# zbw2577/fea-large

Measured on AMD Instinct MI355X. Metric: element-stiffness assemblies/sec, higher is better.
Workload: dtype f64; 1 GPU; 10349856 TET4/1GP neohookean block (66x396x66 Kuhn cubes on the 1x6x1 bar), stiffness+residual assembly, deformed state k1=1.1; elements=10349856, nodes=1782133, scalar_nnz=236453589, clock_ramp_launches_before_warmup=80

## Files before the change

### fea-large_amd/csrc/feahip_internal.h

```cpp
#pragma once
#include <hip/hip_runtime.h>
#include <algorithm>
#include <cstdint>
#include <cstdio>
#include <initializer_list>
#include <string>
#include <thread>
#include <type_traits>
#include <vector>
#include "../../include/fea_hip.h"

hipError_t feahip_device_malloc(void **p, size_t bytes);
#define hipMalloc(p, bytes) feahip_device_malloc((void **)(p), (bytes))

#define FEA_MAX_NPE 10
#define FEA_MAX_GAUSS 27

#define FEA_CHUNK_BLOCKS 128
#define FEA_CHUNK_ROWS 16
#define FEA_WAVES_PER_WG 4
#define FEA_RED_BLOCKS 2048

struct ElemTable {
  double w[FEA_MAX_GAUSS];
  double dN[FEA_MAX_GAUSS][3][FEA_MAX_NPE];
};

#define FEA_HIP_CHECK(ctx, call)                                            \
  do {                                                                      \
    hipError_t _e = (call);                                                 \
    if (_e != hipSuccess) {                                                 \
      (ctx)->err = std::string(#call) + ": " + hipGetErrorString(_e);       \
      return FEAHIP_EHIP;                                                   \
    }                                                                       \
  } while (0)

template <class F>
void parallel_ranges(int n, int serial_below, F f)
{
  unsigned hw = std::thread::hardware_concurrency();
  int nt = (int)std::min<unsigned>(hw ? hw : 4, 32);
  if (n < serial_below) nt = 1;
  if (nt <= 1) { f(0, n); return; }
  std::vector<std::thread> th;
  for (int t = 0; t < nt; ++t) {
    int lo = (int)((long long)n * t / nt), hi = (int)((long long)n * (t + 1) / nt);
    th.emplace_back([=] { f(lo, hi); });
  }
  for (auto &x : th) x.join();
}
inline int round_up(int v, int m) { return (v + m - 1) / m * m; }

struct HostPattern {
  std::vector<int> rowptr, colidx;
  std::vector<int> incptr;
  std::vector<uint32_t> inc;
  std::vector<uint8_t> incslot;
  std::vector<int> chunk;
  std::vector<int> diag;
  std::vector<uint32_t> inc_rows;
  std::vector<int> achunk;
  std::vector<int> super_achunk;
  int max_rowlen = 0;
  int break_chunk = 0, break_super = 0;
};
int build_host_pattern(int N, int E, int npe, const int *conn, HostPattern &hp,
                       std::string &err, int row_break = -1);
inline int inc_elem(uint32_t w) { return (int)(w & 0x0FFFFFFFu); }
inline int inc_node(uint32_t w) { return (int)(w >> 28); }
inline int csr_pos(const HostPattern &hp, int a, int b)
{
  const int *cb = hp.colidx.data() + hp.rowptr[a], *ce = hp.colidx.data() + hp.rowptr[a + 1];
  return hp.rowptr[a] + (int)(std::lower_bound(cb, ce, b) - cb);
}

#define FEA_VISIT_MAX_NODES 64
#define FEA_VISIT_MAX_VISITS 128
#define FEA_ACHUNK_BLOCKS 80
#define FEA_ACHUNK_ROWS 8
#define FEA_SUPER_CHUNKS 8
struct VisitDesc {
  int r0, r1, b0, nb;
  int node_off, nnode;
  int visit_off, nvisit;
};
struct HostVisits {
  std::vector<VisitDesc> desc;
  std::vector<int> vnode;
  std::vector<uint32_t> vrec;
  bool ok = false;
};
void build_host_visits(int N, int E, const int *conn, const HostPattern &hp, HostVisits &out);
#define FEA_QUAD_BLOCKS 256
#define FEA_QUAD_PAIRS 512
#define FEA_QUAD_ELEMS 64
#define FEA_QUAD_NODES 126
#define FEA_QUAD_VISITS 96
struct QuadDesc {
  int r0, r1, b0, nb;
  int elem_off, nelem;
  int pair_off, npair;
  int node_off, nnode;
};
struct HostQuad {
  std::vector<QuadDesc> desc;
  std::vector<int> qnode;
  std::vector<uint32_t> qelem;
  std::vector<uint32_t> qpair;
  bool ok = false;
};
void build_host_quad(int N, int E, int npe, const int *conn, const HostPattern &hp, int p_lo, int p_hi, HostQuad &out);
int ensure_quad(feahip_ctx *c);
int launch_assemble_quad(feahip_ctx *c, bool doF);

inline bool first_visit(const HostPattern &hp, const int *conn, int npe, uint32_t w, int r0, int r)
{
  const int e = inc_elem(w), la = inc_node(w);
  for (int k = 0; k < npe; ++k) {
    const int g = conn[(size_t)e * npe + k];
    if (k != la && g >= r0 && g < r) return false;
  }
  return true;
}
template <class Fits>
void chunk_costs(const HostPattern &hp, const int *conn, int npe, int r0, int row_hi, int L, std::vector<int> &fresh,
                 uint16_t *cost, Fits fits)
{
  int nel = 0, ntask = 0;
  for (int l = 1; l <= L && r0 + l <= row_hi; ++l) {
    const int r = r0 + l - 1;
    fresh.clear();
    for (int q = hp.incptr[r]; q < hp.incptr[r + 1]; ++q)
      if (first_visit(hp, conn, npe, hp.inc_rows[q], r0, r)) fresh.push_back(inc_elem(hp.inc_rows[q]));
    nel += (int)fresh.size();
    const int *cb = hp.colidx.data() + hp.rowptr[r], *ce = hp.colidx.data() + hp.rowptr[r + 1];
    ntask += (int)(ce - cb) - 1 - (int)(std::lower_bound(cb, ce, r) - std::lower_bound(cb, ce, r0));
    if (!fits(r, l, nel, ntask, fresh)) break;
    cost[l - 1] = (uint16_t)nel;
  }
}
int partition_rows(const std::vector<uint16_t> &cost, int row_lo, int row_hi, int L, int alpha, std::vector<int> &first_row);
void chunk_elements(const HostPattern &hp, int r0, int r1, std::vector<int> &el);
void chunk_block_tasks(const HostPattern &hp, int r0, int r1, std::vector<uint32_t> &tpos, std::vector<int> &task_of);
void chunk_block_lists(const HostPattern &hp, const int *conn, int npe, int r0, int r1, const std::vector<int> &el,
                       const std::vector<int> &task_of, int ntask, int la_shift, int lb_shift,
                       std::vector<std::vector<uint16_t>> &lists);
long long count_distinct_elems(const HostPattern &hp, const int *conn, int npe, int r0, int r1);
struct HostChunkMaps {
  std::vector<unsigned char> blob;
  std::vector<int> first_row;
  long long total_evals = 0, distinct_elems = 0;
  int nchunks = 0;
  bool ok = false;
};

#ifndef FEA_G_BIG
#define FEA_G_BIG 1
#endif
#if FEA_G_BIG == 1
#define FEA_G_THREADS 1024
#define FEA_G_TASK_THREADS 768
#define FEA_G_MAX_ROWS 64
#define FEA_G_MAX_NODES 256
#define FEA_G_MAX_ELEMS 719
#define FEA_G_ELEMS_TARGET 672
#define FEA_G_CELL 4, 4, 4
#elif FEA_G_BIG == 2
#define FEA_G_THREADS 512
#define FEA_G_TASK_THREADS 384
#define FEA_G_MAX_ROWS 32
#define FEA_G_MAX_NODES 128
#define FEA_G_MAX_ELEMS 351
#define FEA_G_ELEMS_TARGET 320
#define FEA_G_CELL 4, 2, 3
#else
#define FEA_G_THREADS 256
#define FEA_G_TASK_THREADS 192
#define FEA_G_MAX_ROWS 16
#define FEA_G_MAX_NODES 128
#define FEA_G_MAX_ELEMS 239
#define FEA_G_ELEMS_TARGET 216
#define FEA_G_CELL 4, 2, 2
#endif
#define FEA_G_DIAG_LANES (FEA_G_THREADS - FEA_G_TASK_THREADS)
#define FEA_G_SLOT_BITS 10
#define FEA_G_MAX_SLOTS 1024
#define FEA_G_REGW 6
struct GatherHeader {
  int r0, r1, b0, nb;
  int nnode, nelem, noffd, depth;
  int nvthr, vdepth;
  int ddepth;
  unsigned wdepth[3];
  int flags;
  int pad[1];
};
static_assert(sizeof(GatherHeader) == 64 && FEA_G_TASK_THREADS / 64 <= 12, "GatherHeader: 64 bytes, twelve block-wave slots");
struct GatherLayout {
  int stride;
  int o_nodes, o_elems, o_bpos, o_rows, o_vlist, o_dlist, o_clist;
  int max_nodes, max_elems, max_tile;
  int max_tasks, max_depth, max_vthr, max_vdepth, max_ddepth;
  int o_emat;
};
struct HostGather : HostChunkMaps {
  GatherLayout lay;
  int same_as_previous = 0;
};
void build_host_gather(int N, int E, const int *conn, const HostPattern &hp, int row_lo, int row_hi, HostGather &out,
                       const uint8_t *elem_mat = nullptr);
int ensure_gather(feahip_ctx *c);
int launch_assemble_gather(feahip_ctx *c, bool doK, bool doF);

#ifndef FEA_Q_THREADS
#define FEA_Q_THREADS 256
#endif
#define FEA_Q_WAVES (FEA_Q_THREADS / 64)
#define FEA_Q_MAX_ROWS 64
#define FEA_Q_MAX_NODES 240
#define FEA_Q_MAX_ELEMS 127
#ifndef FEA_Q_SLOTS
#define FEA_Q_SLOTS 5
#endif
#define FEA_Q_REGW 4
#define FEA_Q_MAX_PASS 7
#define FEA_Q_FLANES 128
#define FEA_Q_ROWS_U16 200
struct Gather10Header {
  int r0, r1, b0, nb;
  int nnode, nelem, ntask, npass;
  int nft, fdw;
  unsigned char prow[8];
  unsigned char cnt[40];
  unsigned char sw[8];
  int pad[8];
};
static_assert(FEA_Q_SLOTS * FEA_Q_WAVES <= 40 && FEA_Q_SLOTS <= 8, "Gather10Header: cnt / sw too small");
static_assert(sizeof(Gather10Header) == 128, "Gather10Header is 128 bytes");
struct Gather10Layout {
  int stride;
  int o_nodes, o_elems, o_rows, o_tpos, o_flist, o_clist;
  int max_nodes, max_elems, max_cw, max_fdw, tile_blocks;
};
enum Gather10Limit {
  G10_FITS = FEAHIP_G10_LIMIT_NONE, G10_ELEMS = FEAHIP_G10_LIMIT_ELEMS, G10_ROW_LENGTH = FEAHIP_G10_LIMIT_ROW_LENGTH,
  G10_TASKS = FEAHIP_G10_LIMIT_TASKS, G10_RESIDUAL_LANES = FEAHIP_G10_LIMIT_RESIDUAL_LANES,
  G10_LIST_LENGTH = FEAHIP_G10_LIMIT_LIST_LENGTH, G10_PASSES = FEAHIP_G10_LIMIT_PASSES, G10_OTHER = FEAHIP_G10_LIMIT_OTHER
};
struct HostGather10 : HostChunkMaps {
  Gather10Layout lay;
  std::vector<int> elist;
  int npe = 10;
  int limit = G10_FITS;
  int limit_row = -1;
  int tile_blocks = 0;
};
void build_host_gather10(int N, int E, int npe, const int *conn, const HostPattern &hp, int row_lo, int row_hi, HostGather10 &out);
int ensure_gather10(feahip_ctx *c);
int launch_assemble_gather10(feahip_ctx *c, bool doK, bool doF);

int launch_assemble_visit(feahip_ctx *c, bool doK, bool doF);

enum class MapOutcome { none, built, failed, declined };
struct MapCache {
  int key0 = -1, key1 = -1;
  MapOutcome outcome = MapOutcome::none;
  long long bytes = 0;
  bool built() const { return outcome == MapOutcome::built; }
  bool is(MapOutcome o, int k0, int k1) const { return outcome == o && key0 == k0 && key1 == k1; }
  bool settled(int k0, int k1) const { return is(MapOutcome::built, k0, k1) || is(MapOutcome::failed, k0, k1); }
  void record(MapOutcome o, int k0, int k1) { outcome = o; key0 = k0; key1 = k1; }
};
inline void dev_free(std::initializer_list<void *> ptrs) { for (void *p : ptrs) if (p) (void)hipFree(p); }
struct GenericMaps : MapCache {
  int *d_incptr = nullptr;
  uint32_t *d_inc = nullptr;
  uint8_t *d_incslot = nullptr;
  void release() { dev_free({d_incptr, d_inc, d_incslot}); *this = GenericMaps(); }
};
struct VisitMaps : MapCache {
  VisitDesc *d_desc = nullptr;
  int *d_node = nullptr;
  uint32_t *d_rec = nullptr;
  int nrecords = 0;
  void release() { dev_free({d_desc, d_node, d_rec}); *this = VisitMaps(); }
};
struct QuadMaps : MapCache {
  QuadDesc *d_desc = nullptr;
  uint32_t *d_elem = nullptr, *d_pair = nullptr;
  int *d_node = nullptr;
  int nchunks = 0;
  void release() { dev_free({d_desc, d_elem, d_pair, d_node}); *this = QuadMaps(); }
};
struct GatherCache : MapCache {
  unsigned char *d_maps = nullptr;
  int nchunks = 0;
  double evals_per_element = 0;
  int same_words = 0;
};
struct GatherMaps : GatherCache {
  GatherLayout lay{};
  void release() { dev_free({d_maps}); *this = GatherMaps(); }
};
struct Gather10Maps : GatherCache {
  Gather10Layout lay{};
  int *d_elist = nullptr;
  double *d_state = nullptr;
  int nloc = 0;
  void release() { dev_free({d_maps, d_elist, d_state}); *this = Gather10Maps(); }
};

struct SurfaceLoads {
  int nfaces = 0, npf = 0;
  std::vector<int> h_lnode;
  int *d_fnode = nullptr;
  int *d_kind = nullptr;
  double *d_val = nullptr;
  double *d_fc = nullptr;
  int *d_lnode = nullptr, *d_lptr = nullptr, *d_lslot = nullptr;
  void release() { dev_free({d_fnode, d_kind, d_val, d_fc, d_lnode, d_lptr, d_lslot}); *this = SurfaceLoads(); }
};

struct MassState {
  bool set = false;
  bool stale = false;
  int n_rho = 0, n_mat = 0, Gm = 0;
  std::vector<double> rho, w, N, dN;
  double *d_m_base = nullptr;
  double *d_m = nullptr;
  long long kb0 = -1, kb1 = -1;
  double *d_vel = nullptr, *d_acc = nullptr, *d_xt = nullptr, *d_vt = nullptr;
  double *d_body = nullptr;
  double body[3] = {0, 0, 0};
  double time = 0;
  double *d_ml = nullptr;
  int ml_row0 = -1, ml_row1 = -1;
  double *d_ke_part = nullptr;
  int ke_parts = 0;
  void release_m() { dev_free({d_m_base}); d_m_base = d_m = nullptr; kb0 = kb1 = -1; }
  void release_lump() { dev_free({d_ml, d_ke_part}); d_ml = d_ke_part = nullptr; ml_row0 = ml_row1 = -1; ke_parts = 0; }
  void release() { dev_free({d_m_base, d_vel, d_acc, d_xt, d_vt, d_body, d_ml, d_ke_part}); *this = MassState(); }
};

struct feahip_ctx {
  int device = 0;
  hipStream_t stream = nullptr;
  std::string err;

  int N = 0, E = 0, npe = 0, G = 0, ndof = 0;
  int nnzb = 0;
  int nchunks = 0;
  int chunk0 = 0, nchunks_local = 0;
  int nachunks = 0, achunk0 = 0, nachunks_local = 0;
  std::vector<int> h_super_achunk, h_chunk;
  int rank = 0, nranks = 1, row0 = 0, row1 = 0;
  struct Transport *tr = nullptr;
  bool owns_tr = false;
  std::vector<int> peer, send_off, recv_off;
  int nsend = 0, nrecv = 0;
  int *d_send_idx = nullptr, *d_recv_idx = nullptr;
  double *d_send_buf = nullptr, *d_recv_buf = nullptr;
  int max_rowlen = 0;
  bool linear_tet = false;
  int model = 0;
  double lambda = 0, mu = 0;
  int n_materials = 0;
  std::vector<double> h_mat_params;
  std::vector<uint8_t> h_elem_mat;
  double2 *d_mat = nullptr;
  uint8_t *d_elem_mat = nullptr;
  double *d_f_discard = nullptr;
  int strategy = FEAHIP_ASM_AUTO;
  int last_strategy = FEAHIP_ASM_AUTO;

  ElemTable table;
  ElemTable *d_table = nullptr;

  int *d_conn = nullptr;
  double *d_X0 = nullptr;
  double *d_x = nullptr;
  int *d_rowptr = nullptr;
  int *d_colidx = nullptr;
  double *d_K = nullptr;
  double *d_Kstash = nullptr;
  double *d_K_base = nullptr, *d_Kstash_base = nullptr;
  double *d_K_alloc = nullptr, *d_Kstash_alloc = nullptr;
  long long kb0 = 0, kb1 = 0;
  bool have_stash = false;
  int *d_chunk = nullptr;
  int *d_diag = nullptr;
  GenericMaps generic;
  VisitMaps visits;
  QuadMaps quad;
  GatherMaps gather;
  Gather10Maps gather10;
  double *d_f = nullptr, *d_u = nullptr;
  double *d_r = nullptr, *d_p = nullptr, *d_q = nullptr, *d_minv = nullptr;
  double *d_part = nullptr;
  double *d_z = nullptr, *d_w = nullptr, *d_s = nullptr;
  int pcg_variant = -1;
  int ichunk_lo = 0, ichunk_hi = 0;
  hipStream_t comm_stream = nullptr;
  hipEvent_t ev_packed = nullptr, ev_unpacked = nullptr;
  double *d_scal = nullptr;
  int *d_flag = nullptr;
  int n_presc = 0;
  int n_cdof = 0;
  int *d_cdof = nullptr;
  double *d_cval = nullptr;
  uint8_t *d_dofmask = nullptr;
  double *d_F = nullptr, *d_S = nullptr;
  bool state_valid = false;

  std::vector<int> h_rowptr, h_colidx;
  std::vector<int> h_conn;
  struct HostPattern *h_pat = nullptr;
  bool incslot_ok = false;

  int last_bad = 0;

  std::vector<int> perm, iperm;
  int rank_own = -1;
  std::vector<int> rank_node_global, rank_elem_global;
  int rank_n_global = 0;
  int rank_e_global = 0;
  bool rank_local_ids = false;

  unsigned long long k_epoch = 0, stash_epoch = 0;
  bool k_bc = false;
  bool k_valid = false;
  int linesearch_max = 0;
  int precond = 0;
  void *amg = nullptr;
  void *coarse = nullptr;
  double *d_vred = nullptr;
  size_t vred_cap = 0;
  SurfaceLoads surf;
  double load_factor = 0;
  double *d2_f = nullptr, *d2_u = nullptr, *d2_r = nullptr, *d2_p = nullptr, *d2_q = nullptr;
  double *d_u2 = nullptr;
  double *d2_part = nullptr;
  double *d2_scal = nullptr;
  int *d2_flag = nullptr;
  MassState mass;
};

template <class F>
void with_kf(bool doK, bool doF, F &&f)
{
  if (doK && doF) f(std::true_type(), std::true_type());
  else if (doK)   f(std::true_type(), std::false_type());
  else            f(std::false_type(), std::true_type());
}

int launch_assemble(feahip_ctx *c, bool doK, bool doF);
int launch_state_export(feahip_ctx *c, double *d_grads = nullptr, double *d_detj = nullptr);
int launch_apply_bc(feahip_ctx *c, double lambda);
int launch_update_nodes_bc(feahip_ctx *c, double lambda);
int launch_surface_loads(feahip_ctx *c, double *d_fv);
int resolve_surface_faces(int N, int E, int npe, const int *conn, int nfaces, int npf, const int *face_nodes,
                          int *face_elem, int *face_local, std::string &why);
int set_surface_loads(feahip_ctx *c, int nfaces, int npf, const int *face_nodes, const int *kind, const double *values);
int ensure_generic_maps(feahip_ctx *c);
int ensure_k(feahip_ctx *c);
void release_k(feahip_ctx *c);
int ensure_visits(feahip_ctx *c);
int dist_nodes_add_scaled(std::vector<feahip_ctx *> &R, double eta, bool exchange);
int launch_update_nodes_solution(feahip_ctx *c, const double *d_u);
int launch_spmv(feahip_ctx *c, const double *d_xv, double *d_yv);
int precond_apply(feahip_ctx *c, const double *r, const double **z);
int solve_pcg(feahip_ctx *c, int type, double tol, int max_iter, int *iters,
              double *resid);
int time_pcg_iteration(feahip_ctx *c, int warmup, int iters, double *avg_ms);
bool pcg_outcome(int flag, int it, const double *scal, int *iters, double *resid);
void enq_reduce_final(feahip_ctx *c, int n, int nsums, int stride, const double *part, double *out);
void enq_precond_blockjacobi(feahip_ctx *c);
int ensure_solve2(feahip_ctx *c);
void release_solve2(feahip_ctx *c);
int solve2_refused(feahip_ctx *c, const char *who);
int launch_spmv2(feahip_ctx *c, const double *d_x2, double *d_y2);
int launch_interleave(feahip_ctx *c, const double *a, const double *b, double *out2);
int launch_deinterleave(feahip_ctx *c, const double *in2, double *a, double *b);
int solve_pcg2(feahip_ctx *c, int type, double tol, int max_iter, int *iters, double *resid);
int time_pcg2_iteration(feahip_ctx *c, int warmup, int iters, double *avg_ms);
int mass_set(feahip_ctx *c, int n_rho, const double *rho, int mass_points, const double *weights, const double *forms,
             const double *dforms);
int mass_ensure(feahip_ctx *c, const char *who);
int mass_set_body_force(feahip_ctx *c, const double *b);
int launch_body_force(feahip_ctx *c, double *d_fv);
int launch_mass_add(feahip_ctx *c, double coef);
int launch_mass_residual(feahip_ctx *c, double a0);
int launch_mass_product(feahip_ctx *c, const double *d_v4, double *d_y);
int launch_newmark_predict(feahip_ctx *c, double dt, double beta, double gamma);
int launch_newmark_correct(feahip_ctx *c, double dt, double beta, double gamma);
int launch_vec3_to_nodes(feahip_ctx *c, const double *d_v3, double *d_v4);
int lump_ensure(feahip_ctx *c, const char *who);
int launch_explicit_kick(feahip_ctx *c, double dt);
int launch_explicit_presc(feahip_ctx *c, double dlambda, double dt);
int launch_explicit_finish(feahip_ctx *c, double dt);
int launch_kinetic_energy(feahip_ctx *c, double *d_out);
// ... 98 lines not shown
```

### fea-large_amd/csrc/gather.cpp

```cpp
#include "feahip_internal.h"
#include <algorithm>
#include <cstdlib>
#include <cstring>

int partition_rows(const std::vector<uint16_t> &cost, int row_lo, int row_hi, int L, int alpha, std::vector<int> &first_row)
{
  const int nrows = row_hi - row_lo;
  std::vector<long long> best((size_t)nrows + 1, -1);
  std::vector<unsigned char> from((size_t)nrows + 1, 0);
  best[0] = 0;
  for (int j = 1; j <= nrows; ++j) {
    long long b = -1; int bl = 0;
    for (int l = 1; l <= L && l <= j; ++l) {
      const uint16_t c = cost[(size_t)(j - l) * L + (l - 1)];
      if (c == 0xFFFFu || best[j - l] < 0) continue;
      const long long v = best[j - l] + c + alpha;
      if (b < 0 || v < b) { b = v; bl = l; }
    }
    if (b < 0) return row_lo + j - 1;
    best[j] = b; from[j] = (unsigned char)bl;
  }
  std::vector<int> cuts;
  for (int j = nrows; j > 0; j -= from[j]) cuts.push_back(row_lo + j);
  cuts.push_back(row_lo);
  first_row.assign(cuts.rbegin(), cuts.rend());
  return -1;
}

void chunk_elements(const HostPattern &hp, int r0, int r1, std::vector<int> &el)
{
  el.clear();
  for (int q = hp.incptr[r0]; q < hp.incptr[r1]; ++q) el.push_back(inc_elem(hp.inc_rows[q]));
  std::sort(el.begin(), el.end());
  el.erase(std::unique(el.begin(), el.end()), el.end());
}

void chunk_block_tasks(const HostPattern &hp, int r0, int r1, std::vector<uint32_t> &tpos, std::vector<int> &task_of)
{
  const int b0 = hp.rowptr[r0];
  tpos.clear();
  task_of.assign((size_t)(hp.rowptr[r1] - b0), -1);
  for (int a = r0; a < r1; ++a)
    for (int q = hp.rowptr[a]; q < hp.rowptr[a + 1]; ++q) {
      const int b = hp.colidx[q];
      if (b == a || (b >= r0 && b < a)) continue;
      const uint32_t m = b > a && b < r1 ? (uint32_t)(csr_pos(hp, b, a) - b0) : 0xFFFFu;
      task_of[q - b0] = (int)tpos.size();
      tpos.push_back((uint32_t)(q - b0) | m << 16);
    }
}

void chunk_block_lists(const HostPattern &hp, const int *conn, int npe, int r0, int r1, const std::vector<int> &el,
                       const std::vector<int> &task_of, int ntask, int la_shift, int lb_shift,
                       std::vector<std::vector<uint16_t>> &lists)
{
  const int b0 = hp.rowptr[r0];
  lists.assign((size_t)ntask, std::vector<uint16_t>());
  for (int a = r0; a < r1; ++a)
    for (int q = hp.incptr[a]; q < hp.incptr[a + 1]; ++q) {
      const int e = inc_elem(hp.inc_rows[q]), la = inc_node(hp.inc_rows[q]);
      const int le = (int)(std::lower_bound(el.begin(), el.end(), e) - el.begin());
      for (int lb = 0; lb < npe; ++lb) {
        if (lb == la) continue;
        const int b = conn[(size_t)e * npe + lb];
        if (b == a) continue;
        const int t = task_of[csr_pos(hp, a, b) - b0];
        if (t < 0) continue;
        lists[(size_t)t].push_back((uint16_t)(le | la << la_shift | lb << lb_shift));
      }
    }
}

long long count_distinct_elems(const HostPattern &hp, const int *conn, int npe, int r0, int r1)
{
  long long d = 0;
  for (int a = r0; a < r1; ++a)
    for (int q = hp.incptr[a]; q < hp.incptr[a + 1]; ++q) d += first_visit(hp, conn, npe, hp.inc_rows[q], r0, a);
  return d;
}

#define G_RS 0
#define G_RD 66
#define G_VF 130
#define G_ROWS_U16 200
#define G_TASK_THREADS FEA_G_TASK_THREADS
#define G_SLOT(w) ((w) & 1023u)
#define G_LA(w) (((w) >> 10) & 3)
#define G_LB(w) (((w) >> 12) & 3)
#define G_NGROUPS (FEA_G_THREADS / 16)

namespace {
inline int b128_group(int t)
{
  static const unsigned char g32[32] = {0, 0, 0, 0, 1, 1, 1, 1, 1, 1, 1, 1, 0, 0, 0, 0, 1, 1, 1, 1, 0, 0, 0, 0, 0, 0, 0, 0, 1, 1, 1, 1};
  return (t >> 6) * 4 + ((t >> 5) & 1) * 2 + g32[t & 31];
}

bool partition(int N, const int *conn, const HostPattern &hp, int row_lo, int row_hi, std::vector<int> &first_row)
{
  int max_rows = FEA_G_MAX_ROWS, max_elems = FEA_G_BIG == 1 ? FEA_G_MAX_ELEMS : FEA_G_ELEMS_TARGET, alpha = 24;
  if (const char *e = getenv("FEAHIP_GATHER_ROWS")) max_rows = std::max(1, std::min(FEA_G_MAX_ROWS, atoi(e)));
  if (const char *e = getenv("FEAHIP_GATHER_ELEMS")) max_elems = std::max(8, std::min(FEA_G_MAX_ELEMS, atoi(e)));
  if (const char *e = getenv("FEAHIP_GATHER_ALPHA")) alpha = std::max(0, atoi(e));
  const int L = max_rows, nrows = row_hi - row_lo;
  std::vector<uint16_t> cost((size_t)nrows * L, 0xFFFFu);
  parallel_ranges(nrows, 4096, [&](int lo, int hi) {
    std::vector<int> nstamp((size_t)N, -1), fresh;
    for (int i = lo; i < hi; ++i) {
      const int r0 = row_lo + i;
      int nnod = 0, nvis = 0;
      chunk_costs(hp, conn, 4, r0, row_hi, L, fresh, &cost[(size_t)i * L], [&](int r, int l, int nel, int ntask, const std::vector<int> &fr) {
        if (nstamp[r] != r0) { nstamp[r] = r0; ++nnod; }
        for (int e : fr)
          for (int k = 0; k < 4; ++k) {
            const int g = conn[(size_t)e * 4 + k];
            if (nstamp[g] != r0) { nstamp[g] = r0; ++nnod; }
          }
        nvis += hp.incptr[r + 1] - hp.incptr[r];
        return nel <= (l > 1 ? max_elems : FEA_G_MAX_ELEMS) && nnod <= FEA_G_MAX_NODES && ntask <= G_TASK_THREADS &&
               nvis <= 4 * G_TASK_THREADS;
      });
    }
  });
  return partition_rows(cost, row_lo, row_hi, L, alpha, first_row) < 0;
}

struct Read { uint16_t set; uint8_t off; };

void sort_unique(std::vector<Read> &rv)
{
  std::sort(rv.begin(), rv.end(), [](const Read &a, const Read &b) { return a.set != b.set ? a.set < b.set : a.off < b.off; });
  rv.erase(std::unique(rv.begin(), rv.end(), [](const Read &a, const Read &b) { return a.set == b.set && a.off == b.off; }), rv.end());
}

void most_read_first(const std::vector<std::vector<Read>> &reads, std::vector<int> &order)
{
  order.resize(reads.size());
  for (size_t i = 0; i < reads.size(); ++i) order[i] = (int)i;
  std::stable_sort(order.begin(), order.end(), [&](int a, int b) { return reads[a].size() > reads[b].size(); });
}

void bank_slots(const std::vector<std::vector<Read>> &reads, const std::vector<int> &order, int nsets, int step,
                std::vector<int> cap, std::vector<uint8_t> &occ, std::vector<int> &res, std::vector<int> &slot)
{
  const int n = (int)reads.size();
  occ.assign((size_t)nsets * 16, 0);
  res.assign((size_t)n, -1);
  auto bank = [&](const Read &rd, int r) { return (size_t)rd.set * 16 + ((rd.off + step * r) & 15); };
  for (int pass = 0; pass < 2; ++pass)
    for (int i : order) {
      if (res[i] >= 0) {
        for (const Read &rd : reads[i]) --occ[bank(rd, res[i])];
        ++cap[res[i]];
      }
      int br = -1; long bc = 0;
      for (int r = 0; r < 16; ++r) {
        if (cap[r] <= 0) continue;
        long c = 0;
        for (const Read &rd : reads[i]) c += occ[bank(rd, r)];
        if (br < 0 || c < bc) { br = r; bc = c; }
      }
      res[i] = br; --cap[br];
      for (const Read &rd : reads[i]) ++occ[bank(rd, br)];
    }
  int next[16];
  for (int r = 0; r < 16; ++r) next[r] = r;
  slot.resize((size_t)n);
  for (int i = 0; i < n; ++i) { slot[i] = next[res[i]]; next[res[i]] += 16; }
}

struct Local {
  GatherHeader h;
  std::vector<int> nodes;
  std::vector<uint32_t> elems, tpos;
  std::vector<uint16_t> rows, vlist, clist, dlist;
  std::vector<uint8_t> emat;
};

struct ChunkBuilder {
  const int *conn;
  const HostPattern &hp;
  const uint8_t *elem_mat;
  int r0 = 0, r1 = 0, nrows = 0, b0 = 0, nb = 0, nelem = 0, nnode = 0, nslots = 0, nnslots = 0;
  int ntask = 0, wdepth[G_TASK_THREADS / 64] = {0}, dwords = 0, ddwords = 0, zslot = 0;
  std::vector<int> el, nd, task_of, thr_blk, order, res, eslot, nslot;
  std::vector<uint32_t> btpos;
  std::vector<std::vector<uint16_t>> blists, lists, dl;
  std::vector<std::vector<Read>> reads;
  std::vector<uint8_t> occ;

  ChunkBuilder(const int *c, const HostPattern &p, const uint8_t *em) : conn(c), hp(p), elem_mat(em) {}
  int lnode(int g) const { return (int)(std::lower_bound(nd.begin(), nd.end(), g) - nd.begin()); }
  int lelem(int e) const { return (int)(std::lower_bound(el.begin(), el.end(), e) - el.begin()); }

  bool build(int row0, int row1, Local &L)
  {
    r0 = row0; r1 = row1; nrows = r1 - r0; b0 = hp.rowptr[r0]; nb = hp.rowptr[r1] - b0;
    if (!chunk_lists(L)) return false;
    deal();
    bank_schedule();
    emit(L);
    return true;
  }

  bool chunk_lists(Local &L)
  {
    chunk_elements(hp, r0, r1, el);
    nd.clear();
    for (int a = r0; a < r1; ++a) nd.push_back(a);
    for (int e : el)
      for (int k = 0; k < 4; ++k) nd.push_back(conn[(size_t)e * 4 + k]);
    std::sort(nd.begin(), nd.end());
    nd.erase(std::unique(nd.begin(), nd.end()), nd.end());
    nnode = (int)nd.size(); nelem = (int)el.size();
    nslots = 16 * ((nelem + 1 + 15) / 16); nnslots = 16 * ((nnode + 15) / 16);
    if (nnslots > FEA_G_MAX_NODES || nslots > FEA_G_MAX_SLOTS || nrows > FEA_G_MAX_ROWS) return false;
    L.rows.assign(G_ROWS_U16, 0);
    for (int a = r0; a < r1; ++a) {
      L.rows[G_RS + (a - r0)] = (uint16_t)(hp.rowptr[a] - b0);
      L.rows[G_RD + (a - r0)] = (uint16_t)(hp.diag[a] - b0);
    }
    L.rows[G_RS + nrows] = (uint16_t)nb;
    chunk_block_tasks(hp, r0, r1, btpos, task_of);
    const int nblk = (int)btpos.size();
    if (nblk > G_TASK_THREADS) return false;
    chunk_block_lists(hp, conn, 4, r0, r1, el, task_of, nblk, 10, 12, blists);
    dl.assign((size_t)4 * FEA_G_MAX_ROWS, std::vector<uint16_t>());
    for (int a = r0; a < r1; ++a)
      for (int q = hp.incptr[a], kv = 0; q < hp.incptr[a + 1]; ++q, ++kv)
        dl[(size_t)4 * (a - r0) + (kv & 3)].push_back((uint16_t)(lelem(inc_elem(hp.inc_rows[q])) | (inc_node(hp.inc_rows[q]) << 10)));
    return true;
  }

  void deal()
  {
    constexpr int NBW = G_TASK_THREADS / 64;
    const int nblk = (int)btpos.size();
    thr_blk.assign((size_t)G_TASK_THREADS, -1);
    std::fill(wdepth, wdepth + NBW, 0);
    ntask = 0;
    auto words = [&](int i) { return ((int)blists[i].size() + 1) / 2; };
    order.resize((size_t)nblk);
    for (int i = 0; i < nblk; ++i) order[i] = i;
    std::stable_sort(order.begin(), order.end(), [&](int x, int y) { return words(x) > words(y); });
    std::vector<int> seq;
    seq.reserve((size_t)nblk);
    for (size_t c0 = 0; c0 < order.size();) {
      size_t c1 = c0;
      while (c1 < order.size() && words(order[c1]) == words(order[c0])) ++c1;
      std::vector<int> bucket[16];
      for (size_t k = c0; k < c1; ++k) bucket[btpos[order[k]] & 15u].push_back(order[k]);
      size_t left = c1 - c0;
      while (left) {
        const int room = 16 - (int)(seq.size() & 15);
        int rs[16];
        for (int r = 0; r < 16; ++r) rs[r] = r;
        std::stable_sort(rs, rs + 16, [&](int x, int y) { return bucket[x].size() > bucket[y].size(); });
        unsigned mused = 0;
        int taken = 0;
        for (int pass = 0; pass < 2 && taken < room && left; ++pass)
          for (int q = 0; q < 16 && taken < room && left; ++q) {
            std::vector<int> &bk = bucket[rs[q]];
            if (bk.empty()) continue;
            size_t pick = 0;
            for (size_t c = 0; c < bk.size() && c < 8; ++c) {
              const unsigned mp = btpos[bk[c]] >> 16;
              if (mp == 0xFFFFu || !((mused >> (mp & 15u)) & 1u)) { pick = c; break; }
            }
            const unsigned mp = btpos[bk[pick]] >> 16;
            if (mp != 0xFFFFu) mused |= 1u << (mp & 15u);
            seq.push_back(bk[pick]);
            bk.erase(bk.begin() + (long)pick);
            ++taken; --left;
          }
      }
      c0 = c1;
    }
    const int nwaves = (nblk + 63) / 64;
    std::vector<int> wcost((size_t)nwaves, 0), word((size_t)nwaves);
    for (int w = 0; w < nwaves; ++w) {
      for (int l = 0; l < 64 && w * 64 + l < nblk; ++l) wcost[w] = std::max(wcost[w], words(seq[(size_t)w * 64 + l]));
      word[w] = w;
    }
    std::stable_sort(word.begin(), word.end(), [&](int x, int y) { return wcost[x] > wcost[y]; });
    int load[4] = {0, 0, 0, 0}, used[4] = {0, 0, 0, 0};
    for (int w : word) {
      int bs = -1;
      for (int sd = 0; sd < 4; ++sd)
        if (used[sd] * 4 + sd < NBW && (bs < 0 || load[sd] < load[bs])) bs = sd;
      const int slot = used[bs] * 4 + bs;
      ++used[bs]; load[bs] += wcost[w];
      wdepth[slot] = wcost[w];
      for (int l = 0; l < 64 && w * 64 + l < nblk; ++l) thr_blk[(size_t)slot * 64 + l] = seq[(size_t)w * 64 + l];
      ntask = std::max(ntask, slot * 64 + std::min(64, nblk - w * 64));
    }
    lists.assign((size_t)ntask, std::vector<uint16_t>());
    for (int t = 0; t < ntask; ++t)
      if (thr_blk[t] >= 0) lists[t] = blists[thr_blk[t]];
    int depth = 0, ddepth = 0;
    for (auto &l : lists) depth = std::max(depth, (int)l.size());
    for (auto &l : dl) ddepth = std::max(ddepth, (int)l.size());
    dwords = (depth + 1) / 2; ddwords = (ddepth + 1) / 2;
  }

  void bank_schedule()
  {
    reads.assign((size_t)nelem, std::vector<Read>());
    const int nsteps = std::max(2 * dwords, 2 * ddwords);
    auto add_reads = [&](int lane, int step, uint16_t w, bool diag) {
      const int le = (int)G_SLOT(w), la = G_LA(w), lb = G_LB(w);
      const int grp = b128_group(lane);
      const int offs[6] = {la, 8 + la, diag ? 4 + la : lb, diag ? -1 : 4 + lb, diag ? -1 : 8 + lb, 12};
      for (int kind = 0; kind < 6; ++kind)
        if (offs[kind] >= 0) reads[le].push_back({(uint16_t)((grp * nsteps + step) * 6 + kind), (uint8_t)offs[kind]});
    };
    for (int t = 0; t < ntask; ++t)
      for (size_t k = 0; k < lists[t].size(); ++k) add_reads(t, (int)k, lists[t][k], false);
    for (int l = 0; l < 4 * nrows; ++l)
      for (size_t k = 0; k < dl[l].size(); ++k) add_reads(G_TASK_THREADS + l, (int)k, dl[l][k], true);
    most_read_first(reads, order);
    for (auto &rv : reads) sort_unique(rv);
    std::vector<int> cap(16, nslots / 16);
    --cap[15];
    bank_slots(reads, order, G_NGROUPS * nsteps * 6, -3, cap, occ, res, eslot);
    std::vector<char> used((size_t)nslots, 0);
    for (int e = 0; e < nelem; ++e) used[eslot[e]] = 1;
    zslot = 0;
    while (used[zslot]) ++zslot;

    reads.assign((size_t)nnode, std::vector<Read>());
    for (int e = 0; e < nelem; ++e)
      for (int k = 0; k < 4; ++k) reads[lnode(conn[(size_t)el[e] * 4 + k])].push_back({(uint16_t)(b128_group(eslot[e]) * 4 + k), 0});
    for (auto &rv : reads) sort_unique(rv);
    most_read_first(reads, order);
    bank_slots(reads, order, G_NGROUPS * 4, 1, std::vector<int>(16, nnslots / 16), occ, res, nslot);
  }

  void emit(Local &L)
  {
    L.nodes.assign((size_t)nnslots, 0);
    for (int i = 0; i < nnode; ++i) L.nodes[nslot[i]] = nd[i];
    L.elems.assign((size_t)nslots, 0xFFFFFFFFu);
    for (int i = 0; i < nelem; ++i) {
      uint32_t w = 0;
      for (int k = 0; k < 4; ++k) w |= (uint32_t)nslot[lnode(conn[(size_t)el[i] * 4 + k])] << (8 * k);
      L.elems[eslot[i]] = w;
    }
    L.emat.clear();
    if (elem_mat) {
      L.emat.assign((size_t)nslots, 0);
      for (int i = 0; i < nelem; ++i) L.emat[eslot[i]] = elem_mat[el[i]];
    }
    L.tpos.assign((size_t)ntask, 0xFFFFFFFFu);
    for (int t = 0; t < ntask; ++t)
      if (thr_blk[t] >= 0) L.tpos[t] = btpos[thr_blk[t]];
    auto reslot = [&](uint16_t w) { return (uint16_t)((w & 0xFC00u) | (uint16_t)eslot[G_SLOT(w)]); };
    L.clist.assign((size_t)dwords * 2 * FEA_G_THREADS, (uint16_t)zslot);
    for (int t = 0; t < ntask; ++t)
      for (size_t k = 0; k < lists[t].size(); ++k)
        L.clist[((size_t)(k / 2) * FEA_G_THREADS + t) * 2 + (k & 1)] = reslot(lists[t][k]);
    L.dlist.assign((size_t)ddwords * 2 * FEA_G_DIAG_LANES, (uint16_t)zslot);
    for (int l = 0; l < 4 * nrows; ++l)
      for (size_t k = 0; k < dl[l].size(); ++k)
        L.dlist[((size_t)(k / 2) * FEA_G_DIAG_LANES + l) * 2 + (k & 1)] = reslot(dl[l][k]);
    int vdepth = 1;
    for (;; ++vdepth) {
      int need = 0;
      for (int a = r0; a < r1; ++a) need += (hp.incptr[a + 1] - hp.incptr[a] + vdepth - 1) / vdepth;
      if (need <= G_TASK_THREADS) break;
    }
    int nvthr = 0;
    for (int a = r0; a < r1; ++a) {
      L.rows[G_VF + (a - r0)] = (uint16_t)nvthr;
      nvthr += (hp.incptr[a + 1] - hp.incptr[a] + vdepth - 1) / vdepth;
    }
    L.rows[G_VF + nrows] = (uint16_t)nvthr;
    L.vlist.assign((size_t)vdepth * FEA_G_THREADS, (uint16_t)zslot);
    for (int a = r0; a < r1; ++a) {
      const int t0 = L.rows[G_VF + (a - r0)];
      for (int q = hp.incptr[a], k = 0; q < hp.incptr[a + 1]; ++q, ++k)
        L.vlist[(size_t)(k % vdepth) * FEA_G_THREADS + t0 + k / vdepth] = (uint16_t)(eslot[lelem(inc_elem(hp.inc_rows[q]))] | (inc_node(hp.inc_rows[q]) << 10));
    }
    GatherHeader &h = L.h;
    memset(&h, 0, sizeof(h));
    h.r0 = r0; h.r1 = r1; h.b0 = b0; h.nb = nb; h.nnode = nnslots; h.nelem = nslots; h.noffd = ntask;
    h.depth = dwords; h.nvthr = nvthr; h.vdepth = vdepth; h.ddepth = ddwords;
    for (int w = 0; w < G_TASK_THREADS / 64; ++w) h.wdepth[w >> 2] |= (unsigned)std::min(wdepth[w], 255) << (8 * (w & 3));
  }
};

bool lay_out(const std::vector<Local> &loc, bool materials, HostGather &out)
{
  const int nch = (int)loc.size();
  int m_v = 0, m_c = 0, m_d = 0, g_nodes = 0, g_elems = 0, g_tile = 0;
  GatherLayout &lay = out.lay;
  memset(&lay, 0, sizeof(lay));
  for (const Local &L : loc) {
    m_v = std::max(m_v, (int)L.vlist.size() * 2); m_c = std::max(m_c, (int)L.clist.size() * 2); m_d = std::max(m_d, (int)L.dlist.size() * 2);
    g_nodes = std::max(g_nodes, L.h.nnode); g_elems = std::max(g_elems, L.h.nelem); g_tile = std::max(g_tile, L.h.nb);
    lay.max_tasks = std::max(lay.max_tasks, L.h.noffd); lay.max_depth = std::max(lay.max_depth, L.h.depth);
    lay.max_vthr = std::max(lay.max_vthr, L.h.nvthr); lay.max_vdepth = std::max(lay.max_vdepth, L.h.vdepth);
    lay.max_ddepth = std::max(lay.max_ddepth, L.h.ddepth);
  }
  lay.max_nodes = g_nodes; lay.max_elems = g_elems; lay.max_tile = g_tile;
  lay.o_nodes = 64;
  lay.o_elems = lay.o_nodes + round_up(4 * FEA_G_MAX_NODES, 64);
  lay.o_bpos = lay.o_elems + round_up(4 * FEA_G_THREADS, 64);
  lay.o_rows = lay.o_bpos + round_up(4 * FEA_G_THREADS, 64);
  lay.o_vlist = lay.o_rows + round_up(2 * G_ROWS_U16, 64);
  lay.o_dlist = lay.o_vlist + round_up(m_v, 64);
  lay.o_clist = lay.o_dlist + round_up(m_d, 64);
  lay.stride = round_up(lay.o_clist + m_c, 128);
  if (materials) { lay.o_emat = lay.stride; lay.stride += round_up(FEA_G_THREADS, 128); }
  if ((long long)nch * lay.stride > 0x7FFFFFFF00LL) return false;
  out.blob.assign((size_t)nch * lay.stride, 0);
  parallel_ranges(nch, 512, [&](int lo, int hi) {
    for (int p = lo; p < hi; ++p) {
      const Local &L = loc[p];
      unsigned char *rec = out.blob.data() + (size_t)p * lay.stride;
      memcpy(rec, &L.h, sizeof(GatherHeader));
      memcpy(rec + lay.o_nodes, L.nodes.data(), L.nodes.size() * 4);
      memcpy(rec + lay.o_elems, L.elems.data(), L.elems.size() * 4);
      memcpy(rec + lay.o_bpos, L.tpos.data(), L.tpos.size() * 4);
      memcpy(rec + lay.o_rows, L.rows.data(), L.rows.size() * 2);
      memcpy(rec + lay.o_vlist, L.vlist.data(), L.vlist.size() * 2);
      memcpy(rec + lay.o_dlist, L.dlist.data(), L.dlist.size() * 2);
      memcpy(rec + lay.o_clist, L.clist.data(), L.clist.size() * 2);
      if (lay.o_emat) memcpy(rec + lay.o_emat, L.emat.data(), L.emat.size());
    }
  });
  return true;
}

void mark_repeats(HostGather &out, int nch)
{
  const GatherLayout &lay = out.lay;
  out.same_as_previous = 0;
  for (int p = 0; p + 1 < nch; ++p) {
    const unsigned char *r0 = out.blob.data() + (size_t)p * lay.stride, *r1 = r0 + lay.stride;
    const GatherHeader &h0 = *reinterpret_cast<const GatherHeader *>(r0), &h1 = *reinterpret_cast<const GatherHeader *>(r1);
    const bool same = h0.nelem == h1.nelem && h0.noffd == h1.noffd && h0.depth == h1.depth && h0.nvthr == h1.nvthr &&
                      h0.vdepth == h1.vdepth && h0.ddepth == h1.ddepth && h0.r1 - h0.r0 == h1.r1 - h1.r0 &&
                      memcmp(r0 + lay.o_elems, r1 + lay.o_elems, (size_t)((lay.o_emat ? lay.o_emat : lay.stride) - lay.o_elems)) == 0;
    if (same) { reinterpret_cast<GatherHeader *>(out.blob.data() + (size_t)p * lay.stride)->flags |= 1; ++out.same_as_previous; }
  }
}
}

void build_host_gather(int N, int E, const int *conn, const HostPattern &hp, int row_lo, int row_hi, HostGather &out,
                       const uint8_t *elem_mat)
{
  (void)E;
  out.ok = false; out.nchunks = 0; out.blob.clear(); out.first_row.clear();
  if (row_lo < 0 || row_hi > N || row_lo >= row_hi) return;
  if (!partition(N, conn, hp, row_lo, row_hi, out.first_row)) return;
  const int nch = (int)out.first_row.size() - 1;
  std::vector<Local> loc((size_t)nch);
  std::vector<char> bad((size_t)nch, 0);
  parallel_ranges(nch, 512, [&](int lo, int hi) {
    ChunkBuilder cb(conn, hp, elem_mat);
    for (int p = lo; p < hi; ++p) bad[p] = !cb.build(out.first_row[p], out.first_row[p + 1], loc[p]);
  });
  for (int p = 0; p < nch; ++p)
    if (bad[p]) return;
  if (!lay_out(loc, elem_mat != nullptr, out)) return;
  mark_repeats(out, nch);
  out.nchunks = nch;
  out.total_evals = 0;
  for (const Local &L : loc)
    for (uint32_t w : L.elems) out.total_evals += w != 0xFFFFFFFFu;
  out.distinct_elems = count_distinct_elems(hp, conn, 4, row_lo, row_hi);
  out.ok = true;
}

namespace {
inline unsigned long long mix(unsigned long long h, unsigned long long v)
{
  h ^= v + 0x9E3779B97F4A7C15ull + (h << 6) + (h >> 2);
  return h * 0xBF58476D1CE4E5B9ull;
}
inline unsigned long long contribution_hash(int a, int b, const int *g, int npe, int pair)
{
  unsigned long long h = 0x1234567ull;
  h = mix(h, (unsigned long long)a); h = mix(h, (unsigned long long)b);
  for (int k = 0; k < npe; ++k) h = mix(h, (unsigned long long)g[k]);
  return mix(h, (unsigned long long)pair);
}
int row_of(const HostPattern &hp, int r0, int r1, int b0, int pos)
{
  int a = r0;
  while (a + 1 < r1 && hp.rowptr[a + 1] - b0 <= pos) ++a;
  return a;
}

void gather_row_digest(const HostGather &hg, const HostPattern &hp, unsigned long long *rowhash)
{
  const GatherLayout &lay = hg.lay;
  for (int p = 0; p < hg.nchunks; ++p) {
    const unsigned char *rec = hg.blob.data() + (size_t)p * lay.stride;
    const GatherHeader &h = *reinterpret_cast<const GatherHeader *>(rec);
    const int *nodes = reinterpret_cast<const int *>(rec + lay.o_nodes);
    const uint32_t *elems = reinterpret_cast<const uint32_t *>(rec + lay.o_elems);
    const uint32_t *tpos = reinterpret_cast<const uint32_t *>(rec + lay.o_bpos);
    const uint16_t *clist = reinterpret_cast<const uint16_t *>(rec + lay.o_clist);
    const uint16_t *dlist = reinterpret_cast<const uint16_t *>(rec + lay.o_dlist);
    auto element_nodes = [&](int slot, int g[4]) {
      for (int k = 0; k < 4; ++k) g[k] = nodes[(elems[slot] >> (8 * k)) & 255u];
    };
    for (int t = 0; t < h.noffd; ++t) {
      if (tpos[t] == 0xFFFFFFFFu) continue;
      const int bpos = (int)(tpos[t] & 0xFFFFu), mpos = (int)(tpos[t] >> 16);
      const int a = row_of(hp, h.r0, h.r1, h.b0, bpos), b = hp.colidx[h.b0 + bpos];
      for (int k = 0; k < 2 * h.depth; ++k) {
        const uint16_t w = clist[((size_t)(k / 2) * FEA_G_THREADS + t) * 2 + (k & 1)];
        const int slot = (int)G_SLOT(w), la = G_LA(w), lb = G_LB(w);
        if (elems[slot] == 0xFFFFFFFFu) continue;
        int g[4];
        element_nodes(slot, g);
        rowhash[a] += contribution_hash(a, b, g, 4, la * 4 + lb);
        if (mpos != 0xFFFF) rowhash[b] += contribution_hash(b, a, g, 4, lb * 4 + la);
      }
    }
    for (int l = 0; l < 4 * (h.r1 - h.r0); ++l)
      for (int k = 0; k < 2 * h.ddepth; ++k) {
        const uint16_t w = dlist[((size_t)(k / 2) * FEA_G_DIAG_LANES + l) * 2 + (k & 1)];
        const int slot = (int)G_SLOT(w), la = G_LA(w);
        if (elems[slot] == 0xFFFFFFFFu) continue;
        int g[4];
        element_nodes(slot, g);
        const int a = h.r0 + (l >> 2);
        rowhash[a] += contribution_hash(a, a, g, 4, la * 4 + la);
      }
  }
}

void gather10_row_digest(const HostGather10 &hg, const HostPattern &hp, const int *conn, unsigned long long *rowhash)
{
  const Gather10Layout &lay = hg.lay;
  for (int p = 0; p < hg.nchunks; ++p) {
    const unsigned char *rec = hg.blob.data() + (size_t)p * lay.stride;
    const Gather10Header &h = *reinterpret_cast<const Gather10Header *>(rec);
    const uint32_t *elems = reinterpret_cast<const uint32_t *>(rec + lay.o_elems);
    const uint32_t *tpos = reinterpret_cast<const uint32_t *>(rec + lay.o_tpos);
    const uint16_t *cl = reinterpret_cast<const uint16_t *>(rec + lay.o_clist);
    int row0 = 0;
    for (int s = 0; s < FEA_Q_SLOTS; ++s) {
      for (int t = 0; t < FEA_Q_THREADS; ++t) {
        const uint32_t tw = tpos[s * FEA_Q_THREADS + t];
        if (tw == 0xFFFFFFFFu) continue;
        const int bpos = (int)(tw & 0xFFFFu), mpos = (int)(tw >> 16);
        const int a = row_of(hp, h.r0, h.r1, h.b0, bpos), b = hp.colidx[h.b0 + bpos];
        for (int k = 0; k < 2 * h.sw[s]; ++k) {
          const uint16_t w = cl[(((size_t)row0 + k / 2) * FEA_Q_THREADS + t) * 2 + (k & 1)];
          const int le = w & 127, la = (w >> 7) & 15, lb = (w >> 11) & 15;
          if (le == lay.max_elems) continue;
          int g[16];
          for (int j = 0; j < hg.npe; ++j) g[j] = conn[(size_t)hg.elist[elems[le]] * hg.npe + j];
          rowhash[a] += contribution_hash(a, b, g, hg.npe, la * 16 + lb);
          if (mpos != 0xFFFF) rowhash[b] += contribution_hash(b, a, g, hg.npe, lb * 16 + la);
        }
      }
      row0 += h.sw[s];
    }
  }
}

void quad_row_digest(const HostQuad &hq, const HostPattern &hp, unsigned long long *rowhash)
{
  for (const QuadDesc &d : hq.desc) {
    for (int p = 0; p < d.npair; ++p) {
      const uint32_t w = hq.qpair[(size_t)d.pair_off + p];
      const int eli = (int)(w & 63u), la = (int)((w >> 6) & 15u), lb = (int)((w >> 10) & 15u), pos = (int)((w >> 14) & 255u);
      const int a = d.r0 + (int)((w >> 22) & 15u), b = hp.colidx[d.b0 + pos];
      const uint32_t *we = hq.qelem.data() + ((size_t)d.elem_off + eli) * 3;
      int g[10];
      for (int k = 0; k < 10; ++k) g[k] = hq.qnode[(size_t)d.node_off + ((we[k / 4] >> (8 * (k % 4))) & 255u)];
      rowhash[a] += contribution_hash(a, b, g, 10, la * 16 + lb);
    }
  }
}
}

extern "C" int feahip_host_assembly_digest(int n_nodes, int n_elems, int npe, const int *elements, int rank, int nranks,
                                           unsigned long long *rowhash, int *rows)
{
  if (!elements || !rowhash || !rows || n_nodes <= 0 || n_elems <= 0 || nranks < 1 || rank < 0 || rank >= nranks) return FEAHIP_EINVAL;
  HostPattern hp;
  std::string err;
  int rc = build_host_pattern(n_nodes, n_elems, npe, elements, hp, err);
  if (rc) return rc;
  int row0, row1;
  shard_row_range(hp.chunk, rank, nranks, row0, row1);
  rows[0] = row0; rows[1] = row1;
  for (int a = 0; a < n_nodes; ++a) rowhash[a] = 0;
  if (npe == 4) {
    HostGather hg;
    build_host_gather(n_nodes, n_elems, elements, hp, row0, row1, hg);
    if (!hg.ok) return FEAHIP_EINVAL;
    gather_row_digest(hg, hp, rowhash);
  } else {
    bool done = false;
    if (npe == 10 || npe == 8) {
      HostGather10 hg;
      build_host_gather10(n_nodes, n_elems, npe, elements, hp, row0, row1, hg);
      if (hg.ok && (double)hg.total_evals <= 12.0 * (double)hg.distinct_elems) {
        gather10_row_digest(hg, hp, elements, rowhash);
        done = true;
      }
    }
    if (!done) {
      if (hp.super_achunk.empty()) return FEAHIP_EINVAL;
      const int nchunks = (int)hp.chunk.size() - 1;
      const int nsuper = (nchunks + FEA_SUPER_CHUNKS - 1) / FEA_SUPER_CHUNKS;
      const int s0 = (int)((long long)nsuper * rank / nranks), s1 = (int)((long long)nsuper * (rank + 1) / nranks);
      HostQuad hq;
      build_host_quad(n_nodes, n_elems, npe, elements, hp, hp.super_achunk[s0], hp.super_achunk[s1], hq);
      if (!hq.ok) return FEAHIP_EINVAL;
      quad_row_digest(hq, hp, rowhash);
    }
  }
  return FEAHIP_OK;
}

extern "C" int feahip_host_gather_stats(int n_nodes, int n_elems, int npe, const int *elements, long long *stats, int *rows_hist)
{
  if (!elements || !stats || n_nodes <= 0 || n_elems <= 0 || (npe != 4 && npe != 10 && npe != 8)) return FEAHIP_EINVAL;
  HostPattern hp;
  std::string err;
  int rc = build_host_pattern(n_nodes, n_elems, npe, elements, hp, err);
  if (rc) return rc;
  stats[6] = stats[7] = 0;
  HostGather hg;
  HostGather10 hq;
  const HostChunkMaps &m = npe == 4 ? static_cast<const HostChunkMaps &>(hg) : hq;
  if (npe == 4) build_host_gather(n_nodes, n_elems, elements, hp, 0, n_nodes, hg);
  else build_host_gather10(n_nodes, n_elems, npe, elements, hp, 0, n_nodes, hq);
  if (!m.ok) return FEAHIP_EINVAL;
  stats[0] = m.nchunks; stats[1] = m.total_evals; stats[2] = m.distinct_elems; stats[3] = n_nodes;
  stats[4] = npe == 4 ? hg.same_as_previous : 0; stats[5] = (long long)m.blob.size();
  if (npe == 4) {
    for (int p = 0; p < hg.nchunks; ++p) {
      const GatherHeader &gh = *reinterpret_cast<const GatherHeader *>(hg.blob.data() + (size_t)p * hg.lay.stride);
      stats[6] += gh.depth > FEA_G_REGW; stats[7] += gh.ddepth > FEA_G_REGW;
    }
    if (getenv("FEAHIP_NUMBERING_VERBOSE")) {
      int hd[17] = {0}, hdd[17] = {0};
      for (int p = 0; p < hg.nchunks; ++p) {
        const GatherHeader &gh = *reinterpret_cast<const GatherHeader *>(hg.blob.data() + (size_t)p * hg.lay.stride);
        ++hd[std::min(gh.depth, 16)]; ++hdd[std::min(gh.ddepth, 16)];
      }
      for (int k = 0; k <= 16; ++k) if (hd[k] || hdd[k]) fprintf(stderr, "gather maps: %d words: %d chunks by block list, %d by diagonal list\n", k, hd[k], hdd[k]);
    }
  }
  if (rows_hist) {
    for (int l = 0; l <= FEA_G_MAX_ROWS; ++l) rows_hist[l] = 0;
    for (int p = 0; p < m.nchunks; ++p) ++rows_hist[std::min(m.first_row[p + 1] - m.first_row[p], FEA_G_MAX_ROWS)];
  }
  return FEAHIP_OK;
}

extern "C" int feahip_host_gather_chunks(int n_nodes, int n_elems, const int *elements, int capacity, int *flags)
{
  if (!elements || n_nodes <= 0 || n_elems <= 0 || capacity < 0 || (capacity > 0 && !flags)) return FEAHIP_EINVAL;
  HostPattern hp;
  std::string err;
  int rc = build_host_pattern(n_nodes, n_elems, 4, elements, hp, err);
  if (rc) return rc;
  HostGather hg;
  build_host_gather(n_nodes, n_elems, elements, hp, 0, n_nodes, hg);
  if (!hg.ok) return FEAHIP_EINVAL;
  for (int p = 0; p < hg.nchunks && p < capacity; ++p) {
    const GatherHeader &gh = *reinterpret_cast<const GatherHeader *>(hg.blob.data() + (size_t)p * hg.lay.stride);
    flags[p] = (gh.flags & 1) | (gh.depth > FEA_G_REGW ? 2 : 0) | (gh.ddepth > FEA_G_REGW ? 4 : 0);
  }
  return hg.nchunks;
}

#ifdef FEAHIP_DEBUG
extern "C" int feahip_debug_gather_record_host(int n_nodes, int n_elems, const int *elements, int chunk, int *layout_ints,
                                               unsigned char *record, int *nchunks)
{
  static HostGather hg;
  static int cached_n = -1, cached_e = -1;
  if (cached_n != n_nodes || cached_e != n_elems) {
    HostPattern hp;
    std::string err;
    if (build_host_pattern(n_nodes, n_elems, 4, elements, hp, err)) return FEAHIP_EINVAL;
    build_host_gather(n_nodes, n_elems, elements, hp, 0, n_nodes, hg);
    if (!hg.ok) return FEAHIP_EINVAL;
    cached_n = n_nodes; cached_e = n_elems;
  }
  if (chunk < 0) chunk = hg.nchunks / 2;
  memcpy(layout_ints, &hg.lay, sizeof(GatherLayout));
  if (nchunks) *nchunks = hg.nchunks;
  if (record) memcpy(record, hg.blob.data() + (size_t)chunk * hg.lay.stride, hg.lay.stride);
  return (int)(sizeof(GatherLayout) / sizeof(int));
}
#endif
```

### fea-large_amd/csrc/gather_device.h

```cpp
#pragma once
#include "fem_device.h"
#define PRIO_STATE 0
#define PRIO_GATHER 1
#define PRIO_OUT 3
#include <algorithm>
#include <cstdlib>
#include <cstring>

struct GatherArgs {
  int chunk0, nchunks, model;
  double lambda, mu;
  const ElemTable *tab;
  const unsigned char *maps;
  GatherLayout lay;
  const double *X0, *x;
  double *K, *f;
  int *bad;
  unsigned long long *stamps;
  int ablate;
  const double2 *mat;
};
#if defined(FEAHIP_DEBUG) && !defined(FEAHIP_NOABL)
#define G_ABL(bit) (A.ablate & (bit))
#else
#define G_ABL(bit) 0
#endif

#ifdef FEAHIP_DEBUG
#define G_STAMP(i) do { if (A.stamps) st[i] = __builtin_amdgcn_s_memtime(); } while (0)
#else
#define G_STAMP(i) do { } while (0)
#endif

#define G_RS 0
#define G_RD 66
#define G_VF 130
#define G_SLOT(w) ((w) & 1023u)
#define G_LA(w) (((w) >> 10) & 3)
#define G_LB(w) (((w) >> 12) & 3)

#define GREC 26
#define GREC_F 12

struct GRead { double2 pa, za, pb, qb, zb, vv; };
__device__ __forceinline__ GRead g_fetch(const double *sT, unsigned w)
{
  const double2 *T = reinterpret_cast<const double2 *>(sT + G_SLOT(w) * GREC);
  const int la = G_LA(w), lb = G_LB(w);
  GRead r;
  r.pa = T[la]; r.za = T[8 + la]; r.pb = T[lb]; r.qb = T[4 + lb]; r.zb = T[8 + lb]; r.vv = T[12];
  return r;
}
__device__ __forceinline__ void g_apply(const GRead &r, double (&acc)[9], double &accd)
{
  const double ga0 = r.pa.x, ga1 = r.pa.y, ga2 = r.za.x;
  const double gb0 = r.pb.x, gb1 = r.pb.y, gb2 = r.zb.x;
  const double tb0 = r.qb.x, tb1 = r.qb.y, tb2 = r.zb.y;
  const double vl = r.vv.x, vm = r.vv.y;
  const double h0 = vl * gb0, h1 = vl * gb1, h2 = vl * gb2;
  const double m0 = vm * gb0, m1 = vm * gb1, m2 = vm * gb2;
  accd = fma(ga0, tb0, fma(ga1, tb1, fma(ga2, tb2, accd)));
  acc[0] = fma(ga0, h0, fma(ga0, m0, acc[0])); acc[1] = fma(ga0, h1, fma(ga1, m0, acc[1])); acc[2] = fma(ga0, h2, fma(ga2, m0, acc[2]));
  acc[3] = fma(ga1, h0, fma(ga0, m1, acc[3])); acc[4] = fma(ga1, h1, fma(ga1, m1, acc[4])); acc[5] = fma(ga1, h2, fma(ga2, m1, acc[5]));
  acc[6] = fma(ga2, h0, fma(ga0, m2, acc[6])); acc[7] = fma(ga2, h1, fma(ga1, m2, acc[7])); acc[8] = fma(ga2, h2, fma(ga2, m2, acc[8]));
}
__device__ __forceinline__ void g_finish(double (&acc)[9], double accd)
{
  acc[0] += accd; acc[4] += accd; acc[8] += accd;
}
__device__ __forceinline__ void g_consume(const double *sT, unsigned w, double (&acc)[9], double &accd)
{
  g_apply(g_fetch(sT, w), acc, accd);
}
__device__ __forceinline__ void g_apply_cheap(const GRead &r, double (&acc)[9])
{
  acc[0] += r.pa.x; acc[1] += r.za.x; acc[2] += r.pb.x; acc[3] += r.qb.x; acc[4] += r.zb.x; acc[5] += r.vv.x;
}
__device__ __forceinline__ GRead g_fetch_cheap(const double *sT, unsigned w)
{
  GRead r; const double v = (double)w;
  r.pa = make_double2(v, v); r.za = r.pa; r.pb = r.pa; r.qb = r.pa; r.zb = r.pa; r.vv = r.pa;
  return r;
}

template <bool DOF>
__device__ __forceinline__ void g_consume_diag(const double *sT, unsigned w, double (&a)[6], double (&fa)[3])
{
  const double2 *T = reinterpret_cast<const double2 *>(sT + G_SLOT(w) * GREC);
  const int la = G_LA(w);
  const double2 pa = T[la], qa = T[4 + la], za = T[8 + la], vv = T[12];
  const double s = vv.x + vv.y;
  const double d = pa.x * qa.x + pa.y * qa.y + za.x * za.y;
  const double h0 = s * pa.x, h1 = s * pa.y, h2 = s * za.x;
  a[0] += fma(h0, pa.x, d); a[1] = fma(h0, pa.y, a[1]); a[2] = fma(h0, za.x, a[2]);
  a[3] += fma(h1, pa.y, d); a[4] = fma(h1, za.x, a[4]); a[5] += fma(h2, za.x, d);
  if (DOF) {
    fa[0] -= __dsub_rn(qa.x, __dmul_rn(vv.y, pa.x)); fa[1] -= __dsub_rn(qa.y, __dmul_rn(vv.y, pa.y)); fa[2] -= __dsub_rn(za.y, __dmul_rn(vv.y, za.x));
  }
}

template <bool DOK>
__device__ __forceinline__ void g_visit(const double *sT, unsigned w, double (&fa)[3])
{
  const int la = G_LA(w);
  if (DOK) {
    const double2 *T = reinterpret_cast<const double2 *>(sT + G_SLOT(w) * GREC);
    const double2 pa = T[la], qa = T[4 + la], za = T[8 + la];
    const double vm = T[12].y;
    fa[0] -= qa.x - vm * pa.x; fa[1] -= qa.y - vm * pa.y; fa[2] -= za.y - vm * za.x;
  } else {
    const double *T = sT + G_SLOT(w) * GREC_F;
    const double2 pa = *reinterpret_cast<const double2 *>(T + 2 * la);
    fa[0] -= pa.x; fa[1] -= pa.y; fa[2] -= T[8 + la];
  }
}

#define G_W2(addr, a, b, o) asm volatile("ds_write2_b64 %0, %1, %2 offset0:%3 offset1:%4" : : "v"(addr), "v"(a), "v"(b), "n"(o), "n"((o) + 1) : "memory")
#define G_LDS_DRAIN() asm volatile("s_waitcnt lgkmcnt(0)" ::: "memory")
#ifndef G_W128
#define G_W128 1
#endif
typedef double g_v2d __attribute__((ext_vector_type(2)));
#if G_W128
#undef G_W2
#define G_W2(addr, a, b, o) do { const g_v2d pr_ = {a, b}; asm volatile("ds_write_b128 %0, %1 offset:%2" : : "v"(addr), "v"(pr_), "n"((o) * 8) : "memory"); } while (0)
#endif

template <bool DOK>
__device__ __forceinline__ void g_store_record(double *dst, const double *R)
{
  const unsigned a = (unsigned)(size_t)(__attribute__((address_space(3))) const void *)dst;
  G_W2(a, R[0], R[1], 0); G_W2(a, R[3], R[4], 2); G_W2(a, R[6], R[7], 4); G_W2(a, R[9], R[10], 6);
  if (DOK) {
    G_W2(a, R[12], R[13], 8); G_W2(a, R[15], R[16], 10); G_W2(a, R[18], R[19], 12); G_W2(a, R[21], R[22], 14);
    G_W2(a, R[2], R[14], 16); G_W2(a, R[5], R[17], 18); G_W2(a, R[8], R[20], 20); G_W2(a, R[11], R[23], 22);
    G_W2(a, R[24], R[25], 24);
  } else {
    G_W2(a, R[2], R[5], 8); G_W2(a, R[8], R[11], 10);
  }
}

template <bool DOK>
__device__ __forceinline__ double lintet_record_nh(const double (&x)[4][3], const double (&X)[4][3], double w,
                                                   double lambda, double mu, double *R)
{
  double J[3][3], D[3][3];
#pragma unroll
  for (int i = 0; i < 3; ++i)
#pragma unroll
    for (int j = 0; j < 3; ++j) { J[i][j] = x[i + 1][j] - x[0][j]; D[i][j] = X[i + 1][j] - X[0][j]; }
  double c[3][3];
  c[0][0] = J[1][1] * J[2][2] - J[1][2] * J[2][1]; c[0][1] = J[1][2] * J[2][0] - J[1][0] * J[2][2]; c[0][2] = J[1][0] * J[2][1] - J[1][1] * J[2][0];
  c[1][0] = J[0][2] * J[2][1] - J[0][1] * J[2][2]; c[1][1] = J[0][0] * J[2][2] - J[0][2] * J[2][0]; c[1][2] = J[0][1] * J[2][0] - J[0][0] * J[2][1];
  c[2][0] = J[0][1] * J[1][2] - J[0][2] * J[1][1]; c[2][1] = J[0][2] * J[1][0] - J[0][0] * J[1][2]; c[2][2] = J[0][0] * J[1][1] - J[0][1] * J[1][0];
  const double detJ = J[0][0] * c[0][0] + J[0][1] * c[0][1] + J[0][2] * c[0][2];
  const double id = fd_rcp(detJ);
  double g[4][3];
#pragma unroll
  for (int k = 0; k < 3; ++k)
#pragma unroll
    for (int i = 0; i < 3; ++i) g[k + 1][i] = c[k][i] * id;
#pragma unroll
  for (int i = 0; i < 3; ++i) g[0][i] = -((g[1][i] + g[2][i]) + g[3][i]);
  double Fi[3][3];
#pragma unroll
  for (int i = 0; i < 3; ++i)
#pragma unroll
    for (int j = 0; j < 3; ++j) Fi[i][j] = g[1][j] * D[0][i] + g[2][j] * D[1][i] + g[3][j] * D[2][i];
  const double detFi = fd_det3(Fi);
  const double Jd = fd_rcp(detFi);
  const double lnJ = -fd_log(detFi);
  double c00 = 0, c01 = 0, c02 = 0, c11 = 0, c12 = 0, c22 = 0;
#pragma unroll
  for (int i = 0; i < 3; ++i) {
    c00 += Fi[i][0] * Fi[i][0]; c01 += Fi[i][0] * Fi[i][1]; c02 += Fi[i][0] * Fi[i][2];
    c11 += Fi[i][1] * Fi[i][1]; c12 += Fi[i][1] * Fi[i][2]; c22 += Fi[i][2] * Fi[i][2];
  }
  const double vol = w * fabs(detJ);
  const double m1 = (mu - lambda * lnJ) * detFi;
  const double vm = vol * m1;
  const double mJ = (vol * mu) * Jd;
  const double a00 = c11 * c22 - c12 * c12, a11 = c00 * c22 - c02 * c02, a22 = c00 * c11 - c01 * c01;
  const double a01 = c02 * c12 - c01 * c22, a02 = c01 * c12 - c02 * c11, a12 = c01 * c02 - c00 * c12;
  if (DOK) {
    const double T00 = mJ * a00, T11 = mJ * a11, T22 = mJ * a22, T01 = mJ * a01, T02 = mJ * a02, T12 = mJ * a12;
#pragma unroll
    for (int b = 0; b < 4; ++b)
#pragma unroll
      for (int i = 0; i < 3; ++i) R[b * 3 + i] = g[b][i];
#pragma unroll
    for (int b = 0; b < 4; ++b) {
      R[12 + b * 3 + 0] = fma(T00, g[b][0], fma(T01, g[b][1], T02 * g[b][2]));
      R[12 + b * 3 + 1] = fma(T11, g[b][1], fma(T01, g[b][0], T12 * g[b][2]));
      R[12 + b * 3 + 2] = fma(T22, g[b][2], fma(T02, g[b][0], T12 * g[b][1]));
    }
    R[24] = (vol * lambda) * detFi;
    R[25] = vm;
  } else {
    double S[3][3];
    S[0][0] = mJ * a00 - vm; S[1][1] = mJ * a11 - vm; S[2][2] = mJ * a22 - vm;
    S[0][1] = S[1][0] = mJ * a01; S[0][2] = S[2][0] = mJ * a02; S[1][2] = S[2][1] = mJ * a12;
#pragma unroll
    for (int b = 1; b < 4; ++b)
#pragma unroll
      for (int i = 0; i < 3; ++i) R[b * 3 + i] = S[i][0] * g[b][0] + S[i][1] * g[b][1] + S[i][2] * g[b][2];
#pragma unroll
    for (int i = 0; i < 3; ++i) R[i] = -((R[3 + i] + R[6 + i]) + R[9 + i]);
  }
  return detJ;
}

template <bool DOK>
__device__ __forceinline__ double lintet_record_a5(const double (&x)[4][3], const double (&X)[4][3], double w,
                                                   double lambda, double mu, double *R)
{
  double J[3][3], D[3][3];
#pragma unroll
  for (int i = 0; i < 3; ++i)
#pragma unroll
    for (int j = 0; j < 3; ++j) { J[i][j] = x[i + 1][j] - x[0][j]; D[i][j] = X[i + 1][j] - X[0][j]; }
  double c[3][3];
  c[0][0] = J[1][1] * J[2][2] - J[1][2] * J[2][1]; c[0][1] = J[1][2] * J[2][0] - J[1][0] * J[2][2]; c[0][2] = J[1][0] * J[2][1] - J[1][1] * J[2][0];
  c[1][0] = J[0][2] * J[2][1] - J[0][1] * J[2][2]; c[1][1] = J[0][0] * J[2][2] - J[0][2] * J[2][0]; c[1][2] = J[0][1] * J[2][0] - J[0][0] * J[2][1];
  c[2][0] = J[0][1] * J[1][2] - J[0][2] * J[1][1]; c[2][1] = J[0][2] * J[1][0] - J[0][0] * J[1][2]; c[2][2] = J[0][0] * J[1][1] - J[0][1] * J[1][0];
  const double detJ = J[0][0] * c[0][0] + J[0][1] * c[0][1] + J[0][2] * c[0][2];
  const double id = fd_rcp(detJ);
  double g[4][3];
#pragma unroll
  for (int k = 0; k < 3; ++k)
#pragma unroll
    for (int i = 0; i < 3; ++i) g[k + 1][i] = c[k][i] * id;
#pragma unroll
  for (int i = 0; i < 3; ++i) g[0][i] = -((g[1][i] + g[2][i]) + g[3][i]);
  double Fi[3][3];
#pragma unroll
  for (int i = 0; i < 3; ++i)
#pragma unroll
    for (int j = 0; j < 3; ++j) Fi[i][j] = g[1][j] * D[0][i] + g[2][j] * D[1][i] + g[3][j] * D[2][i];
  double A[3][3];
  A[0][0] = Fi[1][1] * Fi[2][2] - Fi[1][2] * Fi[2][1]; A[0][1] = Fi[0][2] * Fi[2][1] - Fi[0][1] * Fi[2][2]; A[0][2] = Fi[0][1] * Fi[1][2] - Fi[0][2] * Fi[1][1];
  A[1][0] = Fi[1][2] * Fi[2][0] - Fi[1][0] * Fi[2][2]; A[1][1] = Fi[0][0] * Fi[2][2] - Fi[0][2] * Fi[2][0]; A[1][2] = Fi[0][2] * Fi[1][0] - Fi[0][0] * Fi[1][2];
  A[2][0] = Fi[1][0] * Fi[2][1] - Fi[1][1] * Fi[2][0]; A[2][1] = Fi[0][1] * Fi[2][0] - Fi[0][0] * Fi[2][1]; A[2][2] = Fi[0][0] * Fi[1][1] - Fi[0][1] * Fi[1][0];
  const double detFi = Fi[0][0] * A[0][0] + Fi[0][1] * A[1][0] + Fi[0][2] * A[2][0];
  const double Jd = fd_rcp(detFi), J2 = Jd * Jd;
  const double b00 = J2 * (A[0][0] * A[0][0] + A[0][1] * A[0][1] + A[0][2] * A[0][2]);
  const double b01 = J2 * (A[0][0] * A[1][0] + A[0][1] * A[1][1] + A[0][2] * A[1][2]);
  const double b02 = J2 * (A[0][0] * A[2][0] + A[0][1] * A[2][1] + A[0][2] * A[2][2]);
  const double b11 = J2 * (A[1][0] * A[1][0] + A[1][1] * A[1][1] + A[1][2] * A[1][2]);
  const double b12 = J2 * (A[1][0] * A[2][0] + A[1][1] * A[2][1] + A[1][2] * A[2][2]);
  const double b22 = J2 * (A[2][0] * A[2][0] + A[2][1] * A[2][1] + A[2][2] * A[2][2]);
  const double I1 = 0.5 * ((b00 + b11 + b22) - 3.0);
  const double vol = w * fabs(detJ);
  const double vd = vol * detFi;
  const double a_ = vd * (lambda * I1 - mu), m_ = vd * mu;
  double S[3][3];
  S[0][0] = a_ * b00 + m_ * (b00 * b00 + b01 * b01 + b02 * b02);
  S[1][1] = a_ * b11 + m_ * (b01 * b01 + b11 * b11 + b12 * b12);
  S[2][2] = a_ * b22 + m_ * (b02 * b02 + b12 * b12 + b22 * b22);
  S[0][1] = S[1][0] = a_ * b01 + m_ * (b00 * b01 + b01 * b11 + b02 * b12);
  S[0][2] = S[2][0] = a_ * b02 + m_ * (b00 * b02 + b01 * b12 + b02 * b22);
  S[1][2] = S[2][1] = a_ * b12 + m_ * (b01 * b02 + b11 * b12 + b12 * b22);
  const double vm = vd * mu;
  if (DOK) {
#pragma unroll
    for (int b = 0; b < 4; ++b)
#pragma unroll
      for (int i = 0; i < 3; ++i) R[b * 3 + i] = g[b][i];
    const double T00 = S[0][0] + vm, T11 = S[1][1] + vm, T22 = S[2][2] + vm;
#pragma unroll
    for (int b = 0; b < 4; ++b) {
      R[12 + b * 3 + 0] = fma(T00, g[b][0], fma(S[0][1], g[b][1], S[0][2] * g[b][2]));
      R[12 + b * 3 + 1] = fma(T11, g[b][1], fma(S[0][1], g[b][0], S[1][2] * g[b][2]));
      R[12 + b * 3 + 2] = fma(T22, g[b][2], fma(S[0][2], g[b][0], S[1][2] * g[b][1]));
    }
    R[24] = vd * lambda;
    R[25] = vm;
  } else {
#pragma unroll
    for (int b = 1; b < 4; ++b)
#pragma unroll
      for (int i = 0; i < 3; ++i) R[b * 3 + i] = S[i][0] * g[b][0] + S[i][1] * g[b][1] + S[i][2] * g[b][2];
#pragma unroll
    for (int i = 0; i < 3; ++i) R[i] = -((R[3 + i] + R[6 + i]) + R[9 + i]);
  }
  return detJ;
}

template <int CTRL>
__device__ __forceinline__ double g_quad_perm(double x)
{
  int lo = __double2loint(x), hi = __double2hiint(x);
  lo = __builtin_amdgcn_update_dpp(0, lo, CTRL, 0xF, 0xF, true);
  hi = __builtin_amdgcn_update_dpp(0, hi, CTRL, 0xF, 0xF, true);
  return __hiloint2double(hi, lo);
}
__device__ __forceinline__ double g_quad_sum(double v)
{
  v += g_quad_perm<0xB1>(v);
  v += g_quad_perm<0x4E>(v);
  return v;
}

#define G_BARRIER() do { __builtin_amdgcn_fence(__ATOMIC_RELEASE, "workgroup", "local"); __builtin_amdgcn_s_barrier(); \
                         __builtin_amdgcn_fence(__ATOMIC_ACQUIRE, "workgroup", "local"); } while (0)

typedef int g_v8i __attribute__((ext_vector_type(8)));
typedef int g_v4i __attribute__((ext_vector_type(4)));

struct GMaps {
  unsigned eids, tpos, cw[FEA_G_REGW], vw[2];
  int kd, vb, ve;
};

#define G_TASK_THREADS FEA_G_TASK_THREADS

template <bool DOK, bool DOF>
__device__ __forceinline__ void g_load_maps(const GatherLayout &lay, const unsigned char *rec, int t, GMaps &m)
{
  const unsigned short *rows = reinterpret_cast<const unsigned short *>(rec + lay.o_rows);
  m.eids = 0xFFFFFFFFu; m.tpos = 0; m.kd = m.vb = m.ve = 0;
#pragma unroll
  for (int k = 0; k < FEA_G_REGW; ++k) m.cw[k] = 0;
  m.vw[0] = m.vw[1] = 0;
  if (t < lay.max_elems) m.eids = reinterpret_cast<const unsigned *>(rec + lay.o_elems)[t];
  if (DOK && t < ((lay.max_tasks + 63) & ~63)) {
    m.tpos = reinterpret_cast<const unsigned *>(rec + lay.o_bpos)[t];
#pragma unroll
    for (int k = 0; k < FEA_G_REGW; ++k)
      if (k < lay.max_depth) m.cw[k] = reinterpret_cast<const unsigned *>(rec + lay.o_clist)[k * FEA_G_THREADS + t];
  }
  if (DOK && t >= G_TASK_THREADS) {
    const int l = t - G_TASK_THREADS;
    m.kd = rows[G_RD + (l >> 2)];
#pragma unroll
    for (int k = 0; k < FEA_G_REGW; ++k)
      if (k < lay.max_ddepth) m.cw[k] = reinterpret_cast<const unsigned *>(rec + lay.o_dlist)[k * FEA_G_DIAG_LANES + l];
  }
  if (!DOK && t < ((lay.max_vthr + 63) & ~63)) {
#pragma unroll
// ... 10 lines not shown
```

### fea-large_amd/csrc/kernels_gather.hip

```cpp
#include "gather_device.h"
#ifndef G_NT_ROWS
#define G_NT_ROWS 1
#endif
template <bool DOK, bool DOF, bool NH, bool HET>
__global__ __launch_bounds__(FEA_G_THREADS, FEA_G_BIG ? 4 : 3)
void k_assemble_gather(GatherArgs A, int run_len)
{
  extern __shared__ double2 g_smem[];
  double2 *sC = g_smem;
  double *sT = reinterpret_cast<double *>(g_smem + A.lay.max_nodes * 3);
  const int t = threadIdx.x;
#ifdef FEAHIP_DEBUG
  unsigned long long st[8] = {0, 0, 0, 0, 0, 0, 0, 0}, sa[8] = {0, 0, 0, 0, 0, 0, 0, 0};
  const unsigned long long clk0 = __builtin_amdgcn_s_memtime(), real0 = __builtin_amdgcn_s_memrealtime();
#endif
  const int nruns = (A.nchunks + run_len - 1) / run_len;
  const int per = ((int)gridDim.x + 7) >> 3;
  const int ridx = ((int)blockIdx.x & 7) * per + ((int)blockIdx.x >> 3);
  if (ridx >= nruns) return;
  int chunk = ridx * run_len;
  const int cend = min(A.nchunks, chunk + run_len);
  constexpr int REC = DOK ? GREC : GREC_F;
  const size_t stride = (size_t)A.lay.stride;
  const unsigned char *rec = A.maps + (size_t)(A.chunk0 + chunk) * stride;
  const bool node_lane = t < A.lay.max_nodes;
  const int wslot = __builtin_amdgcn_readfirstlane(t >> 6);

  const double gauss_w = A.tab->w[0];
  GMaps mn;
  g_load_maps<DOK, DOF>(A.lay, G_ABL(64) ? A.maps + (size_t)A.chunk0 * stride : rec, t, mn);
  GatherHeader hn = *reinterpret_cast<const GatherHeader *>(rec);
  int node1 = reinterpret_cast<const int *>(rec + A.lay.o_nodes)[t & (FEA_G_MAX_NODES - 1)];
  if (node_lane) {
    const double *gx = A.x + (size_t)node1 * 4, *gX = A.X0 + (size_t)node1 * 4;
    const double2 a0 = *reinterpret_cast<const double2 *>(gx), a1 = *reinterpret_cast<const double2 *>(gx + 2);
    const double2 c0 = *reinterpret_cast<const double2 *>(gX), c1 = *reinterpret_cast<const double2 *>(gX + 2);
    sC[t * 3] = a0; sC[t * 3 + 1] = make_double2(a1.x, c0.x); sC[t * 3 + 2] = make_double2(c0.y, c1.x);
  }
  {
    const int cn = min(chunk + 1, cend - 1);
    node1 = reinterpret_cast<const int *>(A.maps + (size_t)(A.chunk0 + cn) * stride + A.lay.o_nodes)[t & (FEA_G_MAX_NODES - 1)];
  }
  int mid1 = 0;
  double2 pn = make_double2(A.lambda, A.mu);
  if constexpr (HET) {
    pn = A.mat[rec[A.lay.o_emat + t]];
    const int cn = min(chunk + 1, cend - 1);
    mid1 = (A.maps + (size_t)(A.chunk0 + cn) * stride + A.lay.o_emat)[t];
    asm volatile("" : : "v"(mid1), "v"(pn.x), "v"(pn.y));
  }
  asm volatile("" : : "v"(mn.eids), "v"(mn.tpos), "v"(mn.cw[0]), "v"(mn.cw[1]), "v"(mn.cw[2]), "v"(mn.cw[3]), "v"(mn.cw[4]), "v"(mn.cw[5]),
               "v"(mn.vw[0]), "v"(mn.vw[1]), "v"(mn.kd), "v"(mn.vb), "v"(mn.ve), "v"(node1), "v"(gauss_w));
  G_BARRIER();

  for (;;) {
    G_STAMP(0);
    const bool more = chunk + 1 < cend;
    const GatherHeader h = hn;
    int hword;
    double2 ca0, ca1, cc0, cc1;
    const GMaps m = mn;
    const int nrows = h.r1 - h.r0;
    const unsigned wdw = wslot < 4 ? h.wdepth[0] : (wslot < 8 ? h.wdepth[1] : h.wdepth[2]);
    const int wd = wslot < G_TASK_THREADS / 64 ? (int)((wdw >> (8 * (wslot & 3))) & 255u) : 0;
    rec = A.maps + (size_t)(A.chunk0 + chunk) * stride;

    __builtin_amdgcn_s_setprio(PRIO_STATE);
    if (t < h.nelem && m.eids != 0xFFFFFFFFu) {
      const unsigned eids = m.eids;
      const int nd[4] = {(int)(eids & 255u), (int)((eids >> 8) & 255u), (int)((eids >> 16) & 255u), (int)(eids >> 24)};
      double xe[4][3], Xe[4][3];
#pragma unroll
      for (int k = 0; k < 4; ++k) {
        const double2 *cc = sC + nd[k] * 3;
        const double2 p0 = cc[0], p1 = cc[1], p2 = cc[2];
        xe[k][0] = p0.x; xe[k][1] = p0.y; xe[k][2] = p1.x;
        Xe[k][0] = p1.y; Xe[k][1] = p2.x; Xe[k][2] = p2.y;
      }
      double R[REC];
      double detJ;
      if (G_ABL(8)) { detJ = 1.0; for (int q = 0; q < REC; ++q) R[q] = xe[q & 3][q % 3] + Xe[(q >> 2) & 3][q % 3]; }
      else detJ = NH ? lintet_record_nh<DOK>(xe, Xe, gauss_w, HET ? pn.x : A.lambda, HET ? pn.y : A.mu, R)
                     : lintet_record_a5<DOK>(xe, Xe, gauss_w, HET ? pn.x : A.lambda, HET ? pn.y : A.mu, R);
      if (!(detJ > 0.0)) {
        if (DOK) {
          const int *gn = reinterpret_cast<const int *>(rec + A.lay.o_nodes);
          const int g0 = min(min(gn[nd[0]], gn[nd[1]]), min(gn[nd[2]], gn[nd[3]]));
          if (g0 >= h.r0 && g0 < h.r1) atomicAdd(A.bad, 1);
        }
      }
      if (detJ == 0.0) {
        double2 *o = reinterpret_cast<double2 *>(sT + t * REC);
#pragma unroll
        for (int q = 0; q < REC / 2; ++q) o[q] = make_double2(0.0, 0.0);
      } else if (!G_ABL(1)) g_store_record<DOK>(sT + t * REC, R);
      else sT[t * REC] = R[0] + R[25 % REC];
    } else if (t < h.nelem) {
      double2 *o = reinterpret_cast<double2 *>(sT + t * REC);
#pragma unroll
      for (int q = 0; q < REC / 2; ++q) o[q] = make_double2(0.0, 0.0);
    }
    {
      const int c1 = min(chunk + 1, cend - 1), c2 = min(chunk + 2, cend - 1);
      const unsigned char *rec1 = A.maps + (size_t)(A.chunk0 + c1) * stride;
      hword = reinterpret_cast<const int *>(rec1)[t & 15];
      if (!(h.flags & 1) || G_ABL(64)) g_load_maps<DOK, DOF>(A.lay, G_ABL(64) ? A.maps + (size_t)A.chunk0 * stride : rec1, t, mn);
      if (wslot < FEA_G_MAX_NODES / 64) {
        const size_t n1 = (size_t)(node_lane ? node1 : 0);
        ca0 = *reinterpret_cast<const double2 *>(A.x + n1 * 4); ca1.x = A.x[n1 * 4 + 2];
        cc0 = *reinterpret_cast<const double2 *>(A.X0 + n1 * 4); cc1.x = A.X0[n1 * 4 + 2];
        node1 = reinterpret_cast<const int *>(A.maps + (size_t)(A.chunk0 + c2) * stride + A.lay.o_nodes)[t & (FEA_G_MAX_NODES - 1)];
      }
      if constexpr (HET) {
        if (wslot * 64 < A.lay.max_elems) {
          pn = A.mat[mid1];
          mid1 = (A.maps + (size_t)(A.chunk0 + c2) * stride + A.lay.o_emat)[t];
        }
      }
    }

    G_LDS_DRAIN();
    G_BARRIER();
    G_STAMP(1);

    __builtin_amdgcn_s_setprio(PRIO_GATHER);
    double acc[9] = {0, 0, 0, 0, 0, 0, 0, 0, 0}, accd = 0;
    if (DOK && t < h.noffd) {
#define G_FETCH(w) (G_ABL(4) ? g_fetch_cheap(sT, w) : g_fetch(sT, w))
#define G_APPLY(r) do { if (G_ABL(2)) g_apply_cheap(r, acc); else g_apply(r, acc, accd); } while (0)
#pragma unroll
      for (int k = 0; k < FEA_G_REGW; ++k)
        if (k < wd) { { const GRead r = G_FETCH(m.cw[k] & 0xFFFFu); G_APPLY(r); } { const GRead r = G_FETCH(m.cw[k] >> 16); G_APPLY(r); } }
      for (int k = FEA_G_REGW; k < wd; ++k) {
        const unsigned w = reinterpret_cast<const unsigned *>(rec + A.lay.o_clist)[k * FEA_G_THREADS + t];
        g_consume(sT, w & 0xFFFFu, acc, accd); g_consume(sT, w >> 16, acc, accd);
      }
      g_finish(acc, accd);
    }
    double dg[6] = {0, 0, 0, 0, 0, 0};
    double fa[3] = {0, 0, 0};
    if (DOK && t >= G_TASK_THREADS && t - G_TASK_THREADS < 4 * nrows) {
#pragma unroll
      for (int k = 0; k < FEA_G_REGW; ++k)
        if (k < h.ddepth) { g_consume_diag<DOF>(sT, m.cw[k] & 0xFFFFu, dg, fa); g_consume_diag<DOF>(sT, m.cw[k] >> 16, dg, fa); }
      for (int k = FEA_G_REGW; k < h.ddepth; ++k) {
        const unsigned w = reinterpret_cast<const unsigned *>(rec + A.lay.o_dlist)[k * FEA_G_DIAG_LANES + t - G_TASK_THREADS];
        g_consume_diag<DOF>(sT, w & 0xFFFFu, dg, fa); g_consume_diag<DOF>(sT, w >> 16, dg, fa);
      }
    }
    if (!DOK && t < h.nvthr) {
      g_visit<DOK>(sT, m.vw[0], fa);
      if (h.vdepth > 1) g_visit<DOK>(sT, m.vw[1], fa);
      for (int v = 2; v < h.vdepth; ++v)
        g_visit<DOK>(sT, reinterpret_cast<const unsigned short *>(rec + A.lay.o_vlist)[v * FEA_G_THREADS + t], fa);
    }
    G_STAMP(2);
    __builtin_amdgcn_s_setprio(PRIO_OUT);
    G_BARRIER();
    G_STAMP(3);

    const int odd = h.b0 & 1;
    double *sK = sT + odd;
    double *sF = DOK ? sT + ((A.lay.max_tile * 9 + 3) & ~1) : sT;
    if (DOK && t < h.noffd && !G_ABL(16)) {
      const int bpos = (int)(m.tpos & 0xFFFFu), mpos = (int)(m.tpos >> 16);
      if (bpos != 0xFFFF) {
#pragma unroll
        for (int q = 0; q < 9; ++q) sK[bpos * 9 + q] = acc[q];
      }
      if (mpos != 0xFFFF) {
#pragma unroll
        for (int i = 0; i < 3; ++i)
#pragma unroll
          for (int j = 0; j < 3; ++j) sK[mpos * 9 + 3 * j + i] = acc[3 * i + j];
      }
    }
    if (DOK && t >= G_TASK_THREADS) {
#pragma unroll
      for (int q = 0; q < 6; ++q) dg[q] = g_quad_sum(dg[q]);
      if (DOF) {
#pragma unroll
        for (int q = 0; q < 3; ++q) fa[q] = g_quad_sum(fa[q]);
      }
      if ((t & 3) == 0 && t - G_TASK_THREADS < 4 * nrows) {
        double *o = sK + m.kd * 9;
        o[0] = dg[0]; o[1] = dg[1]; o[2] = dg[2]; o[3] = dg[1]; o[4] = dg[3]; o[5] = dg[4]; o[6] = dg[2]; o[7] = dg[4]; o[8] = dg[5];
      }
    }
    if (!DOK && t < h.nvthr) { sF[t * 3] = fa[0]; sF[t * 3 + 1] = fa[1]; sF[t * 3 + 2] = fa[2]; }
    G_STAMP(4);
    asm volatile("" : : "v"(mn.eids), "v"(mn.tpos), "v"(mn.cw[0]), "v"(mn.cw[1]), "v"(mn.cw[2]), "v"(mn.cw[3]), "v"(mn.cw[4]), "v"(mn.cw[5]),
                 "v"(mn.vw[0]), "v"(mn.vw[1]), "v"(mn.kd), "v"(mn.vb), "v"(mn.ve), "v"(node1), "v"(hword));
    if constexpr (HET) asm volatile("" : : "v"(mid1), "v"(pn.x), "v"(pn.y));
    if (more && node_lane) {
      sC[t * 3] = ca0; sC[t * 3 + 1] = make_double2(ca1.x, cc0.x); sC[t * 3 + 2] = make_double2(cc0.y, cc1.x);
    }
    hn.r0 = __builtin_amdgcn_readlane(hword, 0); hn.r1 = __builtin_amdgcn_readlane(hword, 1);
    hn.b0 = __builtin_amdgcn_readlane(hword, 2); hn.nb = __builtin_amdgcn_readlane(hword, 3);
    hn.nnode = __builtin_amdgcn_readlane(hword, 4); hn.nelem = __builtin_amdgcn_readlane(hword, 5);
    hn.noffd = __builtin_amdgcn_readlane(hword, 6); hn.depth = __builtin_amdgcn_readlane(hword, 7);
    hn.nvthr = __builtin_amdgcn_readlane(hword, 8); hn.vdepth = __builtin_amdgcn_readlane(hword, 9);
    hn.ddepth = __builtin_amdgcn_readlane(hword, 10);
    hn.wdepth[0] = (unsigned)__builtin_amdgcn_readlane(hword, 11); hn.wdepth[1] = (unsigned)__builtin_amdgcn_readlane(hword, 12);
    hn.wdepth[2] = (unsigned)__builtin_amdgcn_readlane(hword, 13); hn.flags = __builtin_amdgcn_readlane(hword, 14);
    G_BARRIER();
    G_STAMP(5);
    if (!DOK) {
      const int ft = t;
      const int fr = ft / 3, fi = ft - 3 * fr;
      if (fr < nrows) {
        double a = 0;
        for (int k = m.vb; k < m.ve; ++k) a += sF[k * 3 + fi];
        A.f[(size_t)(h.r0 + fr) * 3 + fi] = a;
      }
    }
    if (DOK && DOF && t >= G_TASK_THREADS && (t & 3) == 0 && t - G_TASK_THREADS < 4 * nrows) {
      double *fo = A.f + (size_t)(h.r0 + ((t - G_TASK_THREADS) >> 2)) * 3;
      fo[0] = fa[0]; fo[1] = fa[1]; fo[2] = fa[2];
    }
    if (DOK) {
      double *Kd = A.K + (size_t)h.b0 * 9;
      const int total = h.nb * 9;
      if (odd && t == 0) Kd[0] = sK[0];
      const int npair = (total - odd) >> 1;
      for (int j = t; j < npair; j += FEA_G_THREADS) {
        const int p = odd + 2 * j;
        if (G_ABL(32) && j >= 64) break;
#if G_NT_ROWS
        __builtin_nontemporal_store(*reinterpret_cast<const g_v2d *>(sK + p), reinterpret_cast<g_v2d *>(Kd + p));
#else
        *reinterpret_cast<double2 *>(Kd + p) = *reinterpret_cast<const double2 *>(sK + p);
#endif
      }
      if (((total - odd) & 1) && t == 0) Kd[total - 1] = sK[total - 1];
    }
    G_BARRIER();
    G_STAMP(6);
#ifdef FEAHIP_DEBUG
    if (A.stamps) for (int i = 0; i < 6; ++i) sa[i] += st[i + 1] - st[i];
#endif
    if (!more) break;
    ++chunk;
  }
#ifdef FEAHIP_DEBUG
  if (A.stamps && (t & 63) == 0) {
    unsigned long long *o = A.stamps + ((size_t)ridx * (FEA_G_THREADS / 64) + (t >> 6)) * 8;
    for (int i = 0; i < 6; ++i) o[i] = sa[i];
    o[6] = __builtin_amdgcn_s_memtime() - clk0;
    o[7] = __builtin_amdgcn_s_memrealtime() - real0;
  }
#endif
}

int ensure_gather(feahip_ctx *c)
{
  GatherMaps &g = c->gather;
  if (g.settled(c->row0, c->row1)) return FEAHIP_OK;
  if (!c->h_pat || c->h_conn.empty() || !c->linear_tet || c->G != 1) return FEAHIP_OK;
  g.release();
  HostGather hg;
  build_host_gather(c->N, c->E, c->h_conn.data(), *c->h_pat, c->row0, c->row1, hg, c->n_materials ? c->h_elem_mat.data() : nullptr);
  if (!hg.ok) { g.record(MapOutcome::failed, c->row0, c->row1); return FEAHIP_OK; }
  FEA_HIP_CHECK(c, hipMalloc((void **)&g.d_maps, hg.blob.size() ? hg.blob.size() : 1));
  FEA_HIP_CHECK(c, hipMemcpy(g.d_maps, hg.blob.data(), hg.blob.size(), hipMemcpyHostToDevice));
  g.lay = hg.lay;
  g.nchunks = hg.nchunks;
  g.bytes = (long long)hg.blob.size();
  g.evals_per_element = hg.distinct_elems ? (double)hg.total_evals / (double)hg.distinct_elems : 0.0;
  g.same_words = hg.same_as_previous;
  g.record(MapOutcome::built, c->row0, c->row1);
  return FEAHIP_OK;
}

#ifdef FEAHIP_DEBUG
extern "C" int feahip_debug_gather_record(feahip_ctx *c, int chunk, int *layout_ints, unsigned char *record)
{
  int rc = ensure_gather(c);
  const GatherMaps &g = c->gather;
  if (rc || !g.built()) return FEAHIP_ESTATE;
  if (chunk < 0) chunk = g.nchunks / 2;
  memcpy(layout_ints, &g.lay, sizeof(GatherLayout));
  if (record) (void)hipMemcpy(record, g.d_maps + (size_t)chunk * g.lay.stride, g.lay.stride, hipMemcpyDeviceToHost);
  return (int)(sizeof(GatherLayout) / sizeof(int));
}
#endif

int launch_assemble_gather(feahip_ctx *c, bool doK, bool doF)
{
  const GatherMaps &g = c->gather;
  GatherArgs A;
  A.chunk0 = 0; A.nchunks = g.nchunks; A.model = c->model; A.lambda = c->lambda; A.mu = c->mu;
  A.tab = c->d_table; A.maps = g.d_maps; A.lay = g.lay; A.X0 = c->d_X0; A.x = c->d_x;
  A.K = c->d_K; A.f = c->d_f; A.bad = c->d_flag + 1; A.stamps = nullptr; A.ablate = 0; A.mat = c->d_mat;
  if (g.nchunks <= 0) return FEAHIP_OK;
#ifdef FEAHIP_DEBUG
  static unsigned long long *d_stamps = nullptr;
  static int stamps_cap = 0;
  { const char *e = getenv("FEAHIP_GATHER_ABLATE"); A.ablate = e ? atoi(e) : 0; }
  const char *dbg = getenv("FEAHIP_GATHER_STAMPS");
  if (dbg && atoi(dbg)) {
    if (!d_stamps || stamps_cap < g.nchunks) {
      if (d_stamps) (void)hipFree(d_stamps);
      (void)hipMalloc((void **)&d_stamps, sizeof(unsigned long long) * 8 * (FEA_G_THREADS / 64) * (size_t)g.nchunks);
      (void)hipMemset(d_stamps, 0, sizeof(unsigned long long) * 8 * (FEA_G_THREADS / 64) * (size_t)g.nchunks);
      stamps_cap = g.nchunks;
    }
    A.stamps = d_stamps;
  }
#endif
  static int run_env = -1;
  if (run_env < 0) { const char *e = getenv("FEAHIP_GATHER_RUN"); run_env = e && atoi(e) > 0 ? atoi(e) : 0; }
  static int ncu_of[64];
  int &ncu = ncu_of[c->device & 63];
  if (ncu <= 0) { hipDeviceProp_t p; ncu = (hipGetDeviceProperties(&p, c->device) == hipSuccess && p.multiProcessorCount > 0) ? p.multiProcessorCount : 256; }
  int run_len = 16;
  if (run_env) run_len = run_env;
  else if (FEA_G_BIG == 1) {
    long best = -1;
    for (int k = 2; k >= 1; --k) {
      const int rl = std::max(1, (g.nchunks + k * ncu - 1) / (k * ncu)), nr = (g.nchunks + rl - 1) / rl;
      const long cost = (long)((nr + ncu - 1) / ncu) * rl;
      if (best < 0 || cost < best) { best = cost; run_len = rl; }
    }
  }
  const int nruns = (g.nchunks + run_len - 1) / run_len;
  const dim3 grid((nruns + 7) & ~7), blk(FEA_G_THREADS);
  const int regK = std::max(A.lay.max_elems * GREC, ((A.lay.max_tile * 9 + 3) & ~1) + 3 * FEA_G_THREADS);
  const int regF = std::max(A.lay.max_elems * GREC_F, 3 * FEA_G_THREADS);
  const int ldsK = A.lay.max_nodes * 48 + ((regK + 1) & ~1) * 8, ldsF = A.lay.max_nodes * 48 + ((regF + 1) & ~1) * 8;
  const bool nh = c->model == FEAHIP_MODEL_COMPRESSIBLE_NEOHOOKEAN;
  const bool het = c->n_materials > 0;
  if (het != (g.lay.o_emat != 0)) { c->err = "gather maps and material table disagree"; return FEAHIP_ESTATE; }
  if (het && !nh && doK && !doF) {
    if (!c->d_f_discard) FEA_HIP_CHECK(c, hipMalloc((void **)&c->d_f_discard, sizeof(double) * (size_t)c->ndof));
    A.f = c->d_f_discard;
    doF = true;
  }
  auto launch = [&](auto K, auto F, auto M, auto H) -> int {
    if constexpr (H && K && !F && !M) { c->err = "gather assembly: no K-only A5 kernel with a material table"; return FEAHIP_ESTATE; }
    else {
    const int lds = K ? ldsK : ldsF;
    FEA_HIP_CHECK(c, hipFuncSetAttribute(reinterpret_cast<const void *>(&k_assemble_gather<K, F, M, H>), hipFuncAttributeMaxDynamicSharedMemorySize, lds));
    hipLaunchKernelGGL((k_assemble_gather<K, F, M, H>), grid, blk, lds, c->stream, A, run_len);
    return FEAHIP_OK;
    }
  };
  int rc;
  with_kf(doK, doF, [&](auto K, auto F) {
    auto model = [&](auto H) { return nh ? launch(K, F, std::true_type(), H) : launch(K, F, std::false_type(), H); };
    rc = het ? model(std::true_type()) : model(std::false_type());
  });
  if (rc) return rc;
  FEA_HIP_CHECK(c, hipGetLastError());
#ifdef FEAHIP_DEBUG
  if (A.stamps) {
    static int calls = 0;
    if (++calls == 50) {
      (void)hipStreamSynchronize(c->stream);
      constexpr int NW = FEA_G_THREADS / 64;
      std::vector<unsigned long long> hst((size_t)g.nchunks * 8 * NW);
      (void)hipMemcpy(hst.data(), A.stamps, hst.size() * 8, hipMemcpyDeviceToHost);
      double sum[NW][8] = {};
      for (int i = 0; i < nruns; ++i)
        for (int w = 0; w < NW; ++w)
          for (int q = 0; q < 8; ++q) sum[w][q] += (double)hst[((size_t)i * NW + w) * 8 + q];
      fprintf(stderr, "[gather stamps] in-kernel clock %.0f MHz (s_memtime / s_memrealtime x 100 MHz over a run), run = %.0f shader cycles for %d chunks\n",
              sum[0][7] > 0 ? 100.0 * sum[0][6] / sum[0][7] : 0.0, sum[0][6] / nruns, run_len);
      for (int w = 0; w < NW; w += (NW > 4 ? 5 : 1))
        fprintf(stderr, "[gather stamps K=%d F=%d wave %d, per chunk] state %.0f  gather %.0f  barrier B %.0f  tile writes %.0f  wait for the prefetched words + coordinates + barrier C %.0f  rows out (+ barrier D) %.0f cycles\n",
                (int)doK, (int)doF, w, sum[w][0] / g.nchunks, sum[w][1] / g.nchunks, sum[w][2] / g.nchunks, sum[w][3] / g.nchunks,
                sum[w][4] / g.nchunks, sum[w][5] / g.nchunks);
    }
  }
#endif
  return FEAHIP_OK;
}
```

### fea-large_amd/feahip.py

```python
import ctypes as C
import os

import numpy as np

_HERE = os.path.dirname(os.path.abspath(__file__))
LIB_PATH = os.environ.get("FEAHIP_LIB") or os.path.join(_HERE, "libfeahip.so")
HOST_LIB_PATH = os.path.join(_HERE, "libfeahost.so")

MODEL_A5, MODEL_COMPRESSIBLE_NEOHOOKEAN = 0, 1
CG, PCG_ILU, CHOLESKY = 0, 1, 2
EINVAL, ESTATE, ENOTCONVERGED = -1, -5, -6
ASM_AUTO, ASM_ROWOWNER, ASM_ATOMIC, ASM_PATCH, ASM_STAGED, ASM_PAIRED, ASM_PIPELINED, ASM_SHARED, ASM_GATHER = 0, 1, 2, 3, 4, 5, 6, 7, 8
TETRAHEDRA10, TETRAHEDRA4, HEXAHEDRA8 = 0, 1, 2
LOAD_PRESSURE, LOAD_TRACTION = 0, 1

_dp = C.POINTER(C.c_double)
_ip = C.POINTER(C.c_int)

ABI = {
    "feahip_create": [C.POINTER(C.c_void_p), C.c_int, C.c_int, C.c_int, C.c_int, C.c_int, _dp, _dp, _ip, _dp,
                      C.c_int, _dp, C.c_int, C.c_int, _ip, _ip, _dp],
    "feahip_destroy": [C.c_void_p],
    "feahip_last_error": [C.c_void_p],
    "feahip_create_error": [],
    "feahip_update_nodes_with_bc": [C.c_void_p, C.c_double],
    "feahip_update_state": [C.c_void_p, _ip],
    "feahip_create_stiffness": [C.c_void_p],
    "feahip_create_residual_forces": [C.c_void_p],
    "feahip_create_stiffness_and_residual": [C.c_void_p],
    "feahip_stash_stiffness": [C.c_void_p],
    "feahip_restore_stiffness": [C.c_void_p],
    "feahip_apply_prescribed_bc": [C.c_void_p, C.c_double],
    "feahip_solve_slae": [C.c_void_p, C.c_int, C.c_double, C.c_int, _ip, _dp],
    "feahip_solve_slae2": [C.c_void_p, C.c_int, C.c_double, C.c_int, _dp, _ip, _dp],
    "feahip_get_solution2": [C.c_void_p, _dp],
    "feahip_spmv2": [C.c_void_p, _dp, _dp],
    "feahip_solve_arclength": [C.c_void_p, C.c_double, C.c_int, C.c_int, C.c_double, C.c_int, C.c_double, C.c_int, _dp, _dp,
                               C.c_int, _ip, _ip],
    "feahip_energy": [C.c_void_p, _dp],
    "feahip_update_nodes_with_solution": [C.c_void_p, _dp],
    "feahip_solve": [C.c_void_p, C.c_int, C.c_int, C.c_int, C.c_double, C.c_int, C.c_double, C.c_int, _dp,
                     C.c_int, _ip, _ip],
    "feahip_set_nodes": [C.c_void_p, _dp],
    "feahip_get_nodes": [C.c_void_p, _dp],
    "feahip_get_forces": [C.c_void_p, _dp],
    "feahip_set_forces": [C.c_void_p, _dp],
    "feahip_get_solution": [C.c_void_p, _dp],
    "feahip_get_graddefs": [C.c_void_p, _dp],
    "feahip_get_stresses": [C.c_void_p, _dp],
    "feahip_get_shape_gradients": [C.c_void_p, _dp, _dp],
    "feahip_matrix_nnz": [C.c_void_p, C.POINTER(C.c_longlong)],
    "feahip_get_matrix_yale": [C.c_void_p, _ip, _ip, _dp],
    "feahip_get_matrix_yale64": [C.c_void_p, C.POINTER(C.c_longlong), _ip, _dp],
    "feahip_spmv": [C.c_void_p, _dp, _dp],
    "feahip_set_assembly": [C.c_void_p, C.c_int],
    "feahip_set_preconditioner": [C.c_void_p, C.c_int],
    "feahip_set_line_search": [C.c_void_p, C.c_int],
    "feahip_set_pcg_variant": [C.c_void_p, C.c_int],
    "feahip_set_row_shard": [C.c_void_p, C.c_int, C.c_int],
    "feahip_comm_unique_id": [C.c_void_p, C.c_int],
    "feahip_comm_init": [C.c_void_p, C.c_int, C.c_int, C.c_void_p],
    "feahip_owned_rows": [C.c_void_p, _ip, _ip],
    "feahip_group_init": [C.POINTER(C.c_void_p), C.c_int],
    "feahip_group_solve_slae": [C.POINTER(C.c_void_p), C.c_int, C.c_int, C.c_double, C.c_int, _ip, _dp],
    "feahip_group_energy": [C.POINTER(C.c_void_p), C.c_int, _dp],
    "feahip_group_update_nodes_with_solution": [C.POINTER(C.c_void_p), C.c_int],
    "feahip_group_solve": [C.POINTER(C.c_void_p), C.c_int, C.c_int, C.c_int, C.c_int, C.c_double, C.c_int,
                           C.c_double, C.c_int, _dp, C.c_int, _ip, _ip],
    "feahip_shard_plan": [C.c_int, C.c_int, C.c_int, _ip, C.c_int, C.c_int, _ip, _ip, _ip, _ip, _ip, _ip],
    "feahip_sync": [C.c_void_p],
    "feahip_time_kernel": [C.c_void_p, C.c_int, C.c_int, C.c_int, _dp],
    "feahip_sizes": [C.c_void_p, C.POINTER(C.c_longlong)],
    "feahip_host_gather_stats": [C.c_int, C.c_int, C.c_int, _ip, C.POINTER(C.c_longlong), _ip],
    "feahip_host_gather10_shape": [C.c_int, C.c_int, C.c_int, _ip, C.POINTER(C.c_longlong)],
    "feahip_host_gather_chunks": [C.c_int, C.c_int, _ip, C.c_int, _ip],
    "feahip_host_assembly_digest": [C.c_int, C.c_int, C.c_int, _ip, C.c_int, C.c_int, C.POINTER(C.c_ulonglong), _ip],
    "feahip_assembly_in_use": [C.c_void_p, _ip],
    "feahip_node_numbering": [C.c_void_p, _ip],
    "feahip_create_rank": [C.POINTER(C.c_void_p), C.c_int, C.c_int, C.c_int, C.c_int, C.c_int, C.c_int, C.c_int, _dp, _dp, _ip, _dp,
                           C.c_int, _dp, C.c_int, C.c_int, _ip, _ip, _dp],
    "feahip_create_rank_local": [C.POINTER(C.c_void_p), C.c_int, C.c_int, C.c_int, C.c_int, C.c_int, C.c_int, C.c_int, C.c_int,
                                 C.c_int, _dp, _dp, _ip, _dp, _ip, _ip, _ip, C.c_int, _dp, C.c_int, C.c_int, _ip, _ip, _dp],
    "feahip_host_rank_local_plan": [C.c_int, C.c_int, C.c_int, C.c_int, C.c_int, C.c_int, _ip, _ip, _ip, _ip, _ip, _ip, _ip,
                                    _ip, _ip],
    "feahip_host_slab_order": [C.c_int, C.c_int, C.c_int, C.c_int, _ip, _dp, _ip],
    "feahip_rank_counts": [C.c_void_p, C.POINTER(C.c_longlong)],
    "feahip_rank_maps": [C.c_void_p, _ip, _ip],
    "feahip_host_rank_plan": [C.c_int, C.c_int, C.c_int, C.c_int, C.c_int, _ip, _dp, _ip, _ip, _ip, _ip, _ip, _ip],
    "feahip_host_rank_mesh": [C.c_int, C.c_int, C.c_int, C.c_int, C.c_int, _ip, _dp, C.POINTER(C.c_longlong), _ip, _ip,
                              C.POINTER(C.c_longlong), _ip],
    "feahip_copy_bandwidth": [C.c_void_p, C.c_longlong, _dp],
    "feahip_copy_bandwidth_detail": [C.c_void_p, C.c_longlong, _dp],
    "feahip_assembly_stats": [C.c_void_p, _dp],
    "feahip_device_layout": [C.c_void_p, C.POINTER(C.c_longlong)],
    "feahip_host_numbering": [C.c_int, C.c_int, C.c_int, _ip, _dp, _ip],
    "feahip_set_surface_loads": [C.c_void_p, C.c_int, C.c_int, _ip, _ip, _dp],
    "feahip_get_surface_forces": [C.c_void_p, _dp],
    "feahip_set_load_factor": [C.c_void_p, C.c_double],
    "feahip_get_load_factor": [C.c_void_p, _dp],
    "feahip_set_materials": [C.c_void_p, C.c_int, _dp, _ip],
    "feahip_get_materials": [C.c_void_p, _ip, _dp, _ip],
    "feahip_host_surface_faces": [C.c_int, C.c_int, C.c_int, _ip, C.c_int, C.c_int, _ip, _ip, _ip, _ip],
    "feahip_apply_preconditioner": [C.c_void_p, _dp, _dp],
    "feahip_amg_info": [C.c_void_p, C.POINTER(C.c_longlong), _dp],
    "feahip_amg_level": [C.c_void_p, C.c_int, C.POINTER(C.c_longlong), _dp, _ip, _ip, _dp, _ip, _dp, _ip],
    "feahip_group_apply_preconditioner": [C.POINTER(C.c_void_p), C.c_int, C.POINTER(_dp), C.POINTER(_dp)],
    "feahip_coarse_info": [C.c_void_p, C.POINTER(C.c_longlong), _ip, _dp],
    "feahip_coarse_matrix": [C.c_void_p, _dp],
    "feahip_host_coarse_aggregates": [C.c_int, C.c_int, _ip],
    "feahip_set_mass": [C.c_void_p, C.c_int, _dp, C.c_int, _dp, _dp, _dp],
    "feahip_mass_spmv": [C.c_void_p, _dp, _dp],
    "feahip_set_body_force": [C.c_void_p, _dp],
    "feahip_set_velocities": [C.c_void_p, _dp],
    "feahip_get_velocities": [C.c_void_p, _dp],
    "feahip_set_accelerations": [C.c_void_p, _dp],
    "feahip_get_accelerations": [C.c_void_p, _dp],
    "feahip_get_time": [C.c_void_p, _dp],
    "feahip_set_time": [C.c_void_p, C.c_double],
    "feahip_consistent_acceleration": [C.c_void_p, C.c_int, C.c_double, C.c_int],
    "feahip_solve_dynamic": [C.c_void_p, C.c_int, C.c_double, C.c_double, C.c_double, C.c_double, C.c_int, C.c_double, C.c_int,
                             C.c_double, C.c_int, _dp, C.c_int, _ip, _ip],
    "feahip_group_solve_dynamic": [C.POINTER(C.c_void_p), C.c_int, C.c_int, C.c_double, C.c_double, C.c_double, C.c_double,
                                   C.c_int, C.c_double, C.c_int, C.c_double, C.c_int, _dp, C.c_int, _ip, _ip],
    "feahip_get_lumped_mass": [C.c_void_p, _dp],
    "feahip_stable_step": [C.c_void_p, _dp],
    "feahip_kinetic_energy": [C.c_void_p, _dp],
    "feahip_solve_explicit": [C.c_void_p, C.c_int, C.c_double, C.c_double, C.c_int, C.c_double, _dp, C.c_int, _ip],
    "feahip_group_solve_explicit": [C.POINTER(C.c_void_p), C.c_int, C.c_int, C.c_double, C.c_double, C.c_int, C.c_double, _dp,
                                    C.c_int, _ip],
}
MASS_POINTS = {TETRAHEDRA4: 4, TETRAHEDRA10: 27, HEXAHEDRA8: 8}
COARSE_INFO_KEYS = ("aggregates", "first_aggregate", "local_aggregates", "unknowns", "epoch", "owned_rows", "m", "pairs")
AMG_INFO_KEYS = ("levels", "gamma", "gamma_from", "gamma_until", "coarse_sweeps", "fine_bits", "coarse_f32", "fused_post",
                 "tail_from", "tail_entry", "tail_cop", "tail_lds_levels", "row0", "row1", "tail_blob")
TAIL_ENTRY = {0: None, 1: "lds", 2: "ell", 3: "l2"}

_lib = None
_host = None


class FeaHipError(RuntimeError):
    pass


def load_library():
    global _lib
    if _lib is None:
        if not os.path.exists(LIB_PATH):
            raise FeaHipError(
                f"{LIB_PATH} is missing: build it with `python -c 'import __graft_entry__ as g; g.build()'`; "
                "there is no fallback implementation")
        lib = C.CDLL(LIB_PATH)
        for name, args in ABI.items():
            fn = getattr(lib, name)
            fn.argtypes = args
            fn.restype = C.c_char_p if name in ("feahip_last_error", "feahip_create_error") else (
                None if name == "feahip_destroy" else C.c_int)
        _lib = lib
    return _lib


class FeaDeck(C.Structure):
    _fields_ = [
        ("model", C.c_int), ("parameters", C.c_double * 10), ("parameters_count", C.c_int),
        ("solver_type", C.c_int), ("solver_tolerance", C.c_double), ("solver_max_iter", C.c_int),
        ("ele_type", C.c_int), ("load_increments_count", C.c_int), ("desired_tolerance", C.c_double),
        ("max_newton_count", C.c_int), ("linesearch_max", C.c_int), ("arclength_max", C.c_int),
        ("modified_newton", C.c_int), ("nodes_per_element", C.c_int), ("gauss_nodes_count", C.c_int),
        ("nodes_count", C.c_int), ("nodes", _dp), ("elements_count", C.c_int), ("elements", _ip),
        ("prescribed_nodes_count", C.c_int), ("presc_node", _ip), ("presc_type", _ip), ("presc_values", _dp),
        ("surface_faces_count", C.c_int), ("surface_nodes_per_face", C.c_int), ("surface_nodes", _ip),
        ("surface_kind", _ip), ("surface_values", _dp),
        ("materials_count", C.c_int), ("material_params", _dp), ("element_material", _ip),
        ("has_dynamics", C.c_int), ("dynamics_steps", C.c_int), ("dynamics_dt", C.c_double), ("dynamics_beta", C.c_double),
        ("dynamics_gamma", C.c_double), ("dynamics_dlambda", C.c_double), ("density", C.c_double),
        ("has_body_force", C.c_int), ("body_force", C.c_double * 3),
        ("dynamics_explicit", C.c_int), ("dynamics_safety", C.c_double), ("dynamics_restep", C.c_int),
    ]


class StepSnapshot(C.Structure):
    _fields_ = [("nodes", _dp), ("stress0", _dp)]


def export_gmsh(path, deck, nodes_steps, stress0_steps):
    h = load_host_library()
    n = len(nodes_steps)
    keep = [(np.ascontiguousarray(a, dtype=np.float64), np.ascontiguousarray(b, dtype=np.float64))
            for a, b in zip(nodes_steps, stress0_steps)]
    arr = (StepSnapshot * max(n, 1))()
    for k, (a, b) in enumerate(keep):
        arr[k].nodes, arr[k].stress0 = _d(a), _d(b)
    fd = deck.to_struct()
    if h.fea_export_gmsh(os.fsencode(path), C.byref(fd), arr, n) != 0:
        raise FeaHipError(f"could not write {path}")


def load_host_library():
    global _host
    if _host is None:
        if not os.path.exists(HOST_LIB_PATH):
            raise FeaHipError(f"{HOST_LIB_PATH} is missing: run __graft_entry__.build()")
        load_library()
        h = C.CDLL(HOST_LIB_PATH)
        h.fea_deck_load.argtypes = [C.c_char_p, C.POINTER(FeaDeck), C.c_char_p, C.c_int]
        h.fea_deck_load.restype = C.c_int
        h.fea_deck_free.argtypes = [C.POINTER(FeaDeck)]
        h.fea_deck_free.restype = None
        h.fea_deck_save.argtypes = [C.c_char_p, C.POINTER(FeaDeck)]
        h.fea_deck_save.restype = C.c_int
        h.fea_element_tables.argtypes = [C.c_int, C.c_int, _dp, _dp, _dp]
        h.fea_element_tables.restype = C.c_int
        h.fea_deck_create_solver.argtypes = [C.POINTER(FeaDeck), C.c_int, C.POINTER(C.c_void_p), C.c_char_p, C.c_int]
        h.fea_deck_create_solver.restype = C.c_int
        h.fea_solve.argtypes = [C.POINTER(FeaDeck), C.c_void_p, C.c_void_p, _dp, C.c_int]
        h.fea_solve.restype = C.c_int
        h.fea_export_gmsh.argtypes = [C.c_char_p, C.POINTER(FeaDeck), C.POINTER(StepSnapshot), C.c_int]
        h.fea_export_gmsh.restype = C.c_int
        h.fea_export_name.argtypes = [C.c_char_p, C.c_char_p]
        h.fea_export_name.restype = None
        _host = h
    return _host


def _d(a):
    return a.ctypes.data_as(_dp)


def _i(a):
    return a.ctypes.data_as(_ip)


def element_tables(ele_type, gauss_count):
    h = load_host_library()
    npe = {TETRAHEDRA10: 10, TETRAHEDRA4: 4, HEXAHEDRA8: 8}[ele_type]
    w = np.zeros(gauss_count)
    forms = np.zeros((gauss_count, npe))
    dforms = np.zeros((gauss_count, 3, npe))
    rc = h.fea_element_tables(ele_type, gauss_count, _d(w), _d(forms), _d(dforms))
    if rc < 0:
        raise FeaHipError(f"unsupported element type {ele_type} with {gauss_count} Gauss points")
    return w, forms, dforms


def _take_dynamics(obj, kw):
    obj.density = kw.get("density")
    bf = kw.get("body_force")
    obj.body_force = None if bf is None else np.ascontiguousarray(bf, dtype=np.float64).reshape(3)
    dyn = kw.get("dynamics")
    obj.dynamics = None if dyn is None else {"steps": int(dyn.get("steps", 0)), "dt": float(dyn["dt"]),
                                             "beta": float(dyn.get("beta", 0.25)), "gamma": float(dyn.get("gamma", 0.5)),
                                             "dlambda": float(dyn.get("dlambda", 0.0))}
    if dyn is not None and dyn.get("scheme", "newmark") != "newmark":
        if dyn["scheme"] != "explicit":
            raise ValueError("dynamics scheme: newmark or explicit")
        obj.dynamics.update(scheme="explicit", safety=float(dyn.get("safety", 0.9)), restep=int(dyn.get("restep", 0)))
    elif dyn is not None and ("safety" in dyn or "restep" in dyn):
        raise ValueError("safety and restep belong to the explicit scheme")
    if (obj.dynamics is not None or obj.body_force is not None) and obj.density is None:
        raise ValueError("dynamics and body_force need a density")


class Deck:

    def __init__(self, **kw):
        self.model = kw.get("model", MODEL_COMPRESSIBLE_NEOHOOKEAN)
        self.parameters = np.array(kw.get("parameters", [100.0, 100.0]), dtype=np.float64)
        self.solver_type = kw.get("solver_type", CG)
        self.solver_tolerance = kw.get("solver_tolerance", 1e-14)
        self.solver_max_iter = kw.get("solver_max_iter", 20000)
        self.ele_type = kw.get("ele_type", TETRAHEDRA10)
        self.load_increments_count = kw.get("load_increments_count", 1)
        self.desired_tolerance = kw.get("desired_tolerance", 1e-8)
        self.max_newton_count = kw.get("max_newton_count", 20)
        self.modified_newton = kw.get("modified_newton", True)
        self.gauss_nodes_count = kw.get("gauss_nodes_count", 5)
        self.linesearch_max = kw.get("linesearch_max", 0)
        self.arclength_max = kw.get("arclength_max", 0)
        self.nodes = np.ascontiguousarray(kw["nodes"], dtype=np.float64)
        self.elements = np.ascontiguousarray(kw["elements"], dtype=np.int32)
        self.nodes_per_element = self.elements.shape[1]
        self.presc_node = np.ascontiguousarray(kw.get("presc_node", []), dtype=np.int32)
        self.presc_type = np.ascontiguousarray(kw.get("presc_type", []), dtype=np.int32)
        self.presc_values = np.ascontiguousarray(kw.get("presc_values", np.zeros((0, 3))), dtype=np.float64).reshape(-1, 3)
        faces = np.asarray(kw.get("surface_faces", np.zeros((0, 0))), dtype=np.int32)
        self.surface_faces = np.ascontiguousarray(faces.reshape(len(faces), -1) if faces.size else np.zeros((0, 0), dtype=np.int32))
        self.surface_kind = np.ascontiguousarray(kw.get("surface_kind", []), dtype=np.int32)
        self.surface_values = np.ascontiguousarray(kw.get("surface_values", np.zeros((0, 3))), dtype=np.float64).reshape(-1, 3)
        self.materials = np.ascontiguousarray(kw.get("materials", np.zeros((0, 2))), dtype=np.float64).reshape(-1, 2)
        self.element_material = np.ascontiguousarray(kw.get("element_material", []), dtype=np.int32)
        if len(self.element_material) != (len(self.elements) if len(self.materials) else 0):
            raise ValueError("materials and element_material come together, one id per element")
        _take_dynamics(self, kw)

    @staticmethod
    def load(path):
        h = load_host_library()
        fd = FeaDeck()
        err = C.create_string_buffer(512)
        if h.fea_deck_load(os.fsencode(path), C.byref(fd), err, 512) != 0:
            raise FeaHipError(f"{path}: {err.value.decode()}")
        try:
            n, e, npe, nb = fd.nodes_count, fd.elements_count, fd.nodes_per_element, fd.prescribed_nodes_count
            ns, npf, nm = fd.surface_faces_count, fd.surface_nodes_per_face, fd.materials_count
            deck = Deck(
                model=fd.model, parameters=[fd.parameters[0], fd.parameters[1]], solver_type=fd.solver_type,
                solver_tolerance=fd.solver_tolerance, solver_max_iter=fd.solver_max_iter, ele_type=fd.ele_type,
                load_increments_count=fd.load_increments_count, desired_tolerance=fd.desired_tolerance,
                max_newton_count=fd.max_newton_count, modified_newton=bool(fd.modified_newton),
                gauss_nodes_count=fd.gauss_nodes_count,
                nodes=np.ctypeslib.as_array(fd.nodes, (n, 3)).copy(),
                elements=np.ctypeslib.as_array(fd.elements, (e, npe)).copy(),
                presc_node=np.ctypeslib.as_array(fd.presc_node, (nb,)).copy() if nb else [],
                presc_type=np.ctypeslib.as_array(fd.presc_type, (nb,)).copy() if nb else [],
                presc_values=np.ctypeslib.as_array(fd.presc_values, (nb, 3)).copy() if nb else np.zeros((0, 3)),
                surface_faces=np.ctypeslib.as_array(fd.surface_nodes, (ns, npf)).copy() if ns else np.zeros((0, 0)),
                surface_kind=np.ctypeslib.as_array(fd.surface_kind, (ns,)).copy() if ns else [],
                surface_values=np.ctypeslib.as_array(fd.surface_values, (ns, 3)).copy() if ns else np.zeros((0, 3)),
                materials=np.ctypeslib.as_array(fd.material_params, (nm, 2)).copy() if nm else np.zeros((0, 2)),
                element_material=np.ctypeslib.as_array(fd.element_material, (e,)).copy() if nm else [],
                density=fd.density if fd.has_dynamics else None,
                body_force=[fd.body_force[k] for k in range(3)] if fd.has_body_force else None,
                dynamics=dict(steps=fd.dynamics_steps, dt=fd.dynamics_dt, beta=fd.dynamics_beta, gamma=fd.dynamics_gamma,
                              dlambda=fd.dynamics_dlambda,
                              **(dict(scheme="explicit", safety=fd.dynamics_safety, restep=fd.dynamics_restep)
                                 if fd.dynamics_explicit else {})) if fd.has_dynamics else None)
            deck.linesearch_max, deck.arclength_max = fd.linesearch_max, fd.arclength_max
            return deck
        finally:
            h.fea_deck_free(C.byref(fd))

    def to_struct(self):
        fd = FeaDeck()
        fd.model = self.model
        fd.parameters[0], fd.parameters[1] = float(self.parameters[0]), float(self.parameters[1])
        fd.parameters_count = 2
        fd.solver_type, fd.solver_tolerance, fd.solver_max_iter = self.solver_type, self.solver_tolerance, self.solver_max_iter
        fd.ele_type = self.ele_type
        fd.load_increments_count, fd.desired_tolerance = self.load_increments_count, self.desired_tolerance
        fd.max_newton_count, fd.modified_newton = self.max_newton_count, int(self.modified_newton)
        fd.nodes_per_element, fd.gauss_nodes_count = self.nodes_per_element, self.gauss_nodes_count
        fd.linesearch_max, fd.arclength_max = int(self.linesearch_max), int(self.arclength_max)
        fd.nodes_count, fd.nodes = len(self.nodes), _d(self.nodes)
        fd.elements_count, fd.elements = len(self.elements), _i(self.elements)
        fd.prescribed_nodes_count = len(self.presc_node)
        fd.presc_node, fd.presc_type, fd.presc_values = _i(self.presc_node), _i(self.presc_type), _d(self.presc_values)
        fd.surface_faces_count = len(self.surface_kind)
        fd.surface_nodes_per_face = self.surface_faces.shape[1] if len(self.surface_kind) else 0
        fd.surface_nodes, fd.surface_kind, fd.surface_values = _i(self.surface_faces), _i(self.surface_kind), _d(self.surface_values)
        self.materials = np.ascontiguousarray(self.materials, dtype=np.float64).reshape(-1, 2)
        self.element_material = np.ascontiguousarray(self.element_material, dtype=np.int32)
        fd.materials_count = len(self.materials)
        fd.material_params, fd.element_material = _d(self.materials), _i(self.element_material)
        if getattr(self, "density", None) is not None:
            rho = np.atleast_1d(np.asarray(self.density, dtype=np.float64))
            if len(rho) != 1:
                raise ValueError("the deck grammar holds one density; per-material densities go through set_mass")
            dyn = getattr(self, "dynamics", None) or {"steps": 0, "dt": 1.0, "beta": 0.25, "gamma": 0.5, "dlambda": 0.0}
            fd.has_dynamics, fd.density = 1, float(rho[0])
            fd.dynamics_steps, fd.dynamics_dt = dyn["steps"], dyn["dt"]
            fd.dynamics_beta, fd.dynamics_gamma, fd.dynamics_dlambda = dyn["beta"], dyn["gamma"], dyn["dlambda"]
            if dyn.get("scheme") == "explicit":
                fd.dynamics_explicit, fd.dynamics_safety, fd.dynamics_restep = 1, dyn["safety"], dyn["restep"]
            if getattr(self, "body_force", None) is not None:
                fd.has_body_force = 1
                for k in range(3):
                    fd.body_force[k] = float(self.body_force[k])
        return fd

    def save(self, path):
        h = load_host_library()
        fd = self.to_struct()
        if h.fea_deck_save(os.fsencode(path), C.byref(fd)) != 0:
            raise FeaHipError(f"could not write {path}")


class FeaSolver:

# ... 239 lines not shown
        self._chk(self._lib.feahip_solve_dynamic(
            self._ctx, ns, float(dyn.get("dt", 0.0) if dt is None else dt), float(dyn.get("beta", 0.25) if beta is None else beta),
            float(dyn.get("gamma", 0.5) if gamma is None else gamma), float(dyn.get("dlambda", 0.0) if dlambda is None else dlambda),
            mn, d.desired_tolerance if desired_tolerance is None else desired_tolerance,
            d.solver_type if solver_type is None else solver_type,
            d.solver_tolerance if solver_tolerance is None else solver_tolerance,
            d.solver_max_iter if solver_max_iter is None else solver_max_iter, _d(tol_log), cap, _i(its), C.byref(done)))
        n = int(its[:min(done.value + 1, ns)].sum())
        return done.value, its[:ns], tol_log[:n]

    def lumped_mass(self):
        ml = np.zeros(self.N)
        self._chk(self._lib.feahip_get_lumped_mass(self._ctx, _d(ml)))
        return ml

    def stable_step(self):
        dt = C.c_double(0)
        self._chk(self._lib.feahip_stable_step(self._ctx, C.byref(dt)))
        return dt.value

    def kinetic_energy(self):
        e = C.c_double(0)
        self._chk(self._lib.feahip_kinetic_energy(self._ctx, C.byref(e)))
        return e.value

    def solve_explicit(self, n_steps=None, dt=None, safety=None, restep=None, dlambda=None, check=True):
        dyn = getattr(self.deck, "dynamics", None) or {}
        ns = int(dyn.get("steps", 0) if n_steps is None else n_steps)
        log, done = np.zeros(max(ns, 1)), C.c_int(0)
        rc = self._lib.feahip_solve_explicit(
            self._ctx, ns, float(dyn.get("dt", 0.0) if dt is None else dt),
            float(dyn.get("safety", 0.9) if safety is None else safety), int(dyn.get("restep", 0) if restep is None else restep),
            float(dyn.get("dlambda", 0.0) if dlambda is None else dlambda), _d(log), len(log), C.byref(done))
        if check or rc != ENOTCONVERGED:
            self._chk(rc)
        taken = log[:ns][log[:ns] > 0]
        return (done.value, taken) if check else (done.value, taken, rc)

    def set_surface_loads(self, faces, kind, values):
        kind = np.ascontiguousarray(kind, dtype=np.int32).reshape(-1)
        n = len(kind)
        faces = np.ascontiguousarray(faces, dtype=np.int32).reshape(n, -1) if n else np.zeros((0, 1), dtype=np.int32)
        values = np.ascontiguousarray(values, dtype=np.float64).reshape(n, 3) if n else np.zeros((0, 3))
        self._chk(self._lib.feahip_set_surface_loads(self._ctx, n, faces.shape[1] if n else 0, _i(faces), _i(kind), _d(values)))

    def surface_forces(self):
        f = np.zeros(self.ndof)
        self._chk(self._lib.feahip_get_surface_forces(self._ctx, _d(f)))
        return f

    def load_factor(self):
        v = C.c_double(0)
        self._chk(self._lib.feahip_get_load_factor(self._ctx, C.byref(v)))
        return v.value

    def set_load_factor(self, lam):
        self._chk(self._lib.feahip_set_load_factor(self._ctx, lam))

    def set_nodes(self, x):
        x = np.ascontiguousarray(x, dtype=np.float64)
        assert x.shape == (self.N, 3)
        self._chk(self._lib.feahip_set_nodes(self._ctx, _d(x)))

    def nodes(self):
        x = np.zeros((self.N, 3))
        self._chk(self._lib.feahip_get_nodes(self._ctx, _d(x)))
        return x

    def shape_gradients(self):
        g = np.zeros((self.E, self.G, 3, self.npe))
        d = np.zeros((self.E, self.G))
        self._chk(self._lib.feahip_get_shape_gradients(self._ctx, _d(g), _d(d)))
        return g, d

    def forces(self):
        f = np.zeros(self.ndof)
        self._chk(self._lib.feahip_get_forces(self._ctx, _d(f)))
        return f

    def set_forces(self, f):
        f = np.ascontiguousarray(f, dtype=np.float64)
        assert f.shape == (self.ndof,)
        self._chk(self._lib.feahip_set_forces(self._ctx, _d(f)))

    def solution(self):
        u = np.zeros(self.ndof)
        self._chk(self._lib.feahip_get_solution(self._ctx, _d(u)))
        return u

    def graddefs(self):
        F = np.zeros((self.E, self.G, 3, 3))
        self._chk(self._lib.feahip_get_graddefs(self._ctx, _d(F)))
        return F

    def stresses(self):
        S = np.zeros((self.E, self.G, 3, 3))
        self._chk(self._lib.feahip_get_stresses(self._ctx, _d(S)))
        return S

    def matrix_yale(self):
        nnz = C.c_longlong(0)
        self._chk(self._lib.feahip_matrix_nnz(self._ctx, C.byref(nnz)))
        off = np.zeros(self.ndof + 1, dtype=np.int32)
        idx = np.zeros(nnz.value, dtype=np.int32)
        val = np.zeros(nnz.value)
        self._chk(self._lib.feahip_get_matrix_yale(self._ctx, _i(off), _i(idx), _d(val)))
        return off, idx, val

    def matrix_yale64(self):
        nnz = C.c_longlong(0)
        self._chk(self._lib.feahip_matrix_nnz(self._ctx, C.byref(nnz)))
        off = np.zeros(self.ndof + 1, dtype=np.int64)
        idx = np.zeros(nnz.value, dtype=np.int32)
        val = np.zeros(nnz.value)
        self._chk(self._lib.feahip_get_matrix_yale64(self._ctx, off.ctypes.data_as(C.POINTER(C.c_longlong)), _i(idx), _d(val)))
        return off, idx, val

    def spmv(self, x):
        x = np.ascontiguousarray(x, dtype=np.float64)
        y = np.zeros(self.ndof)
        self._chk(self._lib.feahip_spmv(self._ctx, _d(x), _d(y)))
        return y

    def spmv2(self, x2):
        x2 = np.ascontiguousarray(x2, dtype=np.float64)
        assert x2.shape == (2, self.ndof)
        y2 = np.zeros((2, self.ndof))
        self._chk(self._lib.feahip_spmv2(self._ctx, _d(x2), _d(y2)))
        return y2

    def set_preconditioner(self, kind):
        self._chk(self._lib.feahip_set_preconditioner(self._ctx, kind))
        self.preconditioner = kind

    def coarse_info(self):
        o = (C.c_longlong * 8)()
        self._chk(self._lib.feahip_coarse_info(self._ctx, o, None, None))
        d = dict(zip(COARSE_INFO_KEYS, [int(v) for v in o]))
        agg = np.zeros(max(d["owned_rows"], 1), dtype=np.int32)
        cent = np.zeros((max(d["aggregates"], 1), 3))
        self._chk(self._lib.feahip_coarse_info(self._ctx, o, _i(agg), _d(cent)))
        d.update(zip(COARSE_INFO_KEYS, [int(v) for v in o]))
        d["agg"], d["centroids"] = agg[:d["owned_rows"]], cent[:d["aggregates"]]
        return d

    def coarse_matrix(self):
        n = self.coarse_info()["unknowns"]
        A = np.zeros((n, n))
        self._chk(self._lib.feahip_coarse_matrix(self._ctx, _d(A)))
        return A

    def apply_preconditioner(self, r):
        r = np.ascontiguousarray(r, dtype=np.float64).ravel()
        z = np.zeros(self.ndof)
        self._chk(self._lib.feahip_apply_preconditioner(self._ctx, _d(r), _d(z)))
        return z

    def amg_info(self):
        o = (C.c_longlong * 16)()
        over = C.c_double(0)
        self._chk(self._lib.feahip_amg_info(self._ctx, o, C.byref(over)))
        d = dict(zip(AMG_INFO_KEYS, [int(v) for v in o]))
        d["tail_entry"] = TAIL_ENTRY[d["tail_entry"]]
        d["coarse_f32"], d["fused_post"], d["tail_cop"], d["tail_blob"] = (bool(d[k]) for k in ("coarse_f32", "fused_post", "tail_cop", "tail_blob"))
        d["tail_lds_levels"] = [l for l in range(d["levels"]) if d["tail_lds_levels"] >> l & 1]
        d["over"] = over.value
        return d

    def amg_level(self, level):
        cnt = (C.c_longlong * 4)()
        om = C.c_double(0)
        self._chk(self._lib.feahip_amg_level(self._ctx, level, cnt, C.byref(om), None, None, None, None, None, None))
        N, nnzb, Nc, bits = (int(v) for v in cnt)
        rowptr, colidx = np.zeros(N + 1, dtype=np.int32), np.zeros(max(nnzb, 1), dtype=np.int32)
        K, agg = np.zeros((max(nnzb, 1), 3, 3)), np.zeros(max(N, 1), dtype=np.int32)
        doff, typ = np.zeros((max(N, 1), 3)), np.zeros(max(N, 1), dtype=np.int32)
        self._chk(self._lib.feahip_amg_level(self._ctx, level, cnt, C.byref(om), _i(rowptr), _i(colidx), _d(K), _i(agg),
                                             _d(doff), _i(typ)))
        return dict(N=N, nnzb=nnzb, Nc=Nc, bits=bits, omega=om.value, rowptr=rowptr, colidx=colidx[:nnzb], K=K[:nnzb],
                    agg=agg[:N], doff=doff[:N], type=typ[:N])

    def set_pcg_variant(self, variant):
        self._chk(self._lib.feahip_set_pcg_variant(self._ctx, variant))

    def set_line_search(self, max_iterations):
        self._chk(self._lib.feahip_set_line_search(self._ctx, max_iterations))

    def set_assembly(self, strategy):
        self._chk(self._lib.feahip_set_assembly(self._ctx, strategy))

    def set_row_shard(self, rank, nranks):
        self._chk(self._lib.feahip_set_row_shard(self._ctx, rank, nranks))

    def owned_rows(self):
        a, b = C.c_int(0), C.c_int(0)
        self._chk(self._lib.feahip_owned_rows(self._ctx, C.byref(a), C.byref(b)))
        return a.value, b.value

    def node_numbering(self):
        out = np.empty(self.N, dtype=np.int32)
        self._chk(self._lib.feahip_node_numbering(self._ctx, _i(out)))
        return out

    def owned_nodes(self):
        r0, r1 = self.owned_rows()
        lib = self.node_numbering()
        return np.nonzero((lib >= r0) & (lib < r1))[0]

    def owned_dofs(self):
        return (3 * self.owned_nodes()[:, None] + np.arange(3)[None, :]).ravel()

    def comm_init(self, rank, nranks, unique_id):
        buf = C.create_string_buffer(bytes(unique_id), 128)
        self._chk(self._lib.feahip_comm_init(self._ctx, rank, nranks, buf))

    def sync(self):
        self._chk(self._lib.feahip_sync(self._ctx))

    def time_kernel(self, what, warmup=2, iters=10):
        ms = C.c_double(0)
        self._chk(self._lib.feahip_time_kernel(self._ctx, what, warmup, iters, C.byref(ms)))
        return ms.value

    def sizes(self):
        o = (C.c_longlong * 8)()
        self._chk(self._lib.feahip_sizes(self._ctx, o))
        keys = ["N", "E", "npe", "G", "nnzb", "nchunks", "aux_bytes", "max_rowlen"]
        return dict(zip(keys, [int(v) for v in o]))

    def copy_bandwidth(self, nbytes=1 << 30):
        v = C.c_double(0)
        self._chk(self._lib.feahip_copy_bandwidth(self._ctx, nbytes, C.byref(v)))
        return v.value

    def assembly_stats(self):
        v = (C.c_double * 4)()
        self._chk(self._lib.feahip_assembly_stats(self._ctx, v))
        return {"evals_per_element": float(v[0]), "chunks": int(v[1]), "chunks_with_predecessors_words": int(v[2]), "map_bytes": int(v[3])}

    def copy_bandwidth_detail(self, nbytes=1 << 30):
        v = (C.c_double * 4)()
        self._chk(self._lib.feahip_copy_bandwidth_detail(self._ctx, nbytes, v))
        return [float(x) for x in v]

    def device_layout(self):
        o = (C.c_longlong * 4)()
        self._chk(self._lib.feahip_device_layout(self._ctx, o))
        return {"K": int(o[0]), "colidx": int(o[1]), "p": int(o[2]), "q": int(o[3])}

    def assembly_in_use(self):
        v = C.c_int(0)
        self._chk(self._lib.feahip_assembly_in_use(self._ctx, C.byref(v)))
        return v.value


def host_numbering(elements, nodes):
    el = np.ascontiguousarray(elements, dtype=np.int32)
    x = np.ascontiguousarray(nodes, dtype=np.float64)
    out = np.empty(len(x), dtype=np.int32)
    rc = load_library().feahip_host_numbering(len(x), el.shape[0], el.shape[1], _i(el), _d(x), _i(out))
    if rc < 0:
        raise FeaHipError(f"feahip_host_numbering failed ({rc})")
    return out, bool(rc)


def host_surface_faces(elements, n_nodes, faces):
    el = np.ascontiguousarray(elements, dtype=np.int32)
    fc = np.ascontiguousarray(faces, dtype=np.int32)
    fc = fc.reshape(len(fc), -1)
    fe, fl = np.full(len(fc), -1, dtype=np.int32), np.full(len(fc), -1, dtype=np.int32)
    bad = C.c_int(-1)
    rc = load_library().feahip_host_surface_faces(n_nodes, el.shape[0], el.shape[1], _i(el), len(fc), fc.shape[1],
                                                  _i(fc), _i(fe), _i(fl), C.byref(bad))
    if rc not in (0, -1):
        raise FeaHipError(f"feahip_host_surface_faces failed ({rc})")
    return fe, fl, int(bad.value)


def host_gather_stats(elements, n_nodes):
    el = np.ascontiguousarray(elements, dtype=np.int32)
    st = np.zeros(8, dtype=np.int64)
    hist = np.zeros(65, dtype=np.int32)
    rc = load_library().feahip_host_gather_stats(n_nodes, el.shape[0], el.shape[1], _i(el), st.ctypes.data_as(C.POINTER(C.c_longlong)), _i(hist))
    if rc:
        raise FeaHipError(f"feahip_host_gather_stats failed ({rc})")
    return {"chunks": int(st[0]), "evals": int(st[1]), "elements": int(st[2]), "rows": int(st[3]),
            "evals_per_element": float(st[1]) / float(st[2]), "rows_per_chunk": float(st[3]) / float(st[0]),
            "chunks_with_predecessors_words": int(st[4]), "map_bytes": int(st[5]),
            "chunks_with_long_block_lists": int(st[6]), "chunks_with_long_diagonal_lists": int(st[7])}, hist


def host_gather_chunks(elements, n_nodes):
    el = np.ascontiguousarray(elements, dtype=np.int32)
    lib = load_library()
    n = lib.feahip_host_gather_chunks(n_nodes, el.shape[0], _i(el), 0, None)
    if n < 0:
        raise FeaHipError(f"feahip_host_gather_chunks failed ({n})")
    flags = np.zeros(n, dtype=np.int32)
    if lib.feahip_host_gather_chunks(n_nodes, el.shape[0], _i(el), n, _i(flags)) != n:
        raise FeaHipError("feahip_host_gather_chunks: chunk count changed")
    return flags


G10_LIMITS = {0: None, 1: "elements", 2: "row length", 3: "tasks", 4: "residual lanes", 5: "list length", 6: "passes",
              7: "other"}


def host_gather10_shape(elements, n_nodes):
    el = np.ascontiguousarray(elements, dtype=np.int32)
    o = np.zeros(16, dtype=np.int64)
    rc = load_library().feahip_host_gather10_shape(n_nodes, el.shape[0], el.shape[1], _i(el), o.ctypes.data_as(C.POINTER(C.c_longlong)))
    if rc:
        raise FeaHipError(f"feahip_host_gather10_shape failed ({rc})")
    ok = bool(o[0])
    return {"ok": ok, "limit": G10_LIMITS[int(o[1])], "chunks": int(o[2]), "max_elems": int(o[3]), "max_nodes": int(o[4]),
            "max_passes": int(o[5]), "min_passes": int(o[6]) if ok else 0, "longest_list": int(o[7]),
            "chunks_with_long_lists": int(o[8]), "max_fdw": int(o[9]), "tile_blocks": int(o[10]),
            "chunks_at_elem_limit": int(o[11]), "zero_slot": int(o[12]), "first_long_list_chunk": int(o[13]),
            "limit_row": int(o[14]), "max_rows": int(o[15])}


def host_assembly_digest(elements, n_nodes, rank=0, nranks=1):
    el = np.ascontiguousarray(elements, dtype=np.int32)
    h = np.zeros(n_nodes, dtype=np.uint64)
    rows = np.zeros(2, dtype=np.int32)
    rc = load_library().feahip_host_assembly_digest(n_nodes, el.shape[0], el.shape[1], _i(el), rank, nranks,
                                                    h.ctypes.data_as(C.POINTER(C.c_ulonglong)), _i(rows))
    if rc:
        raise FeaHipError(f"feahip_host_assembly_digest failed ({rc})")
    return h, (int(rows[0]), int(rows[1]))


def host_coarse_aggregates(n_owned, m):
    lib = load_library()
    mr = lib.feahip_host_coarse_aggregates(n_owned, m, None)
    if mr < 1:
        raise FeaHipError(f"feahip_host_coarse_aggregates failed ({mr})")
    first = np.zeros(mr + 1, dtype=np.int32)
    lib.feahip_host_coarse_aggregates(n_owned, m, _i(first))
    return first


def comm_unique_id():
    buf = C.create_string_buffer(128)
    n = load_library().feahip_comm_unique_id(buf, 128)
    if n <= 0:
        raise FeaHipError(f"feahip_comm_unique_id failed ({n})")
    return bytes(buf.raw[:128])


def shard_plan(deck, rank, nranks):
    lib = load_library()
    el = np.ascontiguousarray(deck.elements, dtype=np.int32)
    counts = np.zeros(5, dtype=np.int32)
    args = (len(deck.nodes), len(el), el.shape[1], _i(el), rank, nranks)
    rc = lib.feahip_shard_plan(*args, _i(counts), None, None, None, None, None)
    if rc != 0:
        raise FeaHipError(f"feahip_shard_plan failed ({rc})")
    npeer, nsend, nrecv = int(counts[0]), int(counts[1]), int(counts[2])
    peers = np.zeros(max(npeer, 1), dtype=np.int32)
    soff, roff = np.zeros(npeer + 1, dtype=np.int32), np.zeros(npeer + 1, dtype=np.int32)
    sidx, ridx = np.zeros(max(nsend, 1), dtype=np.int32), np.zeros(max(nrecv, 1), dtype=np.int32)
    rc = lib.feahip_shard_plan(*args, _i(counts), _i(peers), _i(soff), _i(roff), _i(sidx), _i(ridx))
    if rc != 0:
        raise FeaHipError(f"feahip_shard_plan failed ({rc})")
    return {"row0": int(counts[3]), "row1": int(counts[4]), "peers": [int(p) for p in peers[:npeer]],
            "send": [sidx[soff[k]:soff[k + 1]].copy() for k in range(npeer)],
            "recv": [ridx[roff[k]:roff[k + 1]].copy() for k in range(npeer)]}


class RankSolver(FeaSolver):

    def __init__(self, deck, rank, nranks, device=0):
        self._lib = load_library()
        self._ctx = C.c_void_p()
        self.deck = deck
        w, _, dforms = element_tables(deck.ele_type, deck.gauss_nodes_count)
        self.npe, self.G = deck.nodes_per_element, deck.gauss_nodes_count
        par = np.zeros(10)
        par[:2] = deck.parameters[:2]
        rc = self._lib.feahip_create_rank(
            C.byref(self._ctx), device, rank, nranks, len(deck.nodes), len(deck.elements), self.npe, self.G, _d(w), _d(dforms),
            _i(deck.elements), _d(deck.nodes), deck.model, _d(par), 2, len(deck.presc_node), _i(deck.presc_node),
            _i(deck.presc_type), _d(deck.presc_values))
        if rc != 0:
            self._ctx = C.c_void_p()
            raise FeaHipError(f"feahip_create_rank failed ({rc}): {self._lib.feahip_create_error().decode()}")
        o = (C.c_longlong * 8)()
        self._chk(self._lib.feahip_rank_counts(self._ctx, o))
        self.N, self.n_own, self.E, self.N_global = int(o[0]), int(o[1]), int(o[2]), int(o[3])
        self.nnzb_local, self.nnzb_owned, self.rows_sent, self.rows_received = int(o[4]), int(o[5]), int(o[6]), int(o[7])
        self.ndof = 3 * self.N
        self.node_global = np.empty(self.N, dtype=np.int32)
        self.elem_global = np.empty(self.E, dtype=np.int32)
        self._chk(self._lib.feahip_rank_maps(self._ctx, _i(self.node_global), _i(self.elem_global)))
        self._deck_surface_loads()
        self._deck_materials()
        self._deck_mass()


def host_rank_mesh(deck, rank, nranks, pattern=False):
    lib = load_library()
    el = np.ascontiguousarray(deck.elements, dtype=np.int32)
    x = np.ascontiguousarray(deck.nodes, dtype=np.float64)
    cnt = (C.c_longlong * 8)()
    args = (rank, nranks, len(x), el.shape[0], el.shape[1], _i(el), _d(x))
    rc = lib.feahip_host_rank_mesh(*args, cnt, None, None, None, None)
    if rc != 0:
        raise FeaHipError(f"feahip_host_rank_mesh failed ({rc})")
    names = ("local_nodes", "owned_nodes", "local_elements", "blocks_owned_rows", "blocks_local_rows", "peers", "rows_sent", "rows_received")
    out = {k: int(v) for k, v in zip(names, cnt)}
    if pattern:
        ng = np.empty(out["local_nodes"], dtype=np.int32); eg = np.empty(out["local_elements"], dtype=np.int32)
        rp = np.empty(out["owned_nodes"] + 1, dtype=np.int64); ci = np.empty(max(out["blocks_owned_rows"], 1), dtype=np.int32)
        rc = lib.feahip_host_rank_mesh(*args, cnt, _i(ng), _i(eg), rp.ctypes.data_as(C.POINTER(C.c_longlong)), _i(ci))
        if rc != 0:
            raise FeaHipError(f"feahip_host_rank_mesh failed ({rc})")
        out.update(node_global=ng, elem_global=eg, rowptr=rp, colidx=ci[:out["blocks_owned_rows"]])
    return out


def host_rank_plan(deck, rank, nranks):
    lib = load_library()
    el = np.ascontiguousarray(deck.elements, dtype=np.int32)
    x = np.ascontiguousarray(deck.nodes, dtype=np.float64)
    cnt = np.zeros(3, dtype=np.int32)
    args = (rank, nranks, len(x), el.shape[0], el.shape[1], _i(el), _d(x))
    if lib.feahip_host_rank_plan(*args, _i(cnt), None, None, None, None, None) != 0:
        raise FeaHipError("feahip_host_rank_plan failed")
    npeer, nsend, nrecv = (int(v) for v in cnt)
    peers = np.zeros(max(npeer, 1), dtype=np.int32)
    soff, roff = np.zeros(npeer + 1, dtype=np.int32), np.zeros(npeer + 1, dtype=np.int32)
    sidx, ridx = np.zeros(max(nsend, 1), dtype=np.int32), np.zeros(max(nrecv, 1), dtype=np.int32)
    if lib.feahip_host_rank_plan(*args, _i(cnt), _i(peers), _i(soff), _i(roff), _i(sidx), _i(ridx)) != 0:
        raise FeaHipError("feahip_host_rank_plan failed")
    return {"peers": [int(p) for p in peers[:npeer]],
            "send": [sidx[soff[k]:soff[k + 1]].copy() for k in range(npeer)],
            "recv": [ridx[roff[k]:roff[k + 1]].copy() for k in range(npeer)]}


class Slab:

    def __init__(self, **kw):
        self.model = kw.get("model", MODEL_COMPRESSIBLE_NEOHOOKEAN)
        self.parameters = np.array(kw.get("parameters", [100.0, 100.0]), dtype=np.float64)
        self.solver_type = kw.get("solver_type", CG)
        self.solver_tolerance = kw.get("solver_tolerance", 1e-14)
        self.solver_max_iter = kw.get("solver_max_iter", 20000)
        self.ele_type = kw.get("ele_type", TETRAHEDRA10)
        self.load_increments_count = kw.get("load_increments_count", 1)
        self.desired_tolerance = kw.get("desired_tolerance", 1e-8)
        self.max_newton_count = kw.get("max_newton_count", 20)
        self.modified_newton = kw.get("modified_newton", True)
        self.gauss_nodes_count = kw.get("gauss_nodes_count", 5)
        self.nodes = np.ascontiguousarray(kw["nodes"], dtype=np.float64).reshape(-1, 3)
        self.elements = np.ascontiguousarray(kw["elements"], dtype=np.int32)
        self.nodes_per_element = self.elements.shape[1]
        self.node_global = np.ascontiguousarray(kw["node_global"], dtype=np.int32)
        eg = kw.get("elem_global")
        self.elem_global = np.arange(len(self.elements), dtype=np.int32) if eg is None else np.ascontiguousarray(eg, dtype=np.int32)
        self.n_own = int(kw["n_own"])
        self.n_global_nodes = int(kw["n_global_nodes"])
        self.halo_owner = np.ascontiguousarray(kw.get("halo_owner", []), dtype=np.int32)
        self.presc_node = np.ascontiguousarray(kw.get("presc_node", []), dtype=np.int32)
        self.presc_type = np.ascontiguousarray(kw.get("presc_type", []), dtype=np.int32)
        self.presc_values = np.ascontiguousarray(kw.get("presc_values", np.zeros((0, 3))), dtype=np.float64).reshape(-1, 3)
        faces = np.asarray(kw.get("surface_faces", np.zeros((0, 0))), dtype=np.int32)
        self.surface_faces = np.ascontiguousarray(faces.reshape(len(faces), -1) if faces.size else np.zeros((0, 0), dtype=np.int32))
        self.surface_kind = np.ascontiguousarray(kw.get("surface_kind", []), dtype=np.int32)
        self.surface_values = np.ascontiguousarray(kw.get("surface_values", np.zeros((0, 3))), dtype=np.float64).reshape(-1, 3)
        self.materials = np.ascontiguousarray(kw.get("materials", np.zeros((0, 2))), dtype=np.float64).reshape(-1, 2)
        self.element_material = np.ascontiguousarray(kw.get("element_material", []), dtype=np.int32)
        if len(self.element_material) != (len(self.elements) if len(self.materials) else 0):
            raise ValueError("materials and element_material come together, one id per element")
        _take_dynamics(self, kw)

    def permuted(self, new_local_id):
        import copy
        new = np.ascontiguousarray(new_local_id, dtype=np.int32)
        n, no = len(self.nodes), self.n_own
        if not (np.array_equal(np.sort(new), np.arange(n)) and np.all(new[:no] < no)):
            raise ValueError("not a permutation of the local ids that keeps the owned nodes first")
        out = copy.copy(self)
        out.nodes = np.empty_like(self.nodes); out.nodes[new] = self.nodes
        out.node_global = np.empty_like(self.node_global); out.node_global[new] = self.node_global
        out.halo_owner = np.empty_like(self.halo_owner); out.halo_owner[new[no:] - no] = self.halo_owner
        out.elements = np.ascontiguousarray(new[self.elements])
        out.presc_node = np.ascontiguousarray(new[self.presc_node]) if len(self.presc_node) else self.presc_node
        if len(self.surface_kind):
            out.surface_faces = np.ascontiguousarray(new[self.surface_faces])
        return out

    def reordered(self):
        new = np.empty(len(self.nodes), dtype=np.int32)
        rc = load_library().feahip_host_slab_order(len(self.nodes), self.n_own, len(self.elements), self.nodes_per_element,
                                                   _i(self.elements), _d(self.nodes), _i(new))
        if rc < 0:
            raise FeaHipError(f"feahip_host_slab_order failed ({rc})")
        return self.permuted(new) if rc else self


class LocalRankSolver(FeaSolver):

    def __init__(self, slab, rank, nranks, device=0):
        self._lib = load_library()
        self._ctx = C.c_void_p()
        self.deck = self.slab = slab
        w, _, dforms = element_tables(slab.ele_type, slab.gauss_nodes_count)
        self.npe, self.G = slab.nodes_per_element, slab.gauss_nodes_count
        par = np.zeros(10)
        par[:2] = slab.parameters[:2]
        rc = self._lib.feahip_create_rank_local(
            C.byref(self._ctx), device, rank, nranks, slab.n_global_nodes, len(slab.nodes), slab.n_own, len(slab.elements),
            self.npe, self.G, _d(w), _d(dforms), _i(slab.elements), _d(slab.nodes), _i(slab.node_global), _i(slab.elem_global),
            _i(slab.halo_owner), slab.model, _d(par), 2, len(slab.presc_node), _i(slab.presc_node), _i(slab.presc_type),
            _d(slab.presc_values))
        if rc != 0:
            self._ctx = C.c_void_p()
            raise FeaHipError(f"feahip_create_rank_local failed ({rc}): {self._lib.feahip_create_error().decode()}")
        o = (C.c_longlong * 8)()
        self._chk(self._lib.feahip_rank_counts(self._ctx, o))
        self.N, self.n_own, self.E, self.N_global = int(o[0]), int(o[1]), int(o[2]), int(o[3])
        self.nnzb_local, self.nnzb_owned, self.rows_sent, self.rows_received = int(o[4]), int(o[5]), int(o[6]), int(o[7])
        self.ndof = 3 * self.N
        self.node_global = np.empty(self.N, dtype=np.int32)
        self.elem_global = np.empty(self.E, dtype=np.int32)
        self._chk(self._lib.feahip_rank_maps(self._ctx, _i(self.node_global), _i(self.elem_global)))
        self._deck_surface_loads()
        self._deck_materials()
        self._deck_mass()


def host_rank_local_plan(slab, rank, nranks):
    lib = load_library()
    cnt = np.zeros(3, dtype=np.int32)
    args = (rank, nranks, len(slab.nodes), slab.n_own, len(slab.elements), slab.nodes_per_element, _i(slab.elements),
            _i(slab.node_global), _i(slab.halo_owner))
    rc = lib.feahip_host_rank_local_plan(*args, _i(cnt), None, None, None, None, None)
    if rc != 0:
        raise FeaHipError(f"feahip_host_rank_local_plan failed ({rc}): {lib.feahip_create_error().decode()}")
    npeer, nsend, nrecv = (int(v) for v in cnt)
    peers = np.zeros(max(npeer, 1), dtype=np.int32)
    soff, roff = np.zeros(npeer + 1, dtype=np.int32), np.zeros(npeer + 1, dtype=np.int32)
    sidx, ridx = np.zeros(max(nsend, 1), dtype=np.int32), np.zeros(max(nrecv, 1), dtype=np.int32)
    rc = lib.feahip_host_rank_local_plan(*args, _i(cnt), _i(peers), _i(soff), _i(roff), _i(sidx), _i(ridx))
    if rc != 0:
        raise FeaHipError(f"feahip_host_rank_local_plan failed ({rc}): {lib.feahip_create_error().decode()}")
    return {"peers": [int(p) for p in peers[:npeer]],
            "send": [sidx[soff[k]:soff[k + 1]].copy() for k in range(npeer)],
            "recv": [ridx[roff[k]:roff[k + 1]].copy() for k in range(npeer)]}


def slab_of(deck, rank, nranks):
    N = len(deck.nodes)
    meshes = [host_rank_mesh(deck, r, nranks, pattern=True) for r in range(nranks)]
    owner = np.full(N, -1, dtype=np.int32)
    for r, m in enumerate(meshes):
        owner[m["node_global"][:m["owned_nodes"]]] = r
    m = meshes[rank]
    ng, eg, no = m["node_global"], m["elem_global"], m["owned_nodes"]
    local_of = np.full(N, -1, dtype=np.int64)
    local_of[ng] = np.arange(len(ng))
    kw = {k: getattr(deck, k) for k in ("model", "parameters", "solver_type", "solver_tolerance", "solver_max_iter", "ele_type",
                                         "load_increments_count", "desired_tolerance", "max_newton_count", "modified_newton",
                                         "gauss_nodes_count")}
    keep = local_of[deck.presc_node] >= 0 if len(deck.presc_node) else np.zeros(0, dtype=bool)
    if len(getattr(deck, "surface_kind", [])):
        fl = local_of[deck.surface_faces]
        fk = np.all(fl >= 0, axis=1)
        kw.update(surface_faces=fl[fk], surface_kind=deck.surface_kind[fk], surface_values=deck.surface_values[fk])
    if len(getattr(deck, "materials", [])):
        kw.update(materials=deck.materials, element_material=deck.element_material[eg])
    slab = Slab(nodes=deck.nodes[ng], elements=local_of[deck.elements[eg]], node_global=ng, elem_global=eg, n_own=no,
                n_global_nodes=N, halo_owner=owner[ng[no:]], presc_node=local_of[deck.presc_node[keep]] if keep.any() else [],
                presc_type=deck.presc_type[keep] if keep.any() else [],
                presc_values=deck.presc_values[keep] if keep.any() else np.zeros((0, 3)), **kw)
    for k in ("linesearch_max", "arclength_max", "density", "body_force", "dynamics"):
        if hasattr(deck, k):
            setattr(slab, k, getattr(deck, k))
    return slab


class FeaGroup:

    def __init__(self, deck, n=None, device=0, rank_contexts=False):
        slabs = list(deck) if isinstance(deck, (list, tuple)) else None
        if slabs is not None:
            if n not in (None, len(slabs)):
                raise ValueError("n slabs make n ranks")
            n, rank_contexts = len(slabs), True
        self.deck, self.n = deck, n
        self.n_global = slabs[0].n_global_nodes if slabs is not None else len(deck.nodes)
        self.rank_contexts = rank_contexts
        if slabs is not None:
            self.ranks = [LocalRankSolver(s, r, n, device=device) for r, s in enumerate(slabs)]
        elif rank_contexts:
            self.ranks = [RankSolver(deck, r, n, device=device) for r in range(n)]
        else:
            self.ranks = [FeaSolver(deck, device=device) for _ in range(n)]
        self._lib = load_library()
        self._arr = (C.c_void_p * n)(*[r._ctx for r in self.ranks])
        self._chk(self._lib.feahip_group_init(self._arr, n))
        self.rows = [r.owned_rows() for r in self.ranks]
        if rank_contexts:
            self.nodes = [r.node_global[:r.n_own].astype(np.int64) for r in self.ranks]
        else:
# ... 123 lines not shown
```

### include/fea_hip.h

```cpp
#ifndef FEA_HIP_H
#define FEA_HIP_H

#ifdef __cplusplus
extern "C" {
#endif

typedef struct feahip_ctx feahip_ctx;

enum {
  FEAHIP_OK = 0,
  FEAHIP_EINVAL = -1,
  FEAHIP_ENODEVICE = -2,
  FEAHIP_EHIP = -3,
  FEAHIP_ENOMEM = -4,
  FEAHIP_ESTATE = -5,
  FEAHIP_ENOTCONVERGED = -6,
  FEAHIP_ECOMM = -7
};

enum { FEAHIP_MODEL_A5 = 0, FEAHIP_MODEL_COMPRESSIBLE_NEOHOOKEAN = 1 };
enum { FEAHIP_CG = 0, FEAHIP_PCG_ILU = 1, FEAHIP_CHOLESKY = 2 };
enum {
  FEAHIP_ASM_AUTO = 0,
  FEAHIP_ASM_ROWOWNER = 1,
  FEAHIP_ASM_ATOMIC = 2,
  FEAHIP_ASM_PATCH = 3,
  FEAHIP_ASM_STAGED = 4,
  FEAHIP_ASM_PAIRED = 5,
  FEAHIP_ASM_PIPELINED = 6,
  FEAHIP_ASM_SHARED = 7,
  FEAHIP_ASM_GATHER = 8
};


int feahip_create(feahip_ctx **out, int device,
                  int n_nodes, int n_elems, int npe, int gauss_count,
                  const double *gauss_weights, const double *dforms,
                  const int *elements, const double *nodes0,
                  int model, const double *model_params, int params_count,
                  int n_presc, const int *presc_node, const int *presc_type,
                  const double *presc_values);

void feahip_destroy(feahip_ctx *ctx);

const char *feahip_last_error(const feahip_ctx *ctx);
const char *feahip_create_error(void);


int feahip_update_nodes_with_bc(feahip_ctx *ctx, double lambda);

int feahip_update_state(feahip_ctx *ctx, int *n_bad);

int feahip_create_stiffness(feahip_ctx *ctx);
int feahip_create_residual_forces(feahip_ctx *ctx);
int feahip_create_stiffness_and_residual(feahip_ctx *ctx);

int feahip_stash_stiffness(feahip_ctx *ctx);
int feahip_restore_stiffness(feahip_ctx *ctx);

int feahip_apply_prescribed_bc(feahip_ctx *ctx, double lambda);

int feahip_solve_slae(feahip_ctx *ctx, int solver_type, double tolerance,
                      int max_iterations, int *iters, double *resid);

int feahip_solve_slae2(feahip_ctx *ctx, int solver_type, double tolerance,
                       int max_iterations, const double *f2, int iters[2], double resid[2]);
int feahip_get_solution2(feahip_ctx *ctx, double *u2);

int feahip_energy(feahip_ctx *ctx, double *tolerance);

int feahip_update_nodes_with_solution(feahip_ctx *ctx, const double *u);

int feahip_solve(feahip_ctx *ctx, int load_increments, int max_newton,
                 int modified_newton, double desired_tolerance,
                 int solver_type, double solver_tolerance, int solver_max_iter,
                 double *tol_log, int tol_log_cap, int *its_log,
                 int *steps_done);

int feahip_solve_arclength(feahip_ctx *ctx, double lambda_max, int max_steps, int max_newton,
                           double desired_tolerance, int solver_type, double solver_tolerance,
                           int solver_max_iter, double *lambda_log, double *tol_log, int log_cap,
                           int *its_log, int *steps_done);

enum { FEAHIP_LOAD_PRESSURE = 0, FEAHIP_LOAD_TRACTION = 1 };
int feahip_set_surface_loads(feahip_ctx *ctx, int n_faces, int nodes_per_face, const int *face_nodes,
                             const int *kind, const double *values);
int feahip_get_surface_forces(feahip_ctx *ctx, double *f);
int feahip_set_load_factor(feahip_ctx *ctx, double lambda);
int feahip_get_load_factor(feahip_ctx *ctx, double *lambda);

#define FEAHIP_MAX_MATERIALS 256
int feahip_set_materials(feahip_ctx *ctx, int n_materials, const double *params, const int *elem_material);
int feahip_get_materials(feahip_ctx *ctx, int *n_materials, double *params, int *elem_material);
int feahip_set_mass(feahip_ctx *ctx, int n_rho, const double *rho, int mass_points, const double *weights,
                    const double *forms, const double *dforms);
int feahip_mass_spmv(feahip_ctx *ctx, const double *x, double *y);
int feahip_set_body_force(feahip_ctx *ctx, const double b[3]);
int feahip_set_velocities(feahip_ctx *ctx, const double *v);
int feahip_get_velocities(feahip_ctx *ctx, double *v);
int feahip_set_accelerations(feahip_ctx *ctx, const double *a);
int feahip_get_accelerations(feahip_ctx *ctx, double *a);
int feahip_get_time(feahip_ctx *ctx, double *t);
int feahip_set_time(feahip_ctx *ctx, double t);
int feahip_consistent_acceleration(feahip_ctx *ctx, int solver_type, double tolerance, int max_iterations);
int feahip_solve_dynamic(feahip_ctx *ctx, int n_steps, double dt, double beta, double gamma, double dlambda,
                         int max_newton, double desired_tolerance, int solver_type, double solver_tolerance,
                         int solver_max_iter, double *tol_log, int tol_log_cap, int *its_log, int *steps_done);

int feahip_host_surface_faces(int n_nodes, int n_elems, int npe, const int *elements, int n_faces,
                              int nodes_per_face, const int *face_nodes, int *face_elem, int *face_local,
                              int *bad);

int feahip_comm_unique_id(void *out, int cap);
int feahip_comm_init(feahip_ctx *ctx, int rank, int nranks, const void *unique_id);
int feahip_owned_rows(feahip_ctx *ctx, int *row0, int *row1);

int feahip_create_rank(feahip_ctx **out, int device, int rank, int nranks,
                       int n_nodes, int n_elems, int npe, int gauss_count,
                       const double *gauss_weights, const double *dforms,
                       const int *elements, const double *nodes0,
                       int model, const double *model_params, int params_count,
                       int n_presc, const int *presc_node, const int *presc_type,
                       const double *presc_values);
int feahip_create_rank_local(feahip_ctx **out, int device, int rank, int nranks,
        int n_global_nodes,
        int n_local, int n_own,
        int n_elems, int npe, int gauss_count,
        const double *gauss_weights, const double *dforms,
        const int *elements,
        const double *nodes0,
        const int *node_global,
        const int *elem_global,
        const int *halo_owner,
        int model, const double *model_params, int params_count,
        int n_presc, const int *presc_node , const int *presc_type,
        const double *presc_values);
int feahip_host_rank_local_plan(int rank, int nranks, int n_local, int n_own, int n_elems, int npe,
        const int *elements, const int *node_global, const int *halo_owner,
        int *counts3, int *peers, int *send_off, int *recv_off, int *send_idx, int *recv_idx);
int feahip_host_slab_order(int n_local, int n_own, int n_elems, int npe, const int *elements,
        const double *nodes0, int *new_local_id);
int feahip_rank_counts(feahip_ctx *ctx, long long *out8);
int feahip_rank_maps(feahip_ctx *ctx, int *node_global, int *elem_global);
int feahip_host_rank_mesh(int rank, int nranks, int n_nodes, int n_elems, int npe,
                          const int *elements, const double *nodes0, long long *counts8,
                          int *node_global, int *elem_global, long long *rowptr, int *colidx);

int feahip_host_rank_plan(int rank, int nranks, int n_nodes, int n_elems, int npe,
                          const int *elements, const double *nodes0, int *counts3, int *peers,
                          int *send_off, int *recv_off, int *send_idx, int *recv_idx);

int feahip_group_init(feahip_ctx **ctxs, int n);
int feahip_group_solve_slae(feahip_ctx **ctxs, int n, int solver_type, double tolerance,
                            int max_iterations, int *iters, double *resid);
int feahip_group_energy(feahip_ctx **ctxs, int n, double *tolerance);
int feahip_group_update_nodes_with_solution(feahip_ctx **ctxs, int n);
int feahip_group_solve(feahip_ctx **ctxs, int n, int load_increments, int max_newton,
                       int modified_newton, double desired_tolerance, int solver_type,
                       double solver_tolerance, int solver_max_iter, double *tol_log,
                       int tol_log_cap, int *its_log, int *steps_done);
int feahip_group_solve_dynamic(feahip_ctx **ctxs, int n, int n_steps, double dt, double beta, double gamma,
                               double dlambda, int max_newton, double desired_tolerance, int solver_type,
                               double solver_tolerance, int solver_max_iter, double *tol_log, int tol_log_cap,
                               int *its_log, int *steps_done);
int feahip_get_lumped_mass(feahip_ctx *ctx, double *ml);
int feahip_stable_step(feahip_ctx *ctx, double *dt_crit);
int feahip_kinetic_energy(feahip_ctx *ctx, double *e);
int feahip_solve_explicit(feahip_ctx *ctx, int n_steps, double dt, double safety, int restep,
                          double dlambda, double *dt_log, int dt_log_cap, int *steps_done);
int feahip_group_solve_explicit(feahip_ctx **ctxs, int n, int n_steps, double dt, double safety,
                                int restep, double dlambda, double *dt_log, int dt_log_cap,
                                int *steps_done);
int feahip_group_apply_preconditioner(feahip_ctx **ctxs, int n, const double *const *r,
                                      double *const *z);

int feahip_shard_plan(int n_nodes, int n_elems, int npe, const int *elements, int rank,
                      int nranks, int *counts, int *peers, int *send_off, int *recv_off,
                      int *send_idx, int *recv_idx);
int feahip_host_assembly_digest(int n_nodes, int n_elems, int npe, const int *elements, int rank, int nranks,
                                unsigned long long *rowhash, int *rows);

int feahip_host_gather_stats(int n_nodes, int n_elems, int npe, const int *elements,
                             long long *stats, int *rows_hist);

int feahip_host_gather_chunks(int n_nodes, int n_elems, const int *elements, int capacity, int *flags);

#define FEAHIP_G10_SHAPE_LEN 16
enum {
  FEAHIP_G10_LIMIT_NONE = 0, FEAHIP_G10_LIMIT_ELEMS = 1, FEAHIP_G10_LIMIT_ROW_LENGTH = 2,
  FEAHIP_G10_LIMIT_TASKS = 3, FEAHIP_G10_LIMIT_RESIDUAL_LANES = 4, FEAHIP_G10_LIMIT_LIST_LENGTH = 5,
  FEAHIP_G10_LIMIT_PASSES = 6, FEAHIP_G10_LIMIT_OTHER = 7
};
int feahip_host_gather10_shape(int n_nodes, int n_elems, int npe, const int *elements, long long *out);

int feahip_node_numbering(feahip_ctx *ctx, int *library_id_of_node);
int feahip_host_numbering(int n_nodes, int n_elems, int npe, const int *elements,
                          const double *nodes0, int *library_id_of_node);


int feahip_set_nodes(feahip_ctx *ctx, const double *nodes);
int feahip_get_nodes(feahip_ctx *ctx, double *nodes);
int feahip_get_forces(feahip_ctx *ctx, double *f);
int feahip_set_forces(feahip_ctx *ctx, const double *f);
int feahip_get_solution(feahip_ctx *ctx, double *u);
int feahip_get_graddefs(feahip_ctx *ctx, double *F);
int feahip_get_stresses(feahip_ctx *ctx, double *S);
int feahip_get_shape_gradients(feahip_ctx *ctx, double *grads, double *detj);

int feahip_matrix_nnz(feahip_ctx *ctx, long long *nnz);
int feahip_get_matrix_yale(feahip_ctx *ctx, int *offsets, int *indexes,
                           double *values);
int feahip_get_matrix_yale64(feahip_ctx *ctx, long long *offsets, int *indexes,
                             double *values);
int feahip_spmv(feahip_ctx *ctx, const double *x, double *y);
int feahip_spmv2(feahip_ctx *ctx, const double *x2, double *y2);


int feahip_set_assembly(feahip_ctx *ctx, int strategy);
int feahip_set_preconditioner(feahip_ctx *ctx, int kind);
int feahip_apply_preconditioner(feahip_ctx *ctx, const double *r, double *z);
int feahip_coarse_info(feahip_ctx *ctx, long long *out8, int *agg_of_owned_row, double *centroids);
int feahip_coarse_matrix(feahip_ctx *ctx, double *A);
int feahip_host_coarse_aggregates(int n_owned, int m, int *first_row_of_aggregate);
int feahip_amg_info(feahip_ctx *ctx, long long *out16, double *over);
int feahip_amg_level(feahip_ctx *ctx, int level, long long *counts, double *omega, int *rowptr, int *colidx,
                     double *K, int *agg, double *doff, int *type);
int feahip_set_pcg_variant(feahip_ctx *ctx, int variant);
int feahip_set_line_search(feahip_ctx *ctx, int max_iterations);
int feahip_set_row_shard(feahip_ctx *ctx, int rank, int nranks);
int feahip_sync(feahip_ctx *ctx);
int feahip_time_kernel(feahip_ctx *ctx, int what, int warmup, int iters,
                       double *avg_ms);
int feahip_copy_bandwidth(feahip_ctx *ctx, long long bytes, double *gbytes_per_s);
int feahip_copy_bandwidth_detail(feahip_ctx *ctx, long long bytes, double *out4);
int feahip_device_layout(feahip_ctx *ctx, long long *out4);
int feahip_sizes(feahip_ctx *ctx, long long *out8);
int feahip_assembly_stats(feahip_ctx *ctx, double *out4);
int feahip_assembly_in_use(feahip_ctx *ctx, int *strategy);

#ifdef __cplusplus
}
#endif
#endif
```

Before: 15.92 billion elements/s.

## Balance diagonal-row waves with block waves across SIMDs using a cost model

Rows in each gather chunk are sorted by visit count and packed into the diagonal waves, so each diagonal wave gets its own depth. Block-task waves and diagonal waves are then placed on wave slots together using a per-wave cost estimate, keeping the better of a cost-based and a word-count-based deal. The diagonal loop now runs to its own wave depth instead of the chunk maximum, and the row index is encoded in the upper bits of each diagonal word. The intent is to cut per-SIMD imbalance and wasted diagonal iterations, at the price of a more complex host builder and a hand-tuned cost model. A host API that exports the gather records is also added for inspection.

Result: no change. 15.86 billion elements/s (-0.4%).

```diff
diff --git a/fea-large_amd/csrc/feahip_internal.h b/fea-large_amd/csrc/feahip_internal.h
--- a/fea-large_amd/csrc/feahip_internal.h
+++ b/fea-large_amd/csrc/feahip_internal.h
@@ -193,9 +193,10 @@
   int ddepth;
   unsigned wdepth[3];
   int flags;
-  int pad[1];
-};
-static_assert(sizeof(GatherHeader) == 64 && FEA_G_TASK_THREADS / 64 <= 12, "GatherHeader: 64 bytes, twelve block-wave slots");
+  unsigned dwdepth;
+};
+static_assert(sizeof(GatherHeader) == 64 && FEA_G_TASK_THREADS / 64 <= 12 && FEA_G_DIAG_LANES / 64 <= 4 && FEA_G_MAX_ROWS <= 64,
+              "GatherHeader: 64 bytes, twelve block-wave slots, four diagonal waves; a row's offset in its chunk is six bits of its diagonal words");
 struct GatherLayout {
   int stride;
   int o_nodes, o_elems, o_bpos, o_rows, o_vlist, o_dlist, o_clist;
diff --git a/fea-large_amd/csrc/gather.cpp b/fea-large_amd/csrc/gather.cpp
--- a/fea-large_amd/csrc/gather.cpp
+++ b/fea-large_amd/csrc/gather.cpp
@@ -88,6 +88,9 @@
 #define G_LA(w) (((w) >> 10) & 3)
 #define G_LB(w) (((w) >> 12) & 3)
 #define G_NGROUPS (FEA_G_THREADS / 16)
+#define G_DIAG_WAVES (FEA_G_DIAG_LANES / 64)
+#define G_NO_ROW 0xFFFFu
+#define G_DIAG_ROW(e0, e1) ((int)(((e0) >> 12) & 15u) | (int)(((e1) >> 12) & 3u) << 4)
 
 namespace {
 inline int b128_group(int t)
@@ -125,6 +128,17 @@
   return partition_rows(cost, row_lo, row_hi, L, alpha, first_row) < 0;
 }
 
+constexpr int G_COST_BLOCK_ENTRY = 100;
+constexpr int G_COST_DIAG_ENTRY = 75;
+constexpr int G_COST_TILE_BLOCK = 40;
+constexpr int G_COST_QUAD_SUMS = 110;
+inline int gather_wave_cost(bool diag, int words, int lanes, int mirrors)
+{
+  if (lanes <= 0) return 0;
+  if (diag) return 2 * words * G_COST_DIAG_ENTRY + G_COST_QUAD_SUMS + G_COST_TILE_BLOCK / 4;
+  return 2 * words * G_COST_BLOCK_ENTRY + G_COST_TILE_BLOCK * (64 + mirrors) / 64;
+}
+
 struct Read { uint16_t set; uint8_t off; };
 
 void sort_unique(std::vector<Read> &rv)
@@ -182,10 +196,11 @@
   const HostPattern &hp;
   const uint8_t *elem_mat;
   int r0 = 0, r1 = 0, nrows = 0, b0 = 0, nb = 0, nelem = 0, nnode = 0, nslots = 0, nnslots = 0;
-  int ntask = 0, wdepth[G_TASK_THREADS / 64] = {0}, dwords = 0, ddwords = 0, zslot = 0;
+  int ntask = 0, wdepth[G_TASK_THREADS / 64] = {0}, dwdepth[G_DIAG_WAVES] = {0}, dwords = 0, ddwords = 0, zslot = 0;
+  int qrow[FEA_G_MAX_ROWS];
   std::vector<int> el, nd, task_of, thr_blk, order, res, eslot, nslot;
   std::vector<uint32_t> btpos;
-  std::vector<std::vector<uint16_t>> blists, lists, dl;
+  std::vector<std::vector<uint16_t>> blists, lists, dl, dll;
   std::vector<std::vector<Read>> reads;
   std::vector<uint8_t> occ;
 
@@ -216,10 +231,7 @@
     nslots = 16 * ((nelem + 1 + 15) / 16); nnslots = 16 * ((nnode + 15) / 16);
     if (nnslots > FEA_G_MAX_NODES || nslots > FEA_G_MAX_SLOTS || nrows > FEA_G_MAX_ROWS) return false;
     L.rows.assign(G_ROWS_U16, 0);
-    for (int a = r0; a < r1; ++a) {
-      L.rows[G_RS + (a - r0)] = (uint16_t)(hp.rowptr[a] - b0);
-      L.rows[G_RD + (a - r0)] = (uint16_t)(hp.diag[a] - b0);
-    }
+    for (int a = r0; a < r1; ++a) L.rows[G_RS + (a - r0)] = (uint16_t)(hp.rowptr[a] - b0);
     L.rows[G_RS + nrows] = (uint16_t)nb;
     chunk_block_tasks(hp, r0, r1, btpos, task_of);
     const int nblk = (int)btpos.size();
@@ -277,30 +289,79 @@
       c0 = c1;
     }
     const int nwaves = (nblk + 63) / 64;
-    std::vector<int> wcost((size_t)nwaves, 0), word((size_t)nwaves);
+    std::vector<int> wwords((size_t)nwaves, 0), wmirr((size_t)nwaves, 0);
+    for (int w = 0; w < nwaves; ++w)
+      for (int l = 0; l < 64 && w * 64 + l < nblk; ++l) {
+        wwords[w] = std::max(wwords[w], words(seq[(size_t)w * 64 + l]));
+        wmirr[w] += (btpos[seq[(size_t)w * 64 + l]] >> 16) != 0xFFFFu;
+      }
+    std::vector<int> rord((size_t)nrows);
+    for (int i = 0; i < nrows; ++i) rord[i] = i;
+    auto visits = [&](int i) { return hp.incptr[r0 + i + 1] - hp.incptr[r0 + i]; };
+    std::stable_sort(rord.begin(), rord.end(), [&](int x, int y) { return visits(x) > visits(y); });
+    int dwords_of[G_DIAG_WAVES], drows_of[G_DIAG_WAVES];
+    for (int j = 0; j < G_DIAG_WAVES; ++j) {
+      drows_of[j] = std::max(0, std::min(16, nrows - 16 * j));
+      dwords_of[j] = drows_of[j] ? ((visits(rord[(size_t)16 * j]) + 3) / 4 + 1) / 2 : 0;
+    }
+    int bslot[NBW], dslot[G_DIAG_WAVES], bslot0[NBW], dslot0[G_DIAG_WAVES];
+    const int heavy = deal_slots(nwaves, wwords.data(), wmirr.data(), dwords_of, drows_of, true, bslot, dslot);
+    const int heavy0 = deal_slots(nwaves, wwords.data(), wmirr.data(), dwords_of, drows_of, false, bslot0, dslot0);
+    if (heavy0 < heavy) { std::copy(bslot0, bslot0 + NBW, bslot); std::copy(dslot0, dslot0 + G_DIAG_WAVES, dslot); }
     for (int w = 0; w < nwaves; ++w) {
-      for (int l = 0; l < 64 && w * 64 + l < nblk; ++l) wcost[w] = std::max(wcost[w], words(seq[(size_t)w * 64 + l]));
-      word[w] = w;
-    }
-    std::stable_sort(word.begin(), word.end(), [&](int x, int y) { return wcost[x] > wcost[y]; });
-    int load[4] = {0, 0, 0, 0}, used[4] = {0, 0, 0, 0};
-    for (int w : word) {
-      int bs = -1;
-      for (int sd = 0; sd < 4; ++sd)
-        if (used[sd] * 4 + sd < NBW && (bs < 0 || load[sd] < load[bs])) bs = sd;
-      const int slot = used[bs] * 4 + bs;
-      ++used[bs]; load[bs] += wcost[w];
-      wdepth[slot] = wcost[w];
+      const int slot = bslot[w];
+      wdepth[slot] = wwords[w];
       for (int l = 0; l < 64 && w * 64 + l < nblk; ++l) thr_blk[(size_t)slot * 64 + l] = seq[(size_t)w * 64 + l];
       ntask = std::max(ntask, slot * 64 + std::min(64, nblk - w * 64));
     }
+    std::fill(qrow, qrow + FEA_G_MAX_ROWS, -1);
+    std::fill(dwdepth, dwdepth + G_DIAG_WAVES, 0);
+    for (int j = 0; j < G_DIAG_WAVES; ++j) {
+      dwdepth[dslot[j]] = dwords_of[j];
+      for (int i = 0; i < drows_of[j]; ++i) qrow[16 * dslot[j] + i] = rord[(size_t)16 * j + i];
+    }
+    dll.assign((size_t)FEA_G_DIAG_LANES, std::vector<uint16_t>());
+    for (int q = 0; q < FEA_G_MAX_ROWS; ++q)
+      for (int k = 0; k < 4 && qrow[q] >= 0; ++k) dll[(size_t)4 * q + k] = dl[(size_t)4 * qrow[q] + k];
     lists.assign((size_t)ntask, std::vector<uint16_t>());
     for (int t = 0; t < ntask; ++t)
       if (thr_blk[t] >= 0) lists[t] = blists[thr_blk[t]];
     int depth = 0, ddepth = 0;
     for (auto &l : lists) depth = std::max(depth, (int)l.size());
     for (auto &l : dl) ddepth = std::max(ddepth, (int)l.size());
-    dwords = (depth + 1) / 2; ddwords = (ddepth + 1) / 2;
+    dwords = (depth + 1) / 2; ddwords = std::max(1, (ddepth + 1) / 2);
+  }
+
+  static int deal_slots(int nwaves, const int *wwords, const int *wmirr, const int *dwords_of, const int *drows_of, bool by_cost,
+                        int *bslot, int *dslot)
+  {
+    constexpr int NBW = G_TASK_THREADS / 64;
+    struct Item { int key, cost, wave; bool diag; };
+    std::vector<Item> items;
+    for (int w = 0; w < nwaves; ++w) {
+      const int c = gather_wave_cost(false, wwords[w], 64, wmirr[w]);
+      items.push_back({by_cost ? c : wwords[w], c, w, false});
+    }
+    if (by_cost)
+      for (int j = 0; j < G_DIAG_WAVES; ++j) {
+        const int c = gather_wave_cost(true, dwords_of[j], drows_of[j], 0);
+        items.push_back({c, c, j, true});
+      }
+    std::stable_sort(items.begin(), items.end(), [](const Item &x, const Item &y) { return x.key != y.key ? x.key > y.key : x.cost > y.cost; });
+    int load[4] = {0, 0, 0, 0}, cost[4] = {0, 0, 0, 0};
+    bool taken[NBW + G_DIAG_WAVES] = {false};
+    if (!by_cost)
+      for (int j = 0; j < G_DIAG_WAVES; ++j) { dslot[j] = j; cost[(NBW + j) & 3] += gather_wave_cost(true, dwords_of[j], drows_of[j], 0); }
+    for (const Item &it : items) {
+      const int lo = it.diag ? NBW : 0, hi = it.diag ? NBW + G_DIAG_WAVES : NBW;
+      int bs = -1;
+      for (int s = lo; s < hi; ++s)
+        if (!taken[s] && (bs < 0 || load[s & 3] < load[bs & 3])) bs = s;
+      taken[bs] = true;
+      load[bs & 3] += it.key; cost[bs & 3] += it.cost;
+      if (it.diag) dslot[it.wave] = bs - NBW; else bslot[it.wave] = bs;
+    }
+    return std::max(std::max(cost[0], cost[1]), std::max(cost[2], cost[3]));
   }
 
   void bank_schedule()
@@ -316,8 +377,8 @@
     };
     for (int t = 0; t < ntask; ++t)
       for (size_t k = 0; k < lists[t].size(); ++k) add_reads(t, (int)k, lists[t][k], false);
-    for (int l = 0; l < 4 * nrows; ++l)
-      for (size_t k = 0; k < dl[l].size(); ++k) add_reads(G_TASK_THREADS + l, (int)k, dl[l][k], true);
+    for (int l = 0; l < FEA_G_DIAG_LANES; ++l)
+      for (size_t k = 0; k < dll[l].size(); ++k) add_reads(G_TASK_THREADS + l, (int)k, dll[l][k], true);
     most_read_first(reads, order);
     for (auto &rv : reads) sort_unique(rv);
     std::vector<int> cap(16, nslots / 16);
@@ -360,9 +421,16 @@
       for (size_t k = 0; k < lists[t].size(); ++k)
         L.clist[((size_t)(k / 2) * FEA_G_THREADS + t) * 2 + (k & 1)] = reslot(lists[t][k]);
     L.dlist.assign((size_t)ddwords * 2 * FEA_G_DIAG_LANES, (uint16_t)zslot);
-    for (int l = 0; l < 4 * nrows; ++l)
-      for (size_t k = 0; k < dl[l].size(); ++k)
-        L.dlist[((size_t)(k / 2) * FEA_G_DIAG_LANES + l) * 2 + (k & 1)] = reslot(dl[l][k]);
+    for (int l = 0; l < FEA_G_DIAG_LANES; ++l)
+      for (size_t k = 0; k < dll[l].size(); ++k)
+        L.dlist[((size_t)(k / 2) * FEA_G_DIAG_LANES + l) * 2 + (k & 1)] = reslot(dll[l][k]);
+    for (int q = 0; q < FEA_G_MAX_ROWS; ++q) {
+      L.rows[G_RD + q] = qrow[q] >= 0 ? (uint16_t)(hp.diag[r0 + qrow[q]] - b0) : (uint16_t)G_NO_ROW;
+      for (int k = 0; k < 4 && qrow[q] >= 0; ++k) {
+        uint16_t *w = &L.dlist[(size_t)(4 * q + k) * 2];
+        w[0] = (uint16_t)(w[0] | (qrow[q] & 15) << 12); w[1] = (uint16_t)(w[1] | (qrow[q] >> 4) << 12);
+      }
+    }
     int vdepth = 1;
     for (;; ++vdepth) {
       int need = 0;
@@ -386,6 +454,7 @@
     h.r0 = r0; h.r1 = r1; h.b0 = b0; h.nb = nb; h.nnode = nnslots; h.nelem = nslots; h.noffd = ntask;
     h.depth = dwords; h.nvthr = nvthr; h.vdepth = vdepth; h.ddepth = ddwords;
     for (int w = 0; w < G_TASK_THREADS / 64; ++w) h.wdepth[w >> 2] |= (unsigned)std::min(wdepth[w], 255) << (8 * (w & 3));
+    for (int j = 0; j < G_DIAG_WAVES; ++j) h.dwdepth |= (unsigned)std::min(dwdepth[j], 255) << (8 * j);
   }
 };
 
@@ -441,6 +510,7 @@
     const GatherHeader &h0 = *reinterpret_cast<const GatherHeader *>(r0), &h1 = *reinterpret_cast<const GatherHeader *>(r1);
     const bool same = h0.nelem == h1.nelem && h0.noffd == h1.noffd && h0.depth == h1.depth && h0.nvthr == h1.nvthr &&
                       h0.vdepth == h1.vdepth && h0.ddepth == h1.ddepth && h0.r1 - h0.r0 == h1.r1 - h1.r0 &&
+                      memcmp(h0.wdepth, h1.wdepth, sizeof(h0.wdepth)) == 0 && h0.dwdepth == h1.dwdepth &&
                       memcmp(r0 + lay.o_elems, r1 + lay.o_elems, (size_t)((lay.o_emat ? lay.o_emat : lay.stride) - lay.o_elems)) == 0;
     if (same) { reinterpret_cast<GatherHeader *>(out.blob.data() + (size_t)p * lay.stride)->flags |= 1; ++out.same_as_previous; }
   }
@@ -521,14 +591,15 @@
         if (mpos != 0xFFFF) rowhash[b] += contribution_hash(b, a, g, 4, lb * 4 + la);
       }
     }
-    for (int l = 0; l < 4 * (h.r1 - h.r0); ++l)
-      for (int k = 0; k < 2 * h.ddepth; ++k) {
+    const uint16_t *rows = reinterpret_cast<const uint16_t *>(rec + lay.o_rows);
+    for (int l = 0; l < FEA_G_DIAG_LANES; ++l)
+      for (int k = 0; k < 2 * h.ddepth && rows[G_RD + (l >> 2)] != G_NO_ROW; ++k) {
         const uint16_t w = dlist[((size_t)(k / 2) * FEA_G_DIAG_LANES + l) * 2 + (k & 1)];
         const int slot = (int)G_SLOT(w), la = G_LA(w);
         if (elems[slot] == 0xFFFFFFFFu) continue;
         int g[4];
         element_nodes(slot, g);
-        const int a = h.r0 + (l >> 2);
+        const int a = h.r0 + G_DIAG_ROW(dlist[(size_t)l * 2], dlist[(size_t)l * 2 + 1]);
         rowhash[a] += contribution_hash(a, a, g, 4, la * 4 + la);
       }
   }
@@ -676,6 +747,26 @@
   return hg.nchunks;
 }
 
+extern "C" int feahip_host_gather_records(int n_nodes, int n_elems, const int *elements, int *info, unsigned char *records,
+                                          long long capacity)
+{
+  if (!elements || !info || n_nodes <= 0 || n_elems <= 0 || capacity < 0 || (capacity > 0 && !records)) return FEAHIP_EINVAL;
+  HostPattern hp;
+  std::string err;
+  int rc = build_host_pattern(n_nodes, n_elems, 4, elements, hp, err);
+  if (rc) return rc;
+  HostGather hg;
+  build_host_gather(n_nodes, n_elems, elements, hp, 0, n_nodes, hg);
+  if (!hg.ok) return FEAHIP_EINVAL;
+  static_assert(sizeof(GatherLayout) == 17 * sizeof(int), "feahip_host_gather_records: info[0..16] is the layout");
+  memcpy(info, &hg.lay, sizeof(GatherLayout));
+  const int tail[11] = {FEA_G_THREADS, FEA_G_TASK_THREADS, FEA_G_MAX_ROWS, FEA_G_REGW, G_RS, G_RD, G_VF,
+                        G_COST_BLOCK_ENTRY, G_COST_DIAG_ENTRY, G_COST_TILE_BLOCK, G_COST_QUAD_SUMS};
+  memcpy(info + 17, tail, sizeof(tail));
+  if ((long long)hg.blob.size() <= capacity) memcpy(records, hg.blob.data(), hg.blob.size());
+  return hg.nchunks;
+}
+
 #ifdef FEAHIP_DEBUG
 extern "C" int feahip_debug_gather_record_host(int n_nodes, int n_elems, const int *elements, int chunk, int *layout_ints,
                                                unsigned char *record, int *nchunks)
diff --git a/fea-large_amd/csrc/gather_device.h b/fea-large_amd/csrc/gather_device.h
--- a/fea-large_amd/csrc/gather_device.h
+++ b/fea-large_amd/csrc/gather_device.h
@@ -35,6 +35,8 @@
 #define G_RS 0
 #define G_RD 66
 #define G_VF 130
+#define G_NO_ROW 0xFFFF
+#define G_DIAG_ROW(w) ((int)(((w) >> 12) & 15u) | (int)(((w) >> 28) & 3u) << 4)
 #define G_SLOT(w) ((w) & 1023u)
 #define G_LA(w) (((w) >> 10) & 3)
 #define G_LB(w) (((w) >> 12) & 3)
diff --git a/fea-large_amd/csrc/kernels_gather.hip b/fea-large_amd/csrc/kernels_gather.hip
--- a/fea-large_amd/csrc/kernels_gather.hip
+++ b/fea-large_amd/csrc/kernels_gather.hip
@@ -61,8 +61,10 @@
     double2 ca0, ca1, cc0, cc1;
     const GMaps m = mn;
     const int nrows = h.r1 - h.r0;
-    const unsigned wdw = wslot < 4 ? h.wdepth[0] : (wslot < 8 ? h.wdepth[1] : h.wdepth[2]);
-    const int wd = wslot < G_TASK_THREADS / 64 ? (int)((wdw >> (8 * (wslot & 3))) & 255u) : 0;
+    constexpr int NBW = G_TASK_THREADS / 64;
+    const unsigned wdw = wslot >= NBW ? h.dwdepth >> (8 * (wslot - NBW))
+                       : (wslot < 4 ? h.wdepth[0] : (wslot < 8 ? h.wdepth[1] : h.wdepth[2])) >> (8 * (wslot & 3));
+    const int wd = (int)(wdw & 255u);
     rec = A.maps + (size_t)(A.chunk0 + chunk) * stride;
 
     __builtin_amdgcn_s_setprio(PRIO_STATE);
@@ -139,11 +141,11 @@
     }
     double dg[6] = {0, 0, 0, 0, 0, 0};
     double fa[3] = {0, 0, 0};
-    if (DOK && t >= G_TASK_THREADS && t - G_TASK_THREADS < 4 * nrows) {
+    if (DOK && wslot >= NBW) {
 #pragma unroll
       for (int k = 0; k < FEA_G_REGW; ++k)
-        if (k < h.ddepth) { g_consume_diag<DOF>(sT, m.cw[k] & 0xFFFFu, dg, fa); g_consume_diag<DOF>(sT, m.cw[k] >> 16, dg, fa); }
-      for (int k = FEA_G_REGW; k < h.ddepth; ++k) {
+        if (k < wd) { g_consume_diag<DOF>(sT, m.cw[k] & 0xFFFFu, dg, fa); g_consume_diag<DOF>(sT, m.cw[k] >> 16, dg, fa); }
+      for (int k = FEA_G_REGW; k < wd; ++k) {
         const unsigned w = reinterpret_cast<const unsigned *>(rec + A.lay.o_dlist)[k * FEA_G_DIAG_LANES + t - G_TASK_THREADS];
         g_consume_diag<DOF>(sT, w & 0xFFFFu, dg, fa); g_consume_diag<DOF>(sT, w >> 16, dg, fa);
       }
@@ -182,7 +184,7 @@
 #pragma unroll
         for (int q = 0; q < 3; ++q) fa[q] = g_quad_sum(fa[q]);
       }
-      if ((t & 3) == 0 && t - G_TASK_THREADS < 4 * nrows) {
+      if ((t & 3) == 0 && m.kd != G_NO_ROW) {
         double *o = sK + m.kd * 9;
         o[0] = dg[0]; o[1] = dg[1]; o[2] = dg[2]; o[3] = dg[1]; o[4] = dg[3]; o[5] = dg[4]; o[6] = dg[2]; o[7] = dg[4]; o[8] = dg[5];
       }
@@ -203,6 +205,7 @@
     hn.ddepth = __builtin_amdgcn_readlane(hword, 10);
     hn.wdepth[0] = (unsigned)__builtin_amdgcn_readlane(hword, 11); hn.wdepth[1] = (unsigned)__builtin_amdgcn_readlane(hword, 12);
     hn.wdepth[2] = (unsigned)__builtin_amdgcn_readlane(hword, 13); hn.flags = __builtin_amdgcn_readlane(hword, 14);
+    hn.dwdepth = (unsigned)__builtin_amdgcn_readlane(hword, 15);
     G_BARRIER();
     G_STAMP(5);
     if (!DOK) {
@@ -214,8 +217,8 @@
         A.f[(size_t)(h.r0 + fr) * 3 + fi] = a;
       }
     }
-    if (DOK && DOF && t >= G_TASK_THREADS && (t & 3) == 0 && t - G_TASK_THREADS < 4 * nrows) {
-      double *fo = A.f + (size_t)(h.r0 + ((t - G_TASK_THREADS) >> 2)) * 3;
+    if (DOK && DOF && t >= G_TASK_THREADS && (t & 3) == 0 && m.kd != G_NO_ROW) {
+      double *fo = A.f + (size_t)(h.r0 + G_DIAG_ROW(m.cw[0])) * 3;
       fo[0] = fa[0]; fo[1] = fa[1]; fo[2] = fa[2];
     }
     if (DOK) {
@@ -366,7 +369,7 @@
           for (int q = 0; q < 8; ++q) sum[w][q] += (double)hst[((size_t)i * NW + w) * 8 + q];
       fprintf(stderr, "[gather stamps] in-kernel clock %.0f MHz (s_memtime / s_memrealtime x 100 MHz over a run), run = %.0f shader cycles for %d chunks\n",
               sum[0][7] > 0 ? 100.0 * sum[0][6] / sum[0][7] : 0.0, sum[0][6] / nruns, run_len);
-      for (int w = 0; w < NW; w += (NW > 4 ? 5 : 1))
+      for (int w = 0; w < NW; ++w)
         fprintf(stderr, "[gather stamps K=%d F=%d wave %d, per chunk] state %.0f  gather %.0f  barrier B %.0f  tile writes %.0f  wait for the prefetched words + coordinates + barrier C %.0f  rows out (+ barrier D) %.0f cycles\n",
                 (int)doK, (int)doF, w, sum[w][0] / g.nchunks, sum[w][1] / g.nchunks, sum[w][2] / g.nchunks, sum[w][3] / g.nchunks,
                 sum[w][4] / g.nchunks, sum[w][5] / g.nchunks);
diff --git a/fea-large_amd/feahip.py b/fea-large_amd/feahip.py
--- a/fea-large_amd/feahip.py
+++ b/fea-large_amd/feahip.py
@@ -74,6 +74,7 @@
     "feahip_host_gather_stats": [C.c_int, C.c_int, C.c_int, _ip, C.POINTER(C.c_longlong), _ip],
     "feahip_host_gather10_shape": [C.c_int, C.c_int, C.c_int, _ip, C.POINTER(C.c_longlong)],
     "feahip_host_gather_chunks": [C.c_int, C.c_int, _ip, C.c_int, _ip],
+    "feahip_host_gather_records": [C.c_int, C.c_int, _ip, _ip, C.POINTER(C.c_ubyte), C.c_longlong],
     "feahip_host_assembly_digest": [C.c_int, C.c_int, C.c_int, _ip, C.c_int, C.c_int, C.POINTER(C.c_ulonglong), _ip],
     "feahip_assembly_in_use": [C.c_void_p, _ip],
     "feahip_node_numbering": [C.c_void_p, _ip],
@@ -919,6 +920,24 @@
     return flags
 
 
+GATHER_INFO = ("stride", "o_nodes", "o_elems", "o_bpos", "o_rows", "o_vlist", "o_dlist", "o_clist", "max_nodes", "max_elems",
+               "max_tile", "max_tasks", "max_depth", "max_vthr", "max_vdepth", "max_ddepth", "o_emat", "threads", "task_threads",
+               "max_rows", "regw", "rs", "rd", "vf", "cost_block_entry", "cost_diag_entry", "cost_tile_block", "cost_quad_sums")
+
+
+def host_gather_records(elements, n_nodes):
+    el = np.ascontiguousarray(elements, dtype=np.int32)
+    fn = load_library().feahip_host_gather_records
+    info = np.zeros(len(GATHER_INFO), dtype=np.int32)
+    n = fn(n_nodes, el.shape[0], _i(el), _i(info), None, 0)
+    if n < 0:
+        raise FeaHipError(f"feahip_host_gather_records failed ({n})")
+    rec = np.zeros((n, int(info[0])), dtype=np.uint8)
+    if fn(n_nodes, el.shape[0], _i(el), _i(info), rec.ctypes.data_as(C.POINTER(C.c_ubyte)), rec.size) != n:
+        raise FeaHipError("feahip_host_gather_records: chunk count changed")
+    return dict(zip(GATHER_INFO, (int(v) for v in info))), rec
+
+
 G10_LIMITS = {0: None, 1: "elements", 2: "row length", 3: "tasks", 4: "residual lanes", 5: "list length", 6: "passes",
               7: "other"}
 
diff --git a/include/fea_hip.h b/include/fea_hip.h
--- a/include/fea_hip.h
+++ b/include/fea_hip.h
@@ -185,6 +185,9 @@
 
 int feahip_host_gather_chunks(int n_nodes, int n_elems, const int *elements, int capacity, int *flags);
 
+int feahip_host_gather_records(int n_nodes, int n_elems, const int *elements, int *info, unsigned char *records,
+                               long long capacity);
+
 #define FEAHIP_G10_SHAPE_LEN 16
 enum {
   FEAHIP_G10_LIMIT_NONE = 0, FEAHIP_G10_LIMIT_ELEMS = 1, FEAHIP_G10_LIMIT_ROW_LENGTH = 2,
```
